# zkemail/zk-email-verify

Measured on NVIDIA H100. Metric: EmailVerifier proofs/sec (witness+prove), higher is better.
Workload: dtype u256 (BN254 Fr/Fq integers, 8x32-bit limbs)

## Files before the change

### include/zkemail_b200.h

```cpp
#ifndef ZKEMAIL_B200_H
#define ZKEMAIL_B200_H

#include <stddef.h>
#include <stdint.h>

#ifdef __cplusplus
extern "C" {
#endif

typedef struct zke_circuit zke_circuit;
typedef struct zke_zkey zke_zkey;
typedef struct zke_ctx zke_ctx;

#define ZKE_FR_BYTES 32

zke_circuit* zke_circuit_build(const char* template_name, const int64_t* params, size_t n_params,
                               char* err, size_t errcap);
zke_circuit* zke_circuit_build_regex(const char* const* parts, const uint8_t* is_public, size_t n_parts, uint32_t msg_len,
                                     char* err, size_t errcap);
zke_circuit* zke_circuit_build_app(const char* spec_json, char* err, size_t errcap);
void zke_circuit_free(zke_circuit* c);
zke_circuit* zke_circuit_from_r1cs(const void* r1cs, size_t len, char* err, size_t errcap);
int64_t zke_circuit_write_r1cs(const zke_circuit* c, uint8_t* out, size_t cap);

typedef struct zke_circuit_info {
    uint32_t n_vars;
    uint32_t n_temps;
    uint32_t n_outputs, n_pub_inputs, n_prv_inputs;
    uint32_t n_public;
    uint32_t n_constraints;
    uint32_t n_levels;
    uint32_t n_ops;
    uint32_t n_coefs;
    uint32_t domain_log2;
    uint32_t n_groups;
    uint64_t nnz_a, nnz_b, nnz_c;
} zke_circuit_info;
int zke_circuit_get_info(const zke_circuit* c, zke_circuit_info* out);

int zke_circuit_group(const zke_circuit* c, uint32_t index, char* name, size_t namecap,
                      uint32_t* first, uint32_t* count, int* kind);
int64_t zke_circuit_input_offset(const zke_circuit* c, const char* name, uint32_t* count);

enum {
    ZKE_ARR_COEFS = 0,
    ZKE_ARR_A_PTR = 1, ZKE_ARR_A_VAR = 2, ZKE_ARR_A_COEF = 3,
    ZKE_ARR_B_PTR = 4, ZKE_ARR_B_VAR = 5, ZKE_ARR_B_COEF = 6,
    ZKE_ARR_C_PTR = 7, ZKE_ARR_C_VAR = 8, ZKE_ARR_C_COEF = 9,
    ZKE_ARR_OPS = 10,
    ZKE_ARR_LEVEL_PTR = 11,
    ZKE_ARR_LC_PTR = 12, ZKE_ARR_LC_VAR = 13, ZKE_ARR_LC_COEF = 14,
    ZKE_ARR_AUX = 15,
    ZKE_ARR_SCOPE_OF_CONSTRAINT = 16,
    ZKE_ARR_SHA_BLOCKS = 17,
    ZKE_ARR_REGEX_SEEDS = 18,
    ZKE_ARR_POSEIDON_BLOCKS = 19
};
const void* zke_circuit_array(const zke_circuit* c, int which, size_t* n_elems);
const char* zke_circuit_scope_name(const zke_circuit* c, uint32_t scope_index);

typedef struct zke_program_stats {
    uint32_t n_levels;
    uint32_t n_iters;
    uint32_t n_ops_kept;
    uint32_t n_coop_ops;
    uint32_t n_terms;
    uint32_t cluster;
    uint64_t digest;
} zke_program_stats;
int zke_circuit_program_stats(const zke_circuit* c, int native_sha, int native_regex, int coop_fpmul, uint32_t cluster,
                              zke_program_stats* out, uint32_t* level_ops, size_t level_cap, char* err, size_t errcap);
enum {
    ZKE_LOWER_NATIVE_SHA = 1, ZKE_LOWER_NATIVE_REGEX = 2, ZKE_LOWER_COOP_FPMUL = 4, ZKE_LOWER_NATIVE_POSEIDON = 8,
    ZKE_LOWER_ALL = 15
};
int zke_circuit_program_stats_ex(const zke_circuit* c, uint32_t flags, uint32_t cluster, zke_program_stats* out,
                                 uint32_t* level_ops, size_t level_cap, char* err, size_t errcap);

int zke_poseidon_hash(const uint8_t* inputs, size_t n, uint8_t* out);

typedef struct zke_registry zke_registry;
int zke_poseidon_batch(const uint8_t* inputs, uint32_t width, size_t count, int device, uint8_t* out, char* err, size_t errcap);
int zke_pubkey_hashes(const uint8_t* moduli, size_t count, uint32_t modulus_bytes, uint32_t n, uint32_t k, int device,
                      uint8_t* out, char* err, size_t errcap);
int zke_domain_key_leaves(const uint8_t* moduli, size_t count, uint32_t modulus_bytes, uint32_t n, uint32_t k,
                          const uint8_t* domains, int device, uint8_t* out, char* err, size_t errcap);
int64_t zke_merkle_build(const uint8_t* leaves, size_t count, uint32_t depth, int device, uint8_t* levels, size_t cap,
                         char* err, size_t errcap);
zke_registry* zke_registry_open(const uint8_t* leaves, size_t count, uint32_t depth, int device, char* err, size_t errcap);
int zke_registry_update(zke_registry* r, const uint64_t* indices, const uint8_t* leaves, size_t k, char* err, size_t errcap);
int zke_registry_nodes(zke_registry* r, const uint32_t* levels, const uint64_t* indices, size_t k, uint8_t* out,
                       char* err, size_t errcap);
int64_t zke_registry_levels(zke_registry* r, uint8_t* out, size_t cap, char* err, size_t errcap);
uint64_t zke_registry_count(const zke_registry* r);
void zke_registry_close(zke_registry* r);
double zke_registry_device_ms(void);


zke_zkey* zke_setup(const zke_circuit* c, uint64_t seed, int device, char* err, size_t errcap);
zke_zkey* zke_zkey_load(const void* zkey_bytes, size_t len, int device, char* err, size_t errcap);
zke_zkey* zke_zkey_load_chunks(const void* const* chunks, const size_t* lens, size_t n_chunks, int device, char* err, size_t errcap);
int64_t zke_zkey_write(const zke_zkey* z, const zke_circuit* c, uint8_t* out, size_t cap);
int zke_zkey_is_toy(const zke_zkey* z);
void zke_zkey_free(zke_zkey* z);
int zke_zkey_info(const zke_zkey* z, uint32_t* n_vars, uint32_t* n_public, uint32_t* domain_log2);
enum {
    ZKE_SEC_ALPHA1 = 101, ZKE_SEC_BETA1 = 102, ZKE_SEC_DELTA1 = 103,
    ZKE_SEC_BETA2 = 104, ZKE_SEC_GAMMA2 = 105, ZKE_SEC_DELTA2 = 106,
    ZKE_SEC_IC = 3, ZKE_SEC_A = 5, ZKE_SEC_B1 = 6, ZKE_SEC_B2 = 7, ZKE_SEC_C = 8, ZKE_SEC_H = 9
};
int64_t zke_zkey_section(const zke_zkey* z, int section, uint8_t* out, size_t cap);

zke_zkey* zke_zkey_from_ptau(const zke_circuit* c, const void* ptau, size_t len, int device, char* err, size_t errcap);
int zke_ptau_info(const zke_circuit* c, const void* ptau, size_t len, uint32_t* power, uint64_t* offsets16, uint64_t* sizes16,
                  char* err, size_t errcap);
int zke_zkey_from_ptau_timing(double* host_ms, double* gpu_ms);
zke_zkey* zke_zkey_contribute(const zke_zkey* prev, const uint8_t* secret32, char* err, size_t errcap);
int zke_zkey_check_contribution(const zke_zkey* prev, const zke_zkey* next, const uint8_t* rand16, char* err, size_t errcap);
int64_t zke_ptau_toy(uint32_t power, const uint8_t* tau_alpha_beta96, int device, uint8_t* out, size_t cap, char* err, size_t errcap);

int64_t zke_ptau_new(uint32_t power, uint8_t* out, size_t cap, char* err, size_t errcap);
int64_t zke_ptau_contribute(const void* ptau, size_t len, const uint8_t* secrets96, int device, uint8_t* out, size_t cap, uint8_t* receipt384,
                            char* err, size_t errcap);
int64_t zke_ptau_prepare(const void* ptau, size_t len, int device, uint8_t* out, size_t cap, char* err, size_t errcap);
int zke_ptau_prepare_timing(double* g1_ms, double* g2_ms);
int zke_ptau_verify(const void* ptau, size_t len, const void* prev, size_t prev_len, const uint8_t* receipt384, const uint8_t* rand16,
                    int device, char* err, size_t errcap);

zke_ctx* zke_ctx_open(const zke_circuit* c, const zke_zkey* zkey_or_null, int device, uint32_t max_batch,
                      char* err, size_t errcap);
void zke_ctx_close(zke_ctx* x);
void* zke_ctx_stream(const zke_ctx* x);
uint64_t zke_kernel_launches(void);

int zke_upload_inputs(zke_ctx* x, const uint8_t* inputs, size_t batch, char* err, size_t errcap);

enum {
    ZKE_STAGE_WITNESS = 0,
    ZKE_STAGE_MATVEC = 1,
    ZKE_STAGE_NTT = 2,
    ZKE_STAGE_MSM_A = 3, ZKE_STAGE_MSM_B1 = 4, ZKE_STAGE_MSM_C = 5,
    ZKE_STAGE_MSM_H = 6,
    ZKE_STAGE_MSM_H_BUCKETS = 7,
    ZKE_STAGE_MSM_B2 = 8,
    ZKE_N_STAGES = 9
};
int zke_ctx_set_lanes(zke_ctx* x, int n);
int zke_ctx_profile(zke_ctx* x, int enable);
int zke_ctx_profile_get(const zke_ctx* x, double* ms_out, uint64_t* count_out);

int zke_witness(zke_ctx* x, const uint8_t* inputs, size_t batch, uint8_t* wtns_out, int32_t* status,
                char* err, size_t errcap);
int zke_load_witness(zke_ctx* x, const uint8_t* wtns, size_t batch, char* err, size_t errcap);
int zke_check_witness(zke_ctx* x, size_t batch, int32_t* status, char* err, size_t errcap);
int zke_prove(zke_ctx* x, size_t batch, const uint8_t* rs, uint8_t* proofs_out, uint8_t* publics_out,
              int32_t* status, char* err, size_t errcap);
int zke_fullprove(zke_ctx* x, const uint8_t* inputs, size_t batch, const uint8_t* rs, uint8_t* proofs_out,
                  uint8_t* publics_out, int32_t* status, char* err, size_t errcap);

int zke_fullprove_submit(zke_ctx* x, const uint8_t* inputs, size_t batch, const uint8_t* rs, char* err, size_t errcap);
int zke_fullprove_collect(zke_ctx* x, uint8_t* proofs_out, uint8_t* publics_out, int32_t* status, char* err, size_t errcap);
int zke_wtns_prove(zke_ctx* x, const void* wtns_bytes, size_t len, const uint8_t* rs, uint8_t* proof_out, uint8_t* publics_out,
                   char* err, size_t errcap);

#define ZKE_SHARD_PARTIAL_BYTES 388
int zke_shard_begin(zke_ctx* x, int rank, int world, char* err, size_t errcap);
void* zke_shard_vector(zke_ctx* x, int which , size_t* n_elems);
int zke_shard_mid(zke_ctx* x, char* err, size_t errcap);
int zke_shard_end(zke_ctx* x, uint8_t* partial_out, uint8_t* publics_out, char* err, size_t errcap);
int zke_shard_combine(const zke_zkey* z, const uint8_t* partials, int world, const uint8_t* rs, uint8_t* proof_out, int32_t* status,
                      char* err, size_t errcap);
int zke_shard_combine_raw(const uint8_t* key_points, const uint8_t* partials, int world, const uint8_t* rs, uint8_t* proof_out,
                          int32_t* status, char* err, size_t errcap);

int zke_verify_json(const char* vkey_json, const char* public_json, const char* proof_json, char* err, size_t errcap);
int zke_verify_batch_json(const char* vkey_json, const char* publics_json, const char* proofs_json, const uint8_t* rand16,
                          uint8_t* ok, char* err, size_t errcap);
typedef struct zke_verifier zke_verifier;
zke_verifier* zke_verifier_open(const char* vkey_json, int device, char* err, size_t errcap);
void zke_verifier_close(zke_verifier* v);
int zke_verifier_batch(zke_verifier* v, size_t n, const uint8_t* proofs, const uint8_t* publics, const uint8_t* rand16,
                       uint8_t* ok, char* err, size_t errcap);
typedef struct zke_agg_srs zke_agg_srs;
zke_agg_srs* zke_agg_srs_from_ptau(const void* ptau_a, size_t len_a, const void* ptau_b, size_t len_b, uint32_t n_max, int device,
                                   char* err, size_t errcap);
void zke_agg_srs_free(zke_agg_srs* s);
uint32_t zke_agg_srs_n_max(const zke_agg_srs* s);
int zke_agg_vk_json(const zke_agg_srs* s, char* out, size_t* len);
size_t zke_agg_bytes(size_t n);
int64_t zke_aggregate(zke_agg_srs* s, const char* vkey_json, size_t n, const uint8_t* proofs, const uint8_t* publics, uint8_t* out,
                      size_t cap, char* err, size_t errcap);
int zke_agg_verify(const char* agg_vk_json, const char* vkey_json, size_t n, const uint8_t* publics, const uint8_t* agg, size_t agg_len,
                   char* err, size_t errcap);
int zke_selftest_pairing_gpu(int device, size_t n, const uint8_t* g1, const uint8_t* g2, uint8_t* out, char* err, size_t errcap);
int zke_zkey_vkey_json(const zke_zkey* z, char* out, size_t* len);
int zke_pairing_alphabeta(const uint8_t* alpha64, const uint8_t* beta128, uint8_t* out384);
int zke_proof_to_json(const uint8_t* proof256, const uint8_t* publics, uint32_t n_public, char* proof_json, size_t* proof_len,
                      char* public_json, size_t* public_len);
int zke_pack_inputs_json(const zke_circuit* c, const char* input_json, uint8_t* out, size_t cap, char* err, size_t errcap);
int zke_fullprove_json(zke_ctx* x, const zke_circuit* c, const char* input_json, char* proof_json, size_t* proof_len,
                       char* public_json, size_t* public_len, char* err, size_t errcap);
int zke_setup_toxic(uint64_t seed, uint8_t* out160);
int zke_selftest_fpmul_hint(uint32_t n, uint32_t k, const uint8_t* a, const uint8_t* b, const uint8_t* p, uint8_t* q, uint8_t* r);

int zke_device_count(void);
const char* zke_version(void);

#ifdef __cplusplus
}
#endif
#endif
```

### zk-email-verify_b200/csrc/engine.cu

```cuda
#include "ff.cuh"
namespace zke { namespace dev { unsigned long long g_kernel_launches = 0; } }
#include "witness.cu"
#include "matvec.cu"
#include "ntt.cu"
#include "msm.cuh"
#include "fixed_base.cuh"
namespace zke { namespace dev {
ZKE_DEFINE_CONSTANT_UPLOAD(upload_constants_engine)
cudaError_t upload_constants_msm_g1(const FieldConsts*, const FieldConsts*);
cudaError_t upload_constants_msm_g2(const FieldConsts*, const FieldConsts*);
cudaError_t upload_constants_fixed_base(const FieldConsts*, const FieldConsts*);
cudaError_t upload_constants_verify(const FieldConsts*, const FieldConsts*);
cudaError_t upload_constants_registry(const FieldConsts*, const FieldConsts*);
} }

#include "../../include/zkemail_b200.h"
#include "cuda_host.hpp"
#include "engine.hpp"
#include "witness_program.hpp"
#include "binfile.hpp"
#include "ec_host.hpp"
#include "setup_host.hpp"
#include <algorithm>
#include <cstdio>
#include <cstring>
#include <atomic>
#include <memory>
#include <mutex>
#include <thread>
#include <unordered_map>

using namespace zke;

void zke::select_device(int device) {
    int n = 0;
    if (cudaGetDeviceCount(&n) != cudaSuccess || n == 0) throw std::runtime_error("no CUDA device available (this library has no CPU fallback)");
    if (device < 0 || device >= n) throw std::runtime_error("bad device index");
    CUDA_OK(cudaSetDevice(device));
    dev::FieldConsts fr, fq;
    fill_consts(fr, fr_params());
    fill_consts(fq, fq_params());
    CUDA_OK(dev::upload_constants_engine(&fr, &fq));
    CUDA_OK(dev::upload_constants_msm_g1(&fr, &fq));
    CUDA_OK(dev::upload_constants_msm_g2(&fr, &fq));
    CUDA_OK(dev::upload_constants_fixed_base(&fr, &fq));
    CUDA_OK(dev::upload_constants_verify(&fr, &fq));
    CUDA_OK(dev::upload_constants_registry(&fr, &fq));
    CUDA_OK(dev::configure_witness_kernel());
}

namespace {

template <class F>
std::vector<AffineH<F>> window_table(const AffineH<F>& gen) {
    std::vector<AffineH<F>> t(32 * 256, AffineH<F>::inf());
    JacobianH<F> base = JacobianH<F>::from_affine(gen);
    for (int w = 0; w < 32; ++w) {
        JacobianH<F> acc = JacobianH<F>::inf();
        for (int d = 1; d < 256; ++d) {
            acc = acc.add(base);
            t[w * 256 + d] = acc.to_affine();
        }
        for (int k = 0; k < 8; ++k) base = base.dbl();
    }
    return t;
}

std::vector<U256> to_standard(const std::vector<Fr>& v) {
    std::vector<U256> out(v.size());
    const unsigned T = std::max(1u, std::min(16u, std::thread::hardware_concurrency()));
    std::vector<std::thread> th;
    for (unsigned t = 0; t < T; ++t)
        th.emplace_back([&, t]() { for (size_t i = v.size() * t / T; i < v.size() * (t + 1) / T; ++i) out[i] = v[i].to_u256(); });
    for (auto& x : th) x.join();
    return out;
}

}

struct zke_zkey {
    uint32_t n_vars = 0, n_public = 0, log_n = 0;
    int device = 0;
    bool toy = false;
    bool delta_one = false;
    G1AffineH alpha1, beta1, delta1;
    G2AffineH beta2, gamma2, delta2;
    std::vector<G1AffineH> ic;
    DevBuf A, B1, B2, C, H;
    int h_levels = 1;
    dev::MsmConfig cfg_h;
    bool has_coefs = false;
    std::vector<uint32_t> a_ptr, a_var, a_coef, b_ptr, b_var, b_coef;
    std::vector<U256> coefs;
};

struct zke_ctx {
    const zke_circuit* circuit = nullptr;
    const zke_zkey* zkey = nullptr;
    int device = 0;
    uint32_t max_batch = 0;
    uint32_t n_vars = 0, n_public = 0, n_inputs = 0;
    cudaStream_t stream = nullptr;
    DevBuf ops, iter_hdr, lc_terms, aux, coop, coef_r, small_inv;
    std::vector<uint32_t> coef_word;
    std::vector<uint32_t> iter_info;
    DevBuf a_ptr, a_terms, b_ptr, b_terms, c_ptr, c_terms;
    dev::DevProgram prog;
    dev::DevR1cs r1cs;
    DevBuf tw_fwd, tw_inv, coset_scale;
    dev::NttTables ntt;
    size_t stride = 0;
    DevBuf inputs, check_flag;
    uint32_t inputs_resident = 0;
    struct Slot {
        bool allocated = false, busy = false;
        DevBuf w_all, inputs, results, first_bad;
        uint8_t* results_host = nullptr;
        uint8_t* publics_host = nullptr;
        std::vector<cudaEvent_t> done;
        cudaEvent_t witness_done = nullptr;
        uint32_t loaded = 0;
        uint32_t batch = 0;
        std::vector<uint8_t> rs;
    };
    Slot slots[2];
    uint64_t n_submitted = 0, n_collected = 0;
    int shard_rank = -1, shard_world = 0, shard_log_g = 0, shard_stage = 0;
    struct Lane { cudaStream_t st = nullptr, heavy = nullptr; cudaEvent_t ev[6] = {}; DevBuf va, vb, vc, vd, msm_ws; };
    Lane lanes[ZKE_MAX_LANES];
    int n_lanes = 1, lanes_alloc = 0;
    int finish_threads = 4;
    dev::MsmConfig cfg_w, cfg_h;
    bool split_streams = true;
    std::vector<uint32_t> bad_host;
    bool profile = false;
    std::vector<cudaEvent_t> ev_pool;
    size_t ev_used = 0;
    struct Span { int stage; size_t e0, e1; };
    std::vector<Span> spans;
    double stage_ms[ZKE_N_STAGES] = {0};
    uint64_t stage_count[ZKE_N_STAGES] = {0};
    cudaEvent_t ev(size_t* idx) {
        if (ev_used == ev_pool.size()) { cudaEvent_t e; cudaEventCreate(&e); ev_pool.push_back(e); }
        *idx = ev_used;
        return ev_pool[ev_used++];
    }
    size_t mark(cudaStream_t st) { size_t i; cudaEventRecord(ev(&i), st); return i; }
    size_t mark() { return mark(stream); }
    void collect() {
        for (auto& s : spans) {
            float ms = 0;
            if (cudaEventElapsedTime(&ms, ev_pool[s.e0], ev_pool[s.e1]) == cudaSuccess) { stage_ms[s.stage] += ms; stage_count[s.stage]++; }
        }
        spans.clear();
        ev_used = 0;
    }
};

static const uint32_t SETUP_SLAB = 1u << 20;
static void h_table_config(zke_zkey* zk, size_t N) {
    const char* e = getenv("ZKE_H_PRECOMP");
    const bool precomp = !(e && atoi(e) == 0);
    zk->cfg_h = dev::msm_config_full((uint32_t)N, precomp);
    zk->h_levels = precomp ? dev::msm_windows(zk->cfg_h) : 1;
}
static void build_h_levels(zke_zkey* zk, size_t N, uint8_t* scratch, cudaStream_t st) {
    for (int lvl = 1; lvl < zk->h_levels; ++lvl) {
        const uint8_t* prev = zk->H.p + (size_t)(lvl - 1) * N * sizeof(dev::G1Affine);
        uint8_t* cur = zk->H.p + (size_t)lvl * N * sizeof(dev::G1Affine);
        for (size_t off = 0; off < N; off += SETUP_SLAB) {
            uint32_t cnt = (uint32_t)std::min<size_t>(SETUP_SLAB, N - off);
            dev::scale_pow2_batch<dev::Fq>(prev + sizeof(dev::G1Affine) * off, cnt, zk->cfg_h.c, scratch, cur + sizeof(dev::G1Affine) * off, st);
        }
    }
    CHECK_LAUNCH();
    CUDA_OK(cudaStreamSynchronize(st));
}

static zke_zkey* do_setup(const zke_circuit* zc, uint64_t seed, int device) {
    select_device(device);
    const Circuit& c = zc->c;
    SetupScalars S = compute_setup_scalars(c, seed);
    std::unique_ptr<zke_zkey> zk(new zke_zkey());
    zk->n_vars = c.n_vars; zk->n_public = c.n_public(); zk->log_n = S.log_n; zk->device = device;
    zk->toy = true;
    const size_t N = (size_t)1 << S.log_n;
    const uint32_t m = c.n_vars, l = c.n_public();

    G1JacH g1 = G1JacH::from_affine(g1_generator());
    G2JacH g2 = G2JacH::from_affine(g2_generator());
    zk->alpha1 = g1.mul(S.alpha.to_u256()).to_affine();
    zk->beta1 = g1.mul(S.beta.to_u256()).to_affine();
    zk->delta1 = g1.mul(S.delta.to_u256()).to_affine();
    zk->beta2 = g2.mul(S.beta.to_u256()).to_affine();
    zk->gamma2 = g2.mul(S.gamma.to_u256()).to_affine();
    zk->delta2 = g2.mul(S.delta.to_u256()).to_affine();

    DevBuf t1, t2, scal, scratch;
    t1.upload(window_table<Fq>(g1_generator()));
    t2.upload(window_table<Fq2>(g2_generator()));
    const uint32_t SLAB = SETUP_SLAB;
    scratch.alloc((size_t)SLAB * sizeof(dev::G2XYZZ));
    cudaStream_t st = nullptr;

    auto run_g1 = [&](const std::vector<Fr>& s, DevBuf& out) {
        std::vector<U256> std_s = to_standard(s);
        scal.upload(std_s);
        out.alloc(s.size() * sizeof(dev::G1Affine));
        for (size_t off = 0; off < s.size(); off += SLAB) {
            uint32_t cnt = (uint32_t)std::min<size_t>(SLAB, s.size() - off);
            dev::fixed_base_batch<dev::Fq>(t1.p, scal.p + 32 * off, cnt, scratch.p, out.p + sizeof(dev::G1Affine) * off, st);
        }
        CHECK_LAUNCH();
        CUDA_OK(cudaStreamSynchronize(st));
    };
    run_g1(S.a, zk->A);
    run_g1(S.b, zk->B1);
    run_g1(S.kc, zk->C);
    {
        h_table_config(zk.get(), N);
        std::vector<U256> std_s = to_standard(S.h);
        scal.upload(std_s);
        zk->H.alloc((size_t)zk->h_levels * N * sizeof(dev::G1Affine));
        for (size_t off = 0; off < N; off += SLAB) {
            uint32_t cnt = (uint32_t)std::min<size_t>(SLAB, N - off);
            dev::fixed_base_batch<dev::Fq>(t1.p, scal.p + 32 * off, cnt, scratch.p, zk->H.p + sizeof(dev::G1Affine) * off, st);
        }
        build_h_levels(zk.get(), N, scratch.p, st);
    }
    {
        std::vector<U256> std_s = to_standard(S.b);
        scal.upload(std_s);
        zk->B2.alloc((size_t)m * sizeof(dev::G2Affine));
        for (size_t off = 0; off < m; off += SLAB) {
            uint32_t cnt = (uint32_t)std::min<size_t>(SLAB, m - off);
            dev::fixed_base_batch<dev::Fq2>(t2.p, scal.p + 32 * off, cnt, scratch.p, zk->B2.p + sizeof(dev::G2Affine) * off, st);
        }
        CHECK_LAUNCH();
        CUDA_OK(cudaStreamSynchronize(st));
    }
    zk->ic.resize(l + 1);
    CUDA_OK(cudaMemcpy(zk->ic.data(), zk->C.p, sizeof(G1AffineH) * (l + 1), cudaMemcpyDeviceToHost));
    CUDA_OK(cudaMemset(zk->C.p, 0, sizeof(G1AffineH) * (l + 1)));
    return zk.release();
}

namespace {
void split_container(const uint8_t* b, size_t len, SecView sec[11]) {
    if (!b || len < 12 || memcmp(b, "zkey", 4) != 0) throw std::runtime_error("not a .zkey file (bad magic)");
    if (rd32(b + 4) != 1) throw std::runtime_error("unsupported .zkey version");
    for (const BinSection& s : binfile_sections(b, len, ".zkey"))
        if (s.type >= 1 && s.type <= 10) sec[s.type] = s.view;
}

template <class Launch>
int64_t first_flagged(uint32_t* flag, Launch launch) {
    CUDA_OK(cudaMemset(flag, 0xff, 4));
    launch(flag);
    ZKE_COUNT_LAUNCH(1);
    CHECK_LAUNCH();
    uint32_t first = 0;
    CUDA_OK(cudaMemcpy(&first, flag, 4, cudaMemcpyDeviceToHost));
    return first == 0xffffffffu ? -1 : (int64_t)first;
}

template <class F>
__global__ void validate_points_kernel(const uint8_t* __restrict__ pts, uint32_t n, F b, uint32_t* bad) {
    const uint32_t i = blockIdx.x * blockDim.x + threadIdx.x;
    if (i >= n) return;
    const dev::Affine<F> p = dev::Affine<F>::load(pts + sizeof(dev::Affine<F>) * (size_t)i);
    if (p.is_inf()) return;
    if (!dev::below_modulus(p.x) || !dev::below_modulus(p.y) || !(p.y.sqr() == p.x.sqr() * p.x + b)) atomicMin(bad, i);
}

template <class F, class HostF>
int64_t first_invalid_point(const uint8_t* pts, size_t n, const HostF& b_host, uint32_t* flag) {
    if (!n) return -1;
    F b;
    static_assert(sizeof(F) == sizeof(HostF), "host / device field images differ");
    memcpy(&b, &b_host, sizeof(F));
    return first_flagged(flag, [&](uint32_t* f) { validate_points_kernel<F><<<(unsigned)((n + 127) / 128), 128>>>(pts, (uint32_t)n, b, f); });
}

Fq2 g2_twist_b() { return Fq2{Fq::from_u64(3), Fq::zero()} * Fq2{Fq::from_u64(9), Fq::one()}.inv(); }

struct U256HashE {
    size_t operator()(const U256& x) const { return (size_t)(x.v[0] * 0x9E3779B97F4A7C15ull ^ x.v[1] * 31 ^ x.v[2] * 131 ^ x.v[3]); }
};
}

static zke_zkey* do_zkey_load(const SecView sec[11], int device) {
    select_device(device);
    for (int s = 1; s <= 9; ++s) if (!sec[s].p) throw std::runtime_error(".zkey section " + std::to_string(s) + " is missing");
    if (sec[1].n < 4 || rd32(sec[1].p) != 1) throw std::runtime_error("not a Groth16 .zkey (protocol id)");
    const uint8_t* h = sec[2].p;
    const size_t HDR = 4 + 32 + 4 + 32 + 12 + 64 + 64 + 128 + 128 + 64 + 128;
    if (sec[2].n < HDR) throw std::runtime_error(".zkey header section too short");
    if (rd32(h) != 32 || memcmp(h + 4, fq_params().p.v, 32) != 0) throw std::runtime_error(".zkey is not over the BN254 base field");
    if (rd32(h + 36) != 32 || memcmp(h + 40, fr_params().p.v, 32) != 0) throw std::runtime_error(".zkey is not over the BN254 scalar field");
    std::unique_ptr<zke_zkey> zk(new zke_zkey());
    zk->device = device;
    zk->n_vars = rd32(h + 72); zk->n_public = rd32(h + 76);
    const uint32_t domain = rd32(h + 80);
    if (domain == 0 || (domain & (domain - 1)) || domain > (1u << 28)) throw std::runtime_error(".zkey domain size is not a power of two <= 2^28");
    zk->log_n = 0;
    while ((1u << zk->log_n) < domain) zk->log_n++;
    const uint32_t m = zk->n_vars, l = zk->n_public;
    if (m == 0 || l + 1 > m) throw std::runtime_error(".zkey header: nPublic + 1 > nVars");
    const size_t N = domain;
    auto need = [&](int s, size_t bytes) {
        if (sec[s].n != bytes) throw std::runtime_error(".zkey section " + std::to_string(s) + " has " + std::to_string(sec[s].n) + " bytes, expected " + std::to_string(bytes));
    };
    need(3, (size_t)(l + 1) * 64); need(5, (size_t)m * 64); need(6, (size_t)m * 64); need(7, (size_t)m * 128);
    need(8, (size_t)(m - l - 1) * 64); need(9, N * 64);

    const uint8_t* q = h + 84;
    memcpy(&zk->alpha1, q, 64); memcpy(&zk->beta1, q + 64, 64); memcpy(&zk->beta2, q + 128, 128);
    memcpy(&zk->gamma2, q + 256, 128); memcpy(&zk->delta1, q + 384, 64); memcpy(&zk->delta2, q + 448, 128);
    auto fq_ok = [](const Fq& x) { return u256_cmp(x.m, fq_params().p) < 0; };
    auto g1_ok = [&](const G1AffineH& p) { return fq_ok(p.x) && fq_ok(p.y) && g1_on_curve(p); };
    auto g2_ok = [&](const G2AffineH& p) { return fq_ok(p.x.c0) && fq_ok(p.x.c1) && fq_ok(p.y.c0) && fq_ok(p.y.c1) && g2_on_curve(p); };
    if (!g1_ok(zk->alpha1) || !g1_ok(zk->beta1) || !g1_ok(zk->delta1) || !g2_ok(zk->beta2) || !g2_ok(zk->gamma2) || !g2_ok(zk->delta2))
        throw std::runtime_error(".zkey header: a key point is not on its curve");
    zk->ic.resize(l + 1);
    memcpy(zk->ic.data(), sec[3].p, (size_t)(l + 1) * 64);
    for (auto& p : zk->ic) if (!g1_ok(p)) throw std::runtime_error(".zkey section 3: an IC point is not on the curve");

    {
        if (sec[4].n < 4) throw std::runtime_error(".zkey section 4 too short");
        const uint32_t n_rec = rd32(sec[4].p);
        if (sec[4].n != 4 + (size_t)n_rec * 44) throw std::runtime_error(".zkey section 4: size does not match its record count");
        const uint8_t* rec = sec[4].p + 4;
        zk->a_ptr.assign(N + 1, 0); zk->b_ptr.assign(N + 1, 0);
        for (uint32_t k = 0; k < n_rec; ++k) {
            const uint8_t* r = rec + 44 * (size_t)k;
            const uint32_t mat = rd32(r), row = rd32(r + 4), sig = rd32(r + 8);
            if (mat > 1 || row >= N || sig >= m) throw std::runtime_error(".zkey section 4: record " + std::to_string(k) + " out of range");
            (mat == 0 ? zk->a_ptr : zk->b_ptr)[row + 1]++;
        }
        for (size_t i = 0; i < N; ++i) { zk->a_ptr[i + 1] += zk->a_ptr[i]; zk->b_ptr[i + 1] += zk->b_ptr[i]; }
        zk->a_var.resize(zk->a_ptr[N]); zk->a_coef.resize(zk->a_ptr[N]);
        zk->b_var.resize(zk->b_ptr[N]); zk->b_coef.resize(zk->b_ptr[N]);
        std::vector<uint32_t> ca(zk->a_ptr.begin(), zk->a_ptr.end() - 1), cb(zk->b_ptr.begin(), zk->b_ptr.end() - 1);
        const Fr r_elem = Fr::from_u256(fr_params().r);
        const Fr rinv2 = (r_elem * r_elem).inv();
        std::unordered_map<U256, uint32_t, U256HashE> index;
        for (uint32_t k = 0; k < n_rec; ++k) {
            const uint8_t* r = rec + 44 * (size_t)k;
            const uint32_t mat = rd32(r), row = rd32(r + 4), sig = rd32(r + 8);
            U256 raw;
            memcpy(raw.v, r + 12, 32);
            auto it = index.find(raw);
            if (it == index.end()) {
                if (u256_cmp(raw, fr_params().p) >= 0) throw std::runtime_error(".zkey section 4: coefficient not reduced mod r");
                it = index.emplace(raw, (uint32_t)zk->coefs.size()).first;
                zk->coefs.push_back((Fr::from_u256(raw) * rinv2).to_u256());
            }
            if (mat == 0) { const uint32_t pos = ca[row]++; zk->a_var[pos] = sig; zk->a_coef[pos] = it->second; }
            else { const uint32_t pos = cb[row]++; zk->b_var[pos] = sig; zk->b_coef[pos] = it->second; }
        }
        if (zk->coefs.size() >= (1u << 24)) throw std::runtime_error(".zkey has more than 2^24 distinct coefficients");
        zk->has_coefs = true;
    }

    DevBuf flag, scratch;
    flag.alloc(4);
    const Fq b1 = Fq::from_u64(3);
    const Fq2 b2 = g2_twist_b();
    auto up = [&](DevBuf& dst, const uint8_t* src, size_t bytes, size_t skip) {
        dst.alloc(skip + bytes);
        if (skip) CUDA_OK(cudaMemset(dst.p, 0, skip));
        if (bytes) CUDA_OK(cudaMemcpy(dst.p + skip, src, bytes, cudaMemcpyHostToDevice));
    };
    auto refuse = [](int64_t bad, const char* what) {
        if (bad >= 0) throw std::runtime_error(std::string(".zkey section ") + what + ": point " + std::to_string(bad) + " is not on the curve");
    };
    uint32_t* fl = (uint32_t*)flag.p;
    up(zk->A, sec[5].p, sec[5].n, 0);   refuse(first_invalid_point<dev::Fq>(zk->A.p, m, b1, fl), "5 (A)");
    up(zk->B1, sec[6].p, sec[6].n, 0);  refuse(first_invalid_point<dev::Fq>(zk->B1.p, m, b1, fl), "6 (B1)");
    up(zk->B2, sec[7].p, sec[7].n, 0);  refuse(first_invalid_point<dev::Fq2>(zk->B2.p, m, b2, fl), "7 (B2)");
    up(zk->C, sec[8].p, sec[8].n, (size_t)(l + 1) * 64);
    refuse(first_invalid_point<dev::Fq>(zk->C.p, m, b1, fl), "8 (C)");
    h_table_config(zk.get(), N);
    zk->H.alloc((size_t)zk->h_levels * N * sizeof(dev::G1Affine));
    CUDA_OK(cudaMemcpy(zk->H.p, sec[9].p, N * 64, cudaMemcpyHostToDevice));
    refuse(first_invalid_point<dev::Fq>(zk->H.p, N, b1, fl), "9 (H)");
    scratch.alloc((size_t)SETUP_SLAB * sizeof(dev::G1XYZZ));
    build_h_levels(zk.get(), N, scratch.p, nullptr);
    return zk.release();
}

static int64_t do_zkey_write(const zke_zkey* zk, const zke_circuit* zc, uint8_t* out, size_t cap) {
    const uint32_t m = zk->n_vars, l = zk->n_public;
    const size_t N = (size_t)1 << zk->log_n;
    const Circuit* c = zc ? &zc->c : nullptr;
    if (!zk->has_coefs) {
        if (!c) throw std::runtime_error("a key made by zke_setup needs its circuit to write the coefficient section");
        if (c->n_vars != m || c->n_public() != l || c->domain_log2() != zk->log_n) throw std::runtime_error("zkey does not belong to this circuit");
    }
    size_t n_rec;
    if (zk->has_coefs) n_rec = zk->a_var.size() + zk->b_var.size();
    else n_rec = c->a_var.size() + c->b_var.size() + l + 1;
    const size_t HDR = 4 + 32 + 4 + 32 + 12 + 64 + 64 + 128 + 128 + 64 + 128;
    const size_t sizes[11] = {0, 4, HDR, (size_t)(l + 1) * 64, 4 + n_rec * 44, (size_t)m * 64, (size_t)m * 64, (size_t)m * 128,
                              (size_t)(m - l - 1) * 64, N * 64, 68};
    size_t total = 12;
    for (int s = 1; s <= 10; ++s) total += 12 + sizes[s];
    if (!out) return (int64_t)total;
    if (cap < total) return -2;
    CUDA_OK(cudaSetDevice(zk->device));
    BinWriter w{out};
    w.header("zkey", 1, 10);
    w.section(1, sizes[1]); w.u32(1);
    w.section(2, sizes[2]);
    w.u32(32); w.bytes(fq_params().p.v, 32); w.u32(32); w.bytes(fr_params().p.v, 32); w.u32(m); w.u32(l); w.u32((uint32_t)N);
    w.bytes(&zk->alpha1, 64); w.bytes(&zk->beta1, 64); w.bytes(&zk->beta2, 128); w.bytes(&zk->gamma2, 128); w.bytes(&zk->delta1, 64); w.bytes(&zk->delta2, 128);
    w.section(3, sizes[3]); w.bytes(zk->ic.data(), (size_t)(l + 1) * 64);
    w.section(4, sizes[4]); w.u32((uint32_t)n_rec);
    {
        const std::vector<U256>& coefs = zk->has_coefs ? zk->coefs : c->coefs;
        const Fr r_elem = Fr::from_u256(fr_params().r);
        const Fr r2 = r_elem * r_elem;
        std::vector<U256> stored(coefs.size());
        for (size_t i = 0; i < coefs.size(); ++i) stored[i] = (Fr::from_u256(coefs[i]) * r2).to_u256();
        auto rows = [&](uint32_t mat, const std::vector<uint32_t>& ptr, const std::vector<uint32_t>& var, const std::vector<uint32_t>& coef, size_t n_rows) {
            for (size_t row = 0; row < n_rows; ++row)
                for (uint32_t k = ptr[row]; k < ptr[row + 1]; ++k) { w.u32(mat); w.u32((uint32_t)row); w.u32(var[k]); w.bytes(stored[coef[k]].v, 32); }
        };
        if (zk->has_coefs) {
            rows(0, zk->a_ptr, zk->a_var, zk->a_coef, N);
            rows(1, zk->b_ptr, zk->b_var, zk->b_coef, N);
        } else {
            rows(0, c->a_ptr, c->a_var, c->a_coef, c->n_constraints);
            rows(1, c->b_ptr, c->b_var, c->b_coef, c->n_constraints);
            const U256 one_r2 = r2.to_u256();
            for (uint32_t j = 0; j <= l; ++j) { w.u32(0); w.u32(c->n_constraints + j); w.u32(j); w.bytes(one_r2.v, 32); }
        }
    }
    auto dev_sec = [&](int s, const DevBuf& b, size_t skip) {
        w.section(s, sizes[s]);
        if (sizes[s]) CUDA_OK(cudaMemcpy(w.p, b.p + skip, sizes[s], cudaMemcpyDeviceToHost));
        w.p += sizes[s];
    };
    dev_sec(5, zk->A, 0); dev_sec(6, zk->B1, 0); dev_sec(7, zk->B2, 0); dev_sec(8, zk->C, (size_t)(l + 1) * 64); dev_sec(9, zk->H, 0);
    w.section(10, sizes[10]); memset(w.p, 0, 68); w.p += 68;
    return (int64_t)(w.p - out);
}

static void alloc_slot(zke_ctx* x, zke_ctx::Slot& S) {
    if (S.allocated) return;
    S.w_all.alloc(x->stride * 32 * x->max_batch);
    S.inputs.alloc((size_t)std::max(1u, x->n_inputs) * 32 * x->max_batch);
    S.first_bad.alloc(4 * (size_t)x->max_batch);
    if (x->zkey) {
        S.results.alloc((size_t)x->max_batch * ZKE_RESULT_STRIDE);
        CUDA_OK(cudaHostAlloc((void**)&S.results_host, (size_t)x->max_batch * ZKE_RESULT_STRIDE, cudaHostAllocDefault));
        CUDA_OK(cudaHostAlloc((void**)&S.publics_host, (size_t)x->max_batch * std::max(1u, x->n_public) * 32, cudaHostAllocDefault));
        S.done.resize(x->max_batch);
        for (auto& e : S.done) CUDA_OK(cudaEventCreateWithFlags(&e, cudaEventDisableTiming));
        CUDA_OK(cudaEventCreateWithFlags(&S.witness_done, cudaEventDisableTiming));
    }
    S.allocated = true;
}

static void check_key_matrices(const Circuit& c, const zke_zkey& zk) {
    const size_t N = (size_t)1 << zk.log_n;
    const uint32_t nc = c.n_constraints, l = c.n_public();
    typedef std::vector<std::pair<uint32_t, Fr>> Form;
    auto canonical = [](Form& f) {
        std::sort(f.begin(), f.end(), [](const std::pair<uint32_t, Fr>& a, const std::pair<uint32_t, Fr>& b) { return a.first < b.first; });
        size_t o = 0;
        for (size_t i = 0; i < f.size();) {
            std::pair<uint32_t, Fr> t = f[i++];
            while (i < f.size() && f[i].first == t.first) t.second = t.second + f[i++].second;
            if (!t.second.is_zero()) f[o++] = t;
        }
        f.resize(o);
    };
    Form x, y;
    auto compare = [&](const char* name, const std::vector<uint32_t>& kp, const std::vector<uint32_t>& kv, const std::vector<uint32_t>& kc,
                       const std::vector<uint32_t>& cp, const std::vector<uint32_t>& cv, const std::vector<uint32_t>& cc, bool extra) {
        for (size_t row = 0; row < N; ++row) {
            const uint32_t kb = kp[row], ke = kp[row + 1];
            if (row < nc) {
                const uint32_t b = cp[row], e = cp[row + 1];
                bool same = e - b == ke - kb;
                for (uint32_t k = 0; same && k < e - b; ++k) same = cv[b + k] == kv[kb + k] && c.coefs[cc[b + k]] == zk.coefs[kc[kb + k]];
                if (same) continue;
            }
            x.clear(); y.clear();
            for (uint32_t k = kb; k < ke; ++k) x.emplace_back(kv[k], Fr::from_u256(zk.coefs[kc[k]]));
            if (row < nc) {
                for (uint32_t k = cp[row]; k < cp[row + 1]; ++k) y.emplace_back(cv[k], Fr::from_u256(c.coefs[cc[k]]));
            } else if (extra && row <= (size_t)nc + l) {
                y.emplace_back((uint32_t)(row - nc), Fr::one());
            }
            canonical(x); canonical(y);
            bool same = x.size() == y.size();
            for (size_t i = 0; same && i < x.size(); ++i) same = x[i].first == y[i].first && x[i].second == y[i].second;
            if (!same) throw std::runtime_error(std::string("zkey does not belong to this circuit: ") + name + " row " + std::to_string(row) + " differs");
        }
    };
    compare("A", zk.a_ptr, zk.a_var, zk.a_coef, c.a_ptr, c.a_var, c.a_coef, true);
    compare("B", zk.b_ptr, zk.b_var, zk.b_coef, c.b_ptr, c.b_var, c.b_coef, false);
}

static void upload_program(zke_ctx* x, const Circuit& c) {
    const uint32_t max_batch = x->max_batch;
    LowerOptions opt;
    if (const char* e = getenv("ZKE_NATIVE_SHA")) opt.native_sha = atoi(e) != 0;
    if (const char* e = getenv("ZKE_NATIVE_REGEX")) opt.native_regex = atoi(e) != 0;
    if (const char* e = getenv("ZKE_NATIVE_POSEIDON")) opt.native_poseidon = atoi(e) != 0;
    if (const char* e = getenv("ZKE_COOP_FPMUL")) opt.coop_fpmul = atoi(e) != 0;
    const uint32_t sms = (uint32_t)dev::sm_count();
    opt.cluster = max_batch <= 8 ? 8 : (max_batch <= 32 ? 4 : (2 * max_batch <= sms ? 2 : 1));
    if (const char* e = getenv("ZKE_WITNESS_CLUSTER")) { const int v = atoi(e); if (v == 1 || v == 2 || v == 4 || v == 8) opt.cluster = (uint32_t)v; }
    WitnessStream S = lower_witness_program(c, x->coef_word, opt);
    x->ops.upload(S.ops);
    x->iter_hdr.upload(S.iter_hdr);
    x->lc_terms.upload(S.terms);
    x->aux.upload(S.aux);
    x->coop.upload(S.coop);
    x->iter_info = std::move(S.iter_info);
    const uint32_t NSMALL = 4096;
    std::vector<Fr> inv(NSMALL);
    for (uint32_t i = 0; i < NSMALL; ++i) inv[i] = Fr::from_u64(i);
    batch_inverse(inv.data(), NSMALL);
    std::vector<U256> inv_std(NSMALL);
    for (uint32_t i = 0; i < NSMALL; ++i) inv_std[i] = inv[i].to_u256();
    x->small_inv.upload(inv_std);
    dev::DevProgram& P = x->prog;
    P.ops = (const uint4*)x->ops.p; P.iter_hdr = (const uint4*)x->iter_hdr.p; P.coop = (const uint32_t*)x->coop.p;
    P.terms = (const uint2*)x->lc_terms.p; P.aux = (const uint32_t*)x->aux.p; P.coef_r = x->coef_r.p;
    P.small_inv = x->small_inv.p; P.n_small_inv = NSMALL;
    P.trace = nullptr;
    P.cluster = S.cluster;
    P.n_iters = S.n_iters; P.n_ops = (uint32_t)c.ops.size(); P.n_vars = c.n_vars; P.n_temps = c.n_temps;
    P.n_outputs = c.n_outputs; P.n_inputs = c.n_inputs();
}

static void upload_r1cs(zke_ctx* x, const Circuit* cp, const zke_zkey* zk) {
    auto up_terms = [&](const std::vector<uint32_t>& var, const std::vector<uint32_t>& coef, DevBuf& dst) {
        std::vector<uint32_t> t(2 * var.size() + 2);
        for (size_t i = 0; i < var.size(); ++i) { t[2 * i] = var[i]; t[2 * i + 1] = x->coef_word[coef[i]]; }
        dst.upload(t);
    };
    dev::DevR1cs& R = x->r1cs;
    if (cp) {
        const Circuit& c = *cp;
        x->a_ptr.upload(c.a_ptr); x->b_ptr.upload(c.b_ptr); x->c_ptr.upload(c.c_ptr);
        up_terms(c.a_var, c.a_coef, x->a_terms); up_terms(c.b_var, c.b_coef, x->b_terms); up_terms(c.c_var, c.c_coef, x->c_terms);
        R.c_ptr = (const uint32_t*)x->c_ptr.p; R.c_terms = (const uint2*)x->c_terms.p;
        R.n_constraints = c.n_constraints; R.n_public = c.n_public();
    } else {
        x->a_ptr.upload(zk->a_ptr); x->b_ptr.upload(zk->b_ptr);
        up_terms(zk->a_var, zk->a_coef, x->a_terms); up_terms(zk->b_var, zk->b_coef, x->b_terms);
        R.c_ptr = nullptr; R.c_terms = nullptr;
        R.n_constraints = 1u << zk->log_n; R.n_public = 0;
    }
    R.a_ptr = (const uint32_t*)x->a_ptr.p; R.b_ptr = (const uint32_t*)x->b_ptr.p;
    R.a_terms = (const uint2*)x->a_terms.p; R.b_terms = (const uint2*)x->b_terms.p;
    R.coef_r = x->coef_r.p; R.n_vars = x->n_vars;
}

namespace {
struct ShoupPair { U256 w, wq; };
U256 mul_lo256(const U256& a, const U256& b) {
    uint64_t t[4] = {0, 0, 0, 0};
    for (int i = 0; i < 4; ++i) {
        u128 c = 0;
        for (int j = 0; i + j < 4; ++j) {
            c += (u128)a.v[j] * b.v[i] + t[i + j];
            t[i + j] = (uint64_t)c;
            c >>= 64;
        }
    }
    return U256{{t[0], t[1], t[2], t[3]}};
}
const U256& fr_neg_inv256() {
    static const U256 v = [] {
        const U256& p = fr_params().p;
        U256 y = {{(uint64_t)0 - fr_params().inv, 0, 0, 0}};
        for (int it = 0; it < 2; ++it) {
            U256 t = mul_lo256(p, y), two = {{2, 0, 0, 0}}, d;
            u256_sub(d, two, t);
            y = mul_lo256(y, d);
        }
        U256 zero = {{0, 0, 0, 0}}, n;
        u256_sub(n, zero, y);
        return n;
    }();
    return v;
}
ShoupPair shoup_pair(const Fr& w) { return ShoupPair{w.to_u256(), mul_lo256(w.m, fr_neg_inv256())}; }
}

static void build_ntt_tables(zke_ctx* x, unsigned log_n) {
    const size_t N = (size_t)1 << log_n;
    const Fr omega = fr_root_of_unity(log_n), omega_inv = omega.inv();
    const Fr g = fr_root_of_unity(log_n + 1);
    const Fr n_inv = Fr::from_u64(N).inv();
    bool shoup = false;
    if (const char* e = getenv("ZKE_NTT_SHOUP")) shoup = atoi(e) != 0;
    const size_t esz = shoup ? 64 : 32;
    std::vector<uint8_t> fw(esz * std::max<size_t>(1, N / 2)), iv(esz * std::max<size_t>(1, N / 2)), cs(esz * N);
    auto put = [&](std::vector<uint8_t>& tab, size_t i, const Fr& w) {
        if (shoup) { const ShoupPair sp = shoup_pair(w); memcpy(&tab[64 * i], sp.w.v, 32); memcpy(&tab[64 * i + 32], sp.wq.v, 32); }
        else memcpy(&tab[32 * i], w.m.v, 32);
    };
    const unsigned T = std::max(1u, std::min(16u, std::thread::hardware_concurrency()));
    std::vector<std::thread> th;
    for (unsigned t = 0; t < T; ++t) {
        th.emplace_back([&, t]() {
            size_t beg = (N / 2) * t / T, end = (N / 2) * (t + 1) / T;
            if (beg < end) {
                U256 e = {{(uint64_t)beg, 0, 0, 0}};
                Fr a = omega.pow(e), b = omega_inv.pow(e);
                for (size_t i = beg; i < end; ++i) { put(fw, i, a); put(iv, i, b); a = a * omega; b = b * omega_inv; }
            }
            beg = N * t / T; end = N * (t + 1) / T;
            if (beg < end) {
                U256 e = {{(uint64_t)beg, 0, 0, 0}};
                Fr a = g.pow(e) * n_inv;
                for (size_t j = beg; j < end; ++j) {
                    size_t p = 0;
                    for (unsigned bit = 0; bit < log_n; ++bit) if (j & ((size_t)1 << bit)) p |= (size_t)1 << (log_n - 1 - bit);
                    put(cs, p, a);
                    a = a * g;
                }
            }
        });
    }
    for (auto& t : th) t.join();
    if (N == 1) { put(fw, 0, Fr::one()); put(iv, 0, Fr::one()); }
    x->tw_fwd.upload(fw); x->tw_inv.upload(iv); x->coset_scale.upload(cs);
    x->ntt.tw_fwd = x->tw_fwd.p; x->ntt.tw_inv = x->tw_inv.p; x->ntt.log_n = (int)log_n; x->ntt.shoup = shoup;
}

static void open_lanes(zke_ctx* x, size_t N, int prio_least, int prio_greatest) {
    const uint32_t max_batch = x->max_batch;
    x->cfg_w = dev::msm_config_witness();
    x->cfg_h = x->zkey->cfg_h;
    size_t ws = std::max(dev::MsmPlan<dev::Fq>::workspace_bytes(x->n_vars, x->cfg_w),
                         dev::MsmPlan<dev::Fq>::workspace_bytes((uint32_t)N, x->cfg_h));
    ws = std::max(ws, dev::MsmPlan<dev::Fq2>::workspace_bytes(x->n_vars, x->cfg_w));
    int want = 8;
    if (const char* e = getenv("ZKE_LANES")) want = atoi(e);
    if (const char* e = getenv("ZKE_SPLIT_STREAMS")) x->split_streams = atoi(e) != 0;
    if (const char* e = getenv("ZKE_FINISH_THREADS")) x->finish_threads = std::max(1, std::min(32, atoi(e)));
    want = std::max(1, std::min(ZKE_MAX_LANES, std::min<int>(want, (int)max_batch)));
    {
        size_t free_b = 0, total_b = 0;
        CUDA_OK(cudaMemGetInfo(&free_b, &total_b));
        const size_t lane_bytes = 4 * N * 32 + ws;
        const size_t keep = x->stride * 32 * max_batch + ((size_t)1 << 30);
        const size_t fit = free_b > keep ? (free_b - keep) / lane_bytes : 0;
        want = std::max(1, std::min<int>(want, (int)std::min<size_t>(fit, ZKE_MAX_LANES)));
    }
    const int prio_light = prio_greatest < prio_least - 1 ? prio_greatest + 1 : prio_greatest;
    for (int i = 0; i < want; ++i) {
        zke_ctx::Lane& L = x->lanes[i];
        CUDA_OK(cudaStreamCreateWithPriority(&L.st, cudaStreamNonBlocking, prio_light));
        CUDA_OK(cudaStreamCreateWithPriority(&L.heavy, cudaStreamNonBlocking, prio_least));
        for (auto& e : L.ev) CUDA_OK(cudaEventCreateWithFlags(&e, cudaEventDisableTiming));
        L.va.alloc(N * 32); L.vb.alloc(N * 32); L.vc.alloc(N * 32); L.vd.alloc(N * 32);
        L.msm_ws.alloc(ws);
    }
    x->lanes_alloc = x->n_lanes = want;
}

static zke_ctx* do_open(const zke_circuit* zc, const zke_zkey* zk, int device, uint32_t max_batch) {
    select_device(device);
    const Circuit* cp = zc ? &zc->c : nullptr;
    if (!cp && !(zk && zk->has_coefs)) throw std::runtime_error("a context needs a circuit, or a proving key loaded from a .zkey");
    if (zk && cp && (zk->n_vars != cp->n_vars || zk->n_public != cp->n_public() || zk->log_n != cp->domain_log2()))
        throw std::runtime_error("zkey does not belong to this circuit");
    if (zk && zk->device != device) throw std::runtime_error("zkey lives on another device");
    if (max_batch == 0) throw std::runtime_error("max_batch must be positive");
    std::unique_ptr<zke_ctx> x(new zke_ctx());
    x->circuit = zc; x->zkey = zk; x->device = device; x->max_batch = max_batch;
    x->n_vars = cp ? cp->n_vars : zk->n_vars;
    x->n_public = cp ? cp->n_public() : zk->n_public;
    x->n_inputs = cp ? cp->n_inputs() : 0;
    int prio_least = 0, prio_greatest = 0;
    CUDA_OK(cudaDeviceGetStreamPriorityRange(&prio_least, &prio_greatest));
    CUDA_OK(cudaStreamCreateWithPriority(&x->stream, cudaStreamNonBlocking, prio_greatest));

    const std::vector<U256>& coefs = cp ? cp->coefs : zk->coefs;
    x->coef_word = coef_words(coefs);
    {
        std::vector<Fr> cr(std::max<size_t>(1, coefs.size()));
        for (size_t i = 0; i < coefs.size(); ++i) cr[i] = Fr::from_u256(coefs[i]);
        x->coef_r.upload(cr);
    }

    if (zk && cp && cp->r1cs_only && zk->has_coefs) check_key_matrices(*cp, *zk);

    if (cp && !cp->r1cs_only) upload_program(x.get(), *cp);
    upload_r1cs(x.get(), cp, zk);
    x->stride = (size_t)x->n_vars + (cp ? cp->n_temps : 0);
    x->inputs.alloc((size_t)std::max(1u, x->n_inputs) * 32 * max_batch);
    x->check_flag.alloc(8);
    x->bad_host.resize(max_batch);
    alloc_slot(x.get(), x->slots[0]);

    if (zk) {
        build_ntt_tables(x.get(), zk->log_n);
        open_lanes(x.get(), (size_t)1 << zk->log_n, prio_least, prio_greatest);
    }
    CUDA_OK(cudaDeviceSynchronize());
    return x.release();
}

static std::string assert_message(const zke_ctx* x, uint32_t email, uint32_t row) {
    std::string scope = "?";
    if (x->circuit) {
        const Circuit& c = x->circuit->c;
        if (row < c.scope_of_constraint.size()) scope = c.scopes[c.scope_of_constraint[row]];
    }
    return "Assert Failed: constraint " + std::to_string(row) + " in template " + scope + " @ email " + std::to_string(email);
}

static void require_idle(const zke_ctx* x) {
    if (x->n_submitted != x->n_collected) throw std::runtime_error("a submitted batch is still in flight: call zke_fullprove_collect first");
}

static void do_witness(zke_ctx* x, zke_ctx::Slot& S, const uint8_t* inputs, size_t batch) {
    if (!x->circuit) throw std::runtime_error("this context was opened from a .zkey alone: it has no witness program (use zke_load_witness / zke_wtns_prove)");
    const Circuit& c = x->circuit->c;
    if (c.r1cs_only) throw std::runtime_error(R1CS_NO_PROGRAM);
    if (batch == 0 || batch > x->max_batch) throw std::runtime_error("batch exceeds the context's max_batch");
    CUDA_OK(cudaSetDevice(x->device));
    const uint8_t* in_dev = x->inputs.p;
    if (inputs) {
        if (c.n_inputs()) CUDA_OK(cudaMemcpyAsync(S.inputs.p, inputs, (size_t)c.n_inputs() * 32 * batch, cudaMemcpyHostToDevice, x->stream));
        in_dev = S.inputs.p;
    } else if (x->inputs_resident < batch) {
        throw std::runtime_error("inputs == NULL but no (or too few) inputs are resident: call zke_upload_inputs first");
    }
    size_t p0 = 0;
    if (x->profile) p0 = x->mark();
    if (const char* tp = getenv("ZKE_WITNESS_TRACE")) {
        DevBuf tr;
        tr.alloc(8 * ((size_t)x->prog.n_iters + 1));
        dev::DevProgram P = x->prog;
        P.trace = (unsigned long long*)tr.p;
        dev::launch_witness(P, S.w_all.p, x->stride, in_dev, (uint32_t)batch, x->stream);
        CUDA_OK(cudaStreamSynchronize(x->stream));
        std::vector<unsigned long long> h(x->prog.n_iters);
        CUDA_OK(cudaMemcpy(h.data(), tr.p, 8 * h.size(), cudaMemcpyDeviceToHost));
        if (FILE* f = fopen(tp, "wb")) {
            fwrite(h.data(), 8, h.size(), f);
            fwrite(x->iter_info.data(), 4, x->iter_info.size(), f);
            fclose(f);
        }
    }
    dev::launch_witness(x->prog, S.w_all.p, x->stride, in_dev, (uint32_t)batch, x->stream);
    CHECK_LAUNCH();
    if (x->profile) x->spans.push_back({ZKE_STAGE_WITNESS, p0, x->mark()});
    S.loaded = (uint32_t)batch;
}

static int do_check(zke_ctx* x, zke_ctx::Slot& S, size_t batch, int32_t* status, std::string& msg) {
    CUDA_OK(cudaMemsetAsync(S.first_bad.p, 0xff, 4 * batch, x->stream));
    dev::launch_check_rows(x->r1cs, S.w_all.p, x->stride, (uint32_t)batch, (uint32_t*)S.first_bad.p, x->stream);
    CHECK_LAUNCH();
    CUDA_OK(cudaMemcpyAsync(x->bad_host.data(), S.first_bad.p, 4 * batch, cudaMemcpyDeviceToHost, x->stream));
    CUDA_OK(cudaStreamSynchronize(x->stream));
    if (x->profile) x->collect();
    int bad = 0;
    for (size_t e = 0; e < batch; ++e) {
        int32_t s = x->bad_host[e] == 0xffffffffu ? -1 : (int32_t)x->bad_host[e];
        if (status) status[e] = s;
        if (s >= 0) { if (!bad) msg = assert_message(x, (uint32_t)e, (uint32_t)s); ++bad; }
    }
    return bad;
}

template <class F>
static AffineH<F> finish_msm(const uint8_t* block, const dev::MsmConfig& cfg) {
    const XyzzH<F>* slots = reinterpret_cast<const XyzzH<F>*>(block);
    const int n_windows = cfg.precomputed ? 1 : (255 + cfg.c - 1) / cfg.c;
    XyzzH<F> acc = XyzzH<F>::inf();
    for (int j = n_windows - 1; j >= 0; --j) {
        if (!acc.is_inf()) for (int k = 0; k < cfg.c; ++k) acc.dbl();
        acc.add(slots[dev::MSM_ONES_SLOTS + j]);
    }
    if (cfg.classify) for (int i = 0; i < dev::MSM_ONES_SLOTS; ++i) acc.add(slots[i]);
    return acc.to_affine();
}

template <class Queued>
static void enqueue_witness_msms(const zke_ctx* x, const uint8_t* w, uint32_t lo, uint32_t hi, uint8_t* ws, uint8_t* res,
                                 cudaStream_t st, Queued queued) {
    const zke_zkey* zk = x->zkey;
    w += 32ull * lo;
    dev::MsmPlan<dev::Fq>::run(zk->A.p + 64ull * lo, w, hi - lo, x->cfg_w, ws, res + RES_A * ZKE_RES_G1_BLOCK, st);
    queued(ZKE_STAGE_MSM_A);
    dev::MsmPlan<dev::Fq>::run(zk->B1.p + 64ull * lo, w, hi - lo, x->cfg_w, ws, res + RES_B1 * ZKE_RES_G1_BLOCK, st);
    queued(ZKE_STAGE_MSM_B1);
    dev::MsmPlan<dev::Fq>::run(zk->C.p + 64ull * lo, w, hi - lo, x->cfg_w, ws, res + RES_C * ZKE_RES_G1_BLOCK, st);
    queued(ZKE_STAGE_MSM_C);
    dev::MsmPlan<dev::Fq2>::run(zk->B2.p + 128ull * lo, w, hi - lo, x->cfg_w, ws, res + RES_B2 * ZKE_RES_G1_BLOCK, st);
    CHECK_LAUNCH();
    queued(ZKE_STAGE_MSM_B2);
}

struct MsmSums { G1AffineH a, b1, c, h; G2AffineH b2; };

static MsmSums finish_msms(const uint8_t* res, const dev::MsmConfig& cfg_w, const dev::MsmConfig& cfg_h) {
    return MsmSums{finish_msm<Fq>(res + RES_A * ZKE_RES_G1_BLOCK, cfg_w), finish_msm<Fq>(res + RES_B1 * ZKE_RES_G1_BLOCK, cfg_w),
                   finish_msm<Fq>(res + RES_C * ZKE_RES_G1_BLOCK, cfg_w), finish_msm<Fq>(res + RES_H * ZKE_RES_G1_BLOCK, cfg_h),
                   finish_msm<Fq2>(res + RES_B2 * ZKE_RES_G1_BLOCK, cfg_w)};
}

struct KeyPoints { G1AffineH alpha1, beta1, delta1; G2AffineH beta2, delta2; };

static void assemble_proof(const KeyPoints& kp, const G1JacH& a, const G1JacH& b1, const G1JacH& c, const G1JacH& h, const G2JacH& b2,
                           const U256& r, const U256& s, uint8_t out[256]) {
    const G1JacH delta1 = G1JacH::from_affine(kp.delta1);
    const G1JacH pa = G1JacH::from_affine(kp.alpha1).add(a).add(delta1.mul(r));
    const G2JacH pb2 = G2JacH::from_affine(kp.beta2).add(b2).add(G2JacH::from_affine(kp.delta2).mul(s));
    const G1JacH pb1 = G1JacH::from_affine(kp.beta1).add(b1).add(delta1.mul(s));
    const U256 rs_prod = (Fr::from_u256(r) * Fr::from_u256(s)).to_u256();
    const G1JacH pc = c.add(h).add(pa.mul(s)).add(pb1.mul(r)).add(delta1.mul(rs_prod).neg());
    store_g1(out, pa.to_affine());
    store_g2(out + 64, pb2.to_affine());
    store_g1(out + 192, pc.to_affine());
}

static void sync_lanes(zke_ctx* x) {
    cudaStreamSynchronize(x->stream);
    for (int i = 0; i < x->lanes_alloc; ++i) { cudaStreamSynchronize(x->lanes[i].st); cudaStreamSynchronize(x->lanes[i].heavy); }
}

static void enqueue_prove(zke_ctx* x, zke_ctx::Slot& S, size_t batch, const uint8_t* rs) {
    const zke_zkey* zk = x->zkey;
    if (!zk) throw std::runtime_error("context was opened without a proving key");
    if (batch == 0 || batch > S.loaded) throw std::runtime_error("no witness loaded for this batch (call zke_witness first)");
    if (rs) {
        for (size_t e = 0; e < 2 * batch; ++e) {
            U256 v;
            memcpy(v.v, rs + 32 * e, 32);
            if (u256_cmp(v, fr_params().p) >= 0) throw std::runtime_error("r / s not reduced mod the group order");
        }
        S.rs.assign(rs, rs + 64 * batch);
    } else {
        S.rs.clear();
    }
    CUDA_OK(cudaSetDevice(x->device));
    const uint32_t N = 1u << zk->log_n, m = x->n_vars, l = x->n_public;
    const bool prof = x->profile;
    const int n_lanes = prof ? 1 : x->n_lanes;
    if (const char* e = getenv("ZKE_SPLIT_STREAMS")) x->split_streams = atoi(e) != 0;
    if (l) CUDA_OK(cudaMemcpy2DAsync(S.publics_host, (size_t)l * 32, S.w_all.p + 32, x->stride * 32, (size_t)l * 32, batch, cudaMemcpyDeviceToHost, x->stream));
    CUDA_OK(cudaEventRecord(S.witness_done, x->stream));
    for (int i = 0; i < n_lanes; ++i) CUDA_OK(cudaStreamWaitEvent(x->lanes[i].st, S.witness_done, 0));
    for (size_t e = 0; e < batch; ++e) {
        zke_ctx::Lane& L = x->lanes[e % n_lanes];
        cudaStream_t st = L.st;
        const uint8_t* w = S.w_all.p + 32 * x->stride * e;
        uint8_t* res = S.results.p + (size_t)ZKE_RESULT_STRIDE * e;
        uint32_t* flag = (uint32_t*)(res + ZKE_RES_FLAG_OFF);
        size_t t0 = 0, t1 = 0;
        CUDA_OK(cudaMemsetAsync(flag, 0xff, 4, st));
        if (prof) t0 = x->mark(st);
        auto span = [&](int stage) { if (prof) { t1 = x->mark(st); x->spans.push_back({stage, t0, t1}); t0 = t1; } };
        cudaStream_t hv = (prof || !x->split_streams) ? st : L.heavy;
        dev::launch_build_ab(x->r1cs, w, L.va.p, L.vb.p, L.vc.p, N, flag, st);
        span(ZKE_STAGE_MATVEC);
        if (hv != st) { CUDA_OK(cudaEventRecord(L.ev[0], st)); CUDA_OK(cudaStreamWaitEvent(hv, L.ev[0], 0)); }
        dev::launch_intt_dif(L.va.p, x->ntt, x->coset_scale.p, hv);
        dev::launch_intt_dif(L.vb.p, x->ntt, x->coset_scale.p, hv);
        dev::launch_intt_dif(L.vc.p, x->ntt, x->coset_scale.p, hv);
        dev::launch_ntt_dit(L.va.p, x->ntt, hv);
        dev::launch_ntt_dit(L.vb.p, x->ntt, hv);
        dev::launch_ntt_dit(L.vc.p, x->ntt, hv);
        dev::launch_quotient(L.va.p, L.vb.p, L.vc.p, L.vd.p, N, hv);
        CHECK_LAUNCH();
        if (hv != st) CUDA_OK(cudaEventRecord(L.ev[1], hv));
        span(ZKE_STAGE_NTT);
        enqueue_witness_msms(x, w, 0, m, L.msm_ws.p, res, st, span);
        if (hv != st) CUDA_OK(cudaStreamWaitEvent(st, L.ev[1], 0));
        const dev::MsmPlan<dev::Fq>::Heavy heavy{hv, L.ev[2], L.ev[3]};
        size_t i0 = 0, i1 = 0;
        cudaEvent_t evs[2] = {prof ? x->ev(&i0) : nullptr, prof ? x->ev(&i1) : nullptr};
        dev::MsmPlan<dev::Fq>::run(zk->H.p, L.vd.p, N, x->cfg_h, L.msm_ws.p, res + RES_H * ZKE_RES_G1_BLOCK, st, prof ? evs : nullptr, &heavy);
        if (prof) x->spans.push_back({ZKE_STAGE_MSM_H_BUCKETS, i0, i1});
        span(ZKE_STAGE_MSM_H);
        CHECK_LAUNCH();
        CUDA_OK(cudaMemcpyAsync(S.results_host + (size_t)ZKE_RESULT_STRIDE * e, res, ZKE_RESULT_STRIDE, cudaMemcpyDeviceToHost, st));
        CUDA_OK(cudaEventRecord(S.done[e], st));
    }
    S.batch = (uint32_t)batch;
}

static int finish_prove(zke_ctx* x, zke_ctx::Slot& S, uint8_t* proofs_out, uint8_t* publics_out, int32_t* status, std::string& msg) {
    const zke_zkey* zk = x->zkey;
    const size_t batch = S.batch;
    const uint32_t l = x->n_public;
    const KeyPoints kp{zk->alpha1, zk->beta1, zk->delta1, zk->beta2, zk->delta2};
    std::vector<int32_t> st_local(batch, -1);
    std::string first_error;
    std::mutex err_mutex;
    auto one = [&](size_t e) {
        CUDA_OK(cudaEventSynchronize(S.done[e]));
        const uint8_t* res = S.results_host + (size_t)ZKE_RESULT_STRIDE * e;
        uint32_t flag;
        memcpy(&flag, res + ZKE_RES_FLAG_OFF, 4);
        const int32_t s = flag == 0xffffffffu ? -1 : (int32_t)flag;
        st_local[e] = s;
        uint8_t* out = proofs_out + 256 * e;
        if (s >= 0) { memset(out, 0, 256); return; }
        U256 r, sc;
        if (!S.rs.empty()) { memcpy(r.v, S.rs.data() + 64 * e, 32); memcpy(sc.v, S.rs.data() + 64 * e + 32, 32); }
        else { random_scalar(r); random_scalar(sc); }
        const MsmSums m = finish_msms(res, x->cfg_w, x->cfg_h);
        assemble_proof(kp, G1JacH::from_affine(m.a), G1JacH::from_affine(m.b1), G1JacH::from_affine(m.c), G1JacH::from_affine(m.h),
                       G2JacH::from_affine(m.b2), r, sc, out);
    };
    const int T = (int)std::max<size_t>(1, std::min<size_t>((size_t)x->finish_threads, batch));
    std::atomic<size_t> next{0};
    auto worker = [&]() {
        try {
            cudaSetDevice(x->device);
            for (;;) {
                const size_t e = next.fetch_add(1);
                if (e >= batch) break;
                one(e);
            }
        } catch (const std::exception& ex) {
            std::lock_guard<std::mutex> lock(err_mutex);
            if (first_error.empty()) first_error = ex.what();
        }
    };
    if (T == 1) worker();
    else {
        std::vector<std::thread> th;
        for (int t = 0; t < T; ++t) th.emplace_back(worker);
        for (auto& t : th) t.join();
    }
    if (x->profile) { sync_lanes(x); x->collect(); }
    if (!first_error.empty()) { sync_lanes(x); throw std::runtime_error(first_error); }
    int bad = 0;
    for (size_t e = 0; e < batch; ++e) {
        if (status) status[e] = st_local[e];
        if (st_local[e] >= 0) { if (!bad) msg = assert_message(x, (uint32_t)e, (uint32_t)st_local[e]); ++bad; }
    }
    if (publics_out && l) memcpy(publics_out, S.publics_host, (size_t)l * 32 * batch);
    return bad;
}

static int do_prove(zke_ctx* x, zke_ctx::Slot& S, size_t batch, const uint8_t* rs, uint8_t* proofs_out, uint8_t* publics_out, int32_t* status, std::string& msg) {
    try {
        enqueue_prove(x, S, batch, rs);
    } catch (...) {
        sync_lanes(x);
        throw;
    }
    return finish_prove(x, S, proofs_out, publics_out, status, msg);
}

static const uint8_t* parse_wtns(const uint8_t* b, size_t len, uint32_t expect_vars) {
    if (!b || len < 12 || memcmp(b, "wtns", 4) != 0) throw std::runtime_error("not a .wtns file (bad magic)");
    std::vector<BinSection> secs;
    try { secs = binfile_sections(b, len, ".wtns"); }
    catch (const std::runtime_error&) { throw std::runtime_error("truncated .wtns"); }
    const uint8_t *s1 = nullptr, *s2 = nullptr;
    size_t n1 = 0, n2 = 0;
    for (const BinSection& s : secs) {
        if (s.type == 1) { s1 = s.view.p; n1 = s.view.n; }
        if (s.type == 2) { s2 = s.view.p; n2 = s.view.n; }
    }
    if (!s1 || !s2 || n1 < 40) throw std::runtime_error(".wtns sections missing");
    if (rd32(s1) != 32 || memcmp(s1 + 4, fr_params().p.v, 32) != 0) throw std::runtime_error(".wtns is not over the BN254 scalar field");
    const uint32_t n = rd32(s1 + 36);
    if (n != expect_vars) throw std::runtime_error(".wtns has " + std::to_string(n) + " values, the key expects " + std::to_string(expect_vars));
    if (n2 != (size_t)n * 32) throw std::runtime_error(".wtns data section has the wrong size");
    return s2;
}

static void load_witness(zke_ctx* x, zke_ctx::Slot& S, const uint8_t* wtns, size_t batch) {
    if (batch == 0 || batch > x->max_batch) throw std::runtime_error("batch exceeds the context's max_batch");
    CUDA_OK(cudaSetDevice(x->device));
    const size_t m = x->n_vars;
    CUDA_OK(cudaMemcpy2DAsync(S.w_all.p, x->stride * 32, wtns, m * 32, m * 32, batch, cudaMemcpyHostToDevice, x->stream));
    CUDA_OK(cudaMemsetAsync(x->check_flag.p, 0, 8, x->stream));
    dev::launch_check_witness(S.w_all.p, x->stride, (uint32_t)m, (uint32_t)batch, (uint32_t*)x->check_flag.p, x->stream);
    CHECK_LAUNCH();
    uint32_t flags[2] = {0, 0};
    CUDA_OK(cudaMemcpyAsync(flags, x->check_flag.p, 8, cudaMemcpyDeviceToHost, x->stream));
    CUDA_OK(cudaStreamSynchronize(x->stream));
    S.loaded = 0;
    if (flags[0]) throw std::runtime_error("witness value not reduced mod r");
    if (flags[1]) throw std::runtime_error("witness[0] must be 1");
    S.loaded = (uint32_t)batch;
}

static void shard_geometry(const zke_ctx* x, int& log_m, int& log_cols, uint32_t& col0) {
    log_m = (int)x->zkey->log_n - x->shard_log_g;
    log_cols = log_m - x->shard_log_g;
    col0 = (uint32_t)x->shard_rank << log_cols;
}

static void shard_begin(zke_ctx* x, int rank, int world) {
    const zke_zkey* zk = x->zkey;
    if (!zk) throw std::runtime_error("context was opened without a proving key");
    require_idle(x);
    int log_g = 0;
    while ((1 << log_g) < world) ++log_g;
    if (world < 2 || world > 8 || (1 << log_g) != world) throw std::runtime_error("sharded proving supports 2, 4 or 8 GPUs");
    if (rank < 0 || rank >= world) throw std::runtime_error("bad shard rank");
    if ((int)zk->log_n < 2 * log_g + 10) throw std::runtime_error("domain too small to shard (use batch parallelism)");
    zke_ctx::Slot& S = x->slots[0];
    if (S.loaded < 1) throw std::runtime_error("no witness loaded (call zke_witness / zke_load_witness on every rank first)");
    CUDA_OK(cudaSetDevice(x->device));
    x->shard_rank = rank; x->shard_world = world; x->shard_log_g = log_g;
    int log_m, log_cols; uint32_t col0;
    shard_geometry(x, log_m, log_cols, col0);
    zke_ctx::Lane& L = x->lanes[0];
    cudaStream_t st = L.st;
    CUDA_OK(cudaStreamSynchronize(x->stream));
    uint32_t* flag = (uint32_t*)(S.results.p + ZKE_RES_FLAG_OFF);
    CUDA_OK(cudaMemsetAsync(flag, 0xff, 4, st));
    dev::RowMap map;
    map.log_cols = log_cols; map.log_m = log_m; map.col0 = col0;
    const uint32_t n_rows = (uint32_t)world << log_cols;
    dev::launch_build_ab(x->r1cs, S.w_all.p, L.va.p, L.vb.p, L.vc.p, n_rows, flag, st, &map);
    const uint32_t n_cols = 1u << log_cols;
    dev::launch_intt_cross(L.va.p, x->ntt, log_g, col0, n_cols, st);
    dev::launch_intt_cross(L.vb.p, x->ntt, log_g, col0, n_cols, st);
    dev::launch_intt_cross(L.vc.p, x->ntt, log_g, col0, n_cols, st);
    CHECK_LAUNCH();
    CUDA_OK(cudaStreamSynchronize(st));
    x->shard_stage = 1;
}

static void shard_mid(zke_ctx* x) {
    if (x->shard_stage != 1) throw std::runtime_error("zke_shard_mid out of order");
    CUDA_OK(cudaSetDevice(x->device));
    int log_m, log_cols; uint32_t col0;
    shard_geometry(x, log_m, log_cols, col0);
    zke_ctx::Lane& L = x->lanes[0];
    cudaStream_t st = L.st;
    const size_t block_off = ((size_t)x->shard_rank << log_m);
    for (uint8_t* v : {L.va.p, L.vb.p, L.vc.p}) {
        dev::launch_intt_dif_block(v + 32 * block_off, x->ntt, log_m, x->coset_scale.p + (x->ntt.shoup ? 64 : 32) * block_off, st);
        dev::launch_ntt_dit_block(v + 32 * block_off, x->ntt, log_m, st);
    }
    CHECK_LAUNCH();
    CUDA_OK(cudaStreamSynchronize(st));
    x->shard_stage = 2;
}

static const char PARTIAL_COORD[] = "partial point coordinate";
static void write_partial(const MsmSums& m, uint32_t first_bad, uint8_t* out) {
    store_g1(out, m.a); store_g1(out + 64, m.b1); store_g1(out + 128, m.c); store_g1(out + 192, m.h); store_g2(out + 256, m.b2);
    memcpy(out + 384, &first_bad, 4);
}
static MsmSums read_partial(const uint8_t* p, uint32_t& first_bad) {
    const MsmSums m{load_g1(p, PARTIAL_COORD), load_g1(p + 64, PARTIAL_COORD), load_g1(p + 128, PARTIAL_COORD),
                    load_g1(p + 192, PARTIAL_COORD), load_g2(p + 256, PARTIAL_COORD)};
    if (!g1_on_curve(m.a) || !g1_on_curve(m.b1) || !g1_on_curve(m.c) || !g1_on_curve(m.h) || !g2_on_curve(m.b2)) throw std::runtime_error("partial point not on the curve");
    memcpy(&first_bad, p + 384, 4);
    return m;
}

static void shard_end(zke_ctx* x, uint8_t* partial_out, uint8_t* publics_out) {
    if (x->shard_stage != 2) throw std::runtime_error("zke_shard_end out of order");
    const zke_zkey* zk = x->zkey;
    CUDA_OK(cudaSetDevice(x->device));
    int log_m, log_cols; uint32_t col0;
    shard_geometry(x, log_m, log_cols, col0);
    zke_ctx::Slot& S = x->slots[0];
    zke_ctx::Lane& L = x->lanes[0];
    cudaStream_t st = L.st;
    const uint32_t N = 1u << zk->log_n, m = x->n_vars, l = x->n_public;
    const int G = x->shard_world, log_g = x->shard_log_g;
    const uint32_t n_cols = 1u << log_cols;
    dev::launch_ntt_cross(L.va.p, x->ntt, log_g, col0, n_cols, st);
    dev::launch_ntt_cross(L.vb.p, x->ntt, log_g, col0, n_cols, st);
    dev::launch_ntt_cross(L.vc.p, x->ntt, log_g, col0, n_cols, st);
    CUDA_OK(cudaMemsetAsync(L.vd.p, 0, (size_t)N * 32, st));
    dev::launch_quotient_cols(L.va.p, L.vb.p, L.vc.p, L.vd.p, (int)zk->log_n, log_g, col0, (uint32_t)log_cols, st);
    CHECK_LAUNCH();
    const uint32_t lo = (uint32_t)((uint64_t)m * x->shard_rank / G), hi = (uint32_t)((uint64_t)m * (x->shard_rank + 1) / G);
    uint8_t* res = S.results.p;
    enqueue_witness_msms(x, S.w_all.p, lo, hi, L.msm_ws.p, res, st, [](int) {});
    dev::MsmPlan<dev::Fq>::run(zk->H.p, L.vd.p, N, x->cfg_h, L.msm_ws.p, res + RES_H * ZKE_RES_G1_BLOCK, st);
    CHECK_LAUNCH();
    CUDA_OK(cudaMemcpyAsync(S.results_host, res, ZKE_RESULT_STRIDE, cudaMemcpyDeviceToHost, st));
    if (l) CUDA_OK(cudaMemcpyAsync(S.publics_host, S.w_all.p + 32, (size_t)l * 32, cudaMemcpyDeviceToHost, st));
    CUDA_OK(cudaStreamSynchronize(st));
    uint32_t first_bad;
    memcpy(&first_bad, S.results_host + ZKE_RES_FLAG_OFF, 4);
    write_partial(finish_msms(S.results_host, x->cfg_w, x->cfg_h), first_bad, partial_out);
    if (publics_out && l) memcpy(publics_out, S.publics_host, (size_t)l * 32);
    x->shard_stage = 0;
}

static int shard_combine(const KeyPoints& kp, const uint8_t* partials, int world, const uint8_t* rs, uint8_t* out, int32_t* status) {
    G1JacH sa = G1JacH::inf(), sb1 = G1JacH::inf(), sc = G1JacH::inf(), sh = G1JacH::inf();
    G2JacH sb2 = G2JacH::inf();
    uint32_t first_bad = 0xffffffffu;
    for (int r = 0; r < world; ++r) {
        uint32_t f;
        const MsmSums m = read_partial(partials + (size_t)ZKE_SHARD_PARTIAL_BYTES * r, f);
        sa = sa.add_affine(m.a); sb1 = sb1.add_affine(m.b1); sc = sc.add_affine(m.c); sh = sh.add_affine(m.h); sb2 = sb2.add_affine(m.b2);
        first_bad = std::min(first_bad, f);
    }
    if (status) *status = first_bad == 0xffffffffu ? -1 : (int32_t)first_bad;
    if (first_bad != 0xffffffffu) { memset(out, 0, 256); return 1; }
    U256 r, s;
    if (rs) { memcpy(r.v, rs, 32); memcpy(s.v, rs + 32, 32); }
    else { random_scalar(r); random_scalar(s); }
    if (u256_cmp(r, fr_params().p) >= 0 || u256_cmp(s, fr_params().p) >= 0) throw std::runtime_error("r / s not reduced mod the group order");
    assemble_proof(kp, sa, sb1, sc, sh, sb2, r, s, out);
    return 0;
}

extern "C" {

int zke_device_count(void) {
    int n = 0;
    if (cudaGetDeviceCount(&n) != cudaSuccess) return 0;
    return n;
}

zke_zkey* zke_setup(const zke_circuit* c, uint64_t seed, int device, char* err, size_t errcap) {
    try { if (!c) throw std::runtime_error("null circuit"); return do_setup(c, seed, device); }
    catch (const std::exception& e) { set_err(err, errcap, e.what()); return nullptr; }
}
zke_zkey* zke_zkey_load(const void* zkey_bytes, size_t len, int device, char* err, size_t errcap) {
    try {
        SecView sec[11];
        split_container((const uint8_t*)zkey_bytes, len, sec);
        return do_zkey_load(sec, device);
    } catch (const std::exception& e) { set_err(err, errcap, e.what()); return nullptr; }
}
zke_zkey* zke_zkey_load_chunks(const void* const* chunks, const size_t* lens, size_t n_chunks, int device, char* err, size_t errcap) {
    try {
        if (!chunks || !lens || n_chunks < 9) throw std::runtime_error("expected the chunk files b..j (sections 1-9; k is optional)");
        SecView sec[11];
        for (size_t i = 0; i < n_chunks && i < 10; ++i) sec[i + 1] = SecView{(const uint8_t*)chunks[i], lens[i]};
        return do_zkey_load(sec, device);
    } catch (const std::exception& e) { set_err(err, errcap, e.what()); return nullptr; }
}
int64_t zke_zkey_write(const zke_zkey* z, const zke_circuit* c, uint8_t* out, size_t cap) {
    try { if (!z) return -1; return do_zkey_write(z, c, out, cap); }
    catch (const std::exception&) { return -3; }
}
int zke_zkey_is_toy(const zke_zkey* z) { return z ? (z->toy ? 1 : 0) : -1; }
void zke_zkey_free(zke_zkey* z) { if (z) { cudaSetDevice(z->device); delete z; } }

int zke_zkey_info(const zke_zkey* z, uint32_t* n_vars, uint32_t* n_public, uint32_t* domain_log2) {
    if (!z) return -1;
    if (n_vars) *n_vars = z->n_vars;
    if (n_public) *n_public = z->n_public;
    if (domain_log2) *domain_log2 = z->log_n;
    return 0;
}

int64_t zke_zkey_section(const zke_zkey* z, int section, uint8_t* out, size_t cap) {
    if (!z) return -1;
    try {
        CUDA_OK(cudaSetDevice(z->device));
        const size_t N = (size_t)1 << z->log_n;
        auto g1_host = [&](const G1AffineH* pts, size_t n) -> int64_t {
            if (!out) return (int64_t)n;
            if (cap < n * 64) return -2;
            for (size_t i = 0; i < n; ++i) store_g1(out + 64 * i, pts[i]);
            return (int64_t)n;
        };
        auto g1_dev = [&](const DevBuf& b, size_t n) -> int64_t {
            if (!out) return (int64_t)n;
            std::vector<G1AffineH> h(n);
            CUDA_OK(cudaMemcpy(h.data(), b.p, n * sizeof(G1AffineH), cudaMemcpyDeviceToHost));
            return g1_host(h.data(), n);
        };
        auto g2_host = [&](const G2AffineH* pts, size_t n) -> int64_t {
            if (!out) return (int64_t)n;
            if (cap < n * 128) return -2;
            for (size_t i = 0; i < n; ++i) store_g2(out + 128 * i, pts[i]);
            return (int64_t)n;
        };
        switch (section) {
            case ZKE_SEC_ALPHA1: return g1_host(&z->alpha1, 1);
            case ZKE_SEC_BETA1: return g1_host(&z->beta1, 1);
            case ZKE_SEC_DELTA1: return g1_host(&z->delta1, 1);
            case ZKE_SEC_BETA2: return g2_host(&z->beta2, 1);
            case ZKE_SEC_GAMMA2: return g2_host(&z->gamma2, 1);
            case ZKE_SEC_DELTA2: return g2_host(&z->delta2, 1);
            case ZKE_SEC_IC: return g1_host(z->ic.data(), z->ic.size());
            case ZKE_SEC_A: return g1_dev(z->A, z->n_vars);
            case ZKE_SEC_B1: return g1_dev(z->B1, z->n_vars);
            case ZKE_SEC_C: return g1_dev(z->C, z->n_vars);
            case ZKE_SEC_H: return g1_dev(z->H, N);
            case ZKE_SEC_B2: {
                if (!out) return z->n_vars;
                std::vector<G2AffineH> h(z->n_vars);
                CUDA_OK(cudaMemcpy(h.data(), z->B2.p, h.size() * sizeof(G2AffineH), cudaMemcpyDeviceToHost));
                return g2_host(h.data(), h.size());
            }
            default: return -1;
        }
    } catch (const std::exception&) { return -3; }
}

zke_ctx* zke_ctx_open(const zke_circuit* c, const zke_zkey* zkey, int device, uint32_t max_batch, char* err, size_t errcap) {
    try { return do_open(c, zkey, device, max_batch); }
    catch (const std::exception& e) { set_err(err, errcap, e.what()); return nullptr; }
}
void zke_ctx_close(zke_ctx* x) {
    if (!x) return;
    cudaSetDevice(x->device);
    sync_lanes(x);
    for (auto e : x->ev_pool) cudaEventDestroy(e);
    for (auto& S : x->slots) {
        for (auto e : S.done) cudaEventDestroy(e);
        if (S.witness_done) cudaEventDestroy(S.witness_done);
        if (S.results_host) cudaFreeHost(S.results_host);
        if (S.publics_host) cudaFreeHost(S.publics_host);
    }
    for (int i = 0; i < x->lanes_alloc; ++i) {
        if (x->lanes[i].st) cudaStreamDestroy(x->lanes[i].st);
        if (x->lanes[i].heavy) cudaStreamDestroy(x->lanes[i].heavy);
        for (auto e : x->lanes[i].ev) if (e) cudaEventDestroy(e);
    }
    if (x->stream) cudaStreamDestroy(x->stream);
    delete x;
}

int zke_upload_inputs(zke_ctx* x, const uint8_t* inputs, size_t batch, char* err, size_t errcap) {
    try {
        if (!x || !inputs) throw std::runtime_error("null argument");
        if (x->circuit && x->circuit->c.r1cs_only) throw std::runtime_error(R1CS_NO_PROGRAM);
        if (batch == 0 || batch > x->max_batch) throw std::runtime_error("batch exceeds the context's max_batch");
        require_idle(x);
        CUDA_OK(cudaSetDevice(x->device));
        const size_t n = x->n_inputs;
        if (n) CUDA_OK(cudaMemcpy(x->inputs.p, inputs, n * 32 * batch, cudaMemcpyHostToDevice));
        x->inputs_resident = (uint32_t)batch;
        return 0;
    } catch (const std::exception& e) { set_err(err, errcap, e.what()); return -1; }
}

int zke_ctx_set_lanes(zke_ctx* x, int n) {
    if (!x || n < 1) return -1;
    x->n_lanes = n > x->lanes_alloc ? x->lanes_alloc : n;
    return x->n_lanes;
}
int zke_ctx_profile(zke_ctx* x, int enable) {
    if (!x) return -1;
    x->profile = enable != 0;
    for (int i = 0; i < ZKE_N_STAGES; ++i) { x->stage_ms[i] = 0; x->stage_count[i] = 0; }
    return 0;
}
int zke_ctx_profile_get(const zke_ctx* x, double* ms_out, uint64_t* count_out) {
    if (!x) return -1;
    for (int i = 0; i < ZKE_N_STAGES; ++i) { if (ms_out) ms_out[i] = x->stage_ms[i]; if (count_out) count_out[i] = x->stage_count[i]; }
    return ZKE_N_STAGES;
}
void* zke_ctx_stream(const zke_ctx* x) { return x ? (void*)x->stream : nullptr; }
uint64_t zke_kernel_launches(void) { return dev::g_kernel_launches; }

int zke_witness(zke_ctx* x, const uint8_t* inputs, size_t batch, uint8_t* wtns_out, int32_t* status, char* err, size_t errcap) {
    try {
        if (!x) throw std::runtime_error("null context");
        require_idle(x);
        zke_ctx::Slot& S = x->slots[0];
        do_witness(x, S, inputs, batch);
        std::string msg;
        int bad = do_check(x, S, batch, status, msg);
        if (wtns_out) {
            const size_t m = x->n_vars;
            CUDA_OK(cudaMemcpy2D(wtns_out, m * 32, S.w_all.p, x->stride * 32, m * 32, batch, cudaMemcpyDeviceToHost));
        }
        if (bad) { set_err(err, errcap, msg); return bad; }
        return 0;
    } catch (const std::exception& e) { set_err(err, errcap, e.what()); return -1; }
}

int zke_load_witness(zke_ctx* x, const uint8_t* wtns, size_t batch, char* err, size_t errcap) {
    try {
        if (!x || !wtns) throw std::runtime_error("null argument");
        require_idle(x);
        load_witness(x, x->slots[0], wtns, batch);
        return 0;
    } catch (const std::exception& e) { set_err(err, errcap, e.what()); return -1; }
}

int zke_check_witness(zke_ctx* x, size_t batch, int32_t* status, char* err, size_t errcap) {
    try {
        if (!x) throw std::runtime_error("null context");
        if (!x->circuit) throw std::runtime_error("this context was opened from a .zkey alone: it has no C matrix to check witnesses against (open it with the circuit)");
        require_idle(x);
        zke_ctx::Slot& S = x->slots[0];
        if (batch == 0 || batch > S.loaded) throw std::runtime_error("no witness loaded for this batch (call zke_load_witness first)");
        CUDA_OK(cudaSetDevice(x->device));
        std::string msg;
        int bad = do_check(x, S, batch, status, msg);
        if (bad) { set_err(err, errcap, msg); return bad; }
        return 0;
    } catch (const std::exception& e) { set_err(err, errcap, e.what()); return -1; }
}

int zke_prove(zke_ctx* x, size_t batch, const uint8_t* rs, uint8_t* proofs_out, uint8_t* publics_out, int32_t* status, char* err, size_t errcap) {
    try {
        if (!x || !proofs_out) throw std::runtime_error("null argument");
        require_idle(x);
        std::string msg;
        int bad = do_prove(x, x->slots[0], batch, rs, proofs_out, publics_out, status, msg);
        if (bad) { set_err(err, errcap, msg); return bad; }
        return 0;
    } catch (const std::exception& e) { set_err(err, errcap, e.what()); return -1; }
}

int zke_wtns_prove(zke_ctx* x, const void* wtns_bytes, size_t len, const uint8_t* rs, uint8_t* proof_out, uint8_t* publics_out,
                   char* err, size_t errcap) {
    try {
        if (!x || !proof_out) throw std::runtime_error("null argument");
        require_idle(x);
        const uint8_t* data = parse_wtns((const uint8_t*)wtns_bytes, len, x->n_vars);
        load_witness(x, x->slots[0], data, 1);
        std::string msg;
        int32_t status = -1;
        int bad = do_prove(x, x->slots[0], 1, rs, proof_out, publics_out, &status, msg);
        if (bad) { set_err(err, errcap, msg); return bad; }
        return 0;
    } catch (const std::exception& e) { set_err(err, errcap, e.what()); return -1; }
}

int zke_fullprove_submit(zke_ctx* x, const uint8_t* inputs, size_t batch, const uint8_t* rs, char* err, size_t errcap) {
    try {
        if (!x) throw std::runtime_error("null context");
        if (x->profile) throw std::runtime_error("stage profiling needs the synchronous entry points");
        if (x->n_submitted - x->n_collected >= 2) throw std::runtime_error("two batches are already in flight: collect one first");
        CUDA_OK(cudaSetDevice(x->device));
        zke_ctx::Slot& S = x->slots[x->n_submitted & 1];
        alloc_slot(x, S);
        try {
            do_witness(x, S, inputs, batch);
            enqueue_prove(x, S, batch, rs);
        } catch (...) { sync_lanes(x); throw; }
        S.busy = true;
        x->n_submitted++;
        return 0;
    } catch (const std::exception& e) { set_err(err, errcap, e.what()); return -1; }
}

int zke_fullprove_collect(zke_ctx* x, uint8_t* proofs_out, uint8_t* publics_out, int32_t* status, char* err, size_t errcap) {
    try {
        if (!x || !proofs_out) throw std::runtime_error("null argument");
        if (x->n_submitted == x->n_collected) throw std::runtime_error("nothing was submitted");
        zke_ctx::Slot& S = x->slots[x->n_collected & 1];
        x->n_collected++;
        S.busy = false;
        std::string msg;
        int bad = finish_prove(x, S, proofs_out, publics_out, status, msg);
        if (bad) { set_err(err, errcap, msg); return bad; }
        return 0;
    } catch (const std::exception& e) { set_err(err, errcap, e.what()); return -1; }
}

int zke_fullprove(zke_ctx* x, const uint8_t* inputs, size_t batch, const uint8_t* rs, uint8_t* proofs_out, uint8_t* publics_out,
                  int32_t* status, char* err, size_t errcap) {
    try {
        if (!x || !proofs_out) throw std::runtime_error("null argument");
        require_idle(x);
        zke_ctx::Slot& S = x->slots[0];
        do_witness(x, S, inputs, batch);
        std::string msg;
        int bad = do_prove(x, S, batch, rs, proofs_out, publics_out, status, msg);
        if (bad) { set_err(err, errcap, msg); return bad; }
        return 0;
    } catch (const std::exception& e) { set_err(err, errcap, e.what()); return -1; }
}

int zke_shard_begin(zke_ctx* x, int rank, int world, char* err, size_t errcap) {
    try { if (!x) throw std::runtime_error("null context"); shard_begin(x, rank, world); return 0; }
    catch (const std::exception& e) { set_err(err, errcap, e.what()); return -1; }
}
void* zke_shard_vector(zke_ctx* x, int which, size_t* n_elems) {
    if (!x || !x->zkey || which < 0 || which > 2 || x->lanes_alloc < 1) return nullptr;
    if (n_elems) *n_elems = (size_t)1 << x->zkey->log_n;
    zke_ctx::Lane& L = x->lanes[0];
    return which == 0 ? L.va.p : (which == 1 ? L.vb.p : L.vc.p);
}
int zke_shard_mid(zke_ctx* x, char* err, size_t errcap) {
    try { if (!x) throw std::runtime_error("null context"); shard_mid(x); return 0; }
    catch (const std::exception& e) { set_err(err, errcap, e.what()); return -1; }
}
int zke_shard_end(zke_ctx* x, uint8_t* partial_out, uint8_t* publics_out, char* err, size_t errcap) {
    try { if (!x || !partial_out) throw std::runtime_error("null argument"); shard_end(x, partial_out, publics_out); return 0; }
    catch (const std::exception& e) { set_err(err, errcap, e.what()); return -1; }
}
int zke_shard_combine(const zke_zkey* z, const uint8_t* partials, int world, const uint8_t* rs, uint8_t* proof_out, int32_t* status,
                      char* err, size_t errcap) {
    try {
        if (!z || !partials || !proof_out || world < 1) throw std::runtime_error("bad argument");
        const KeyPoints kp{z->alpha1, z->beta1, z->delta1, z->beta2, z->delta2};
        int bad = shard_combine(kp, partials, world, rs, proof_out, status);
        if (bad) set_err(err, errcap, "Assert Failed: constraint " + std::to_string(status ? *status : 0));
        return bad;
    } catch (const std::exception& e) { set_err(err, errcap, e.what()); return -1; }
}
int zke_shard_combine_raw(const uint8_t* key_points, const uint8_t* partials, int world, const uint8_t* rs, uint8_t* proof_out,
                          int32_t* status, char* err, size_t errcap) {
    try {
        if (!key_points || !partials || !proof_out || world < 1) throw std::runtime_error("bad argument");
        const KeyPoints kp{load_g1(key_points, PARTIAL_COORD), load_g1(key_points + 64, PARTIAL_COORD), load_g1(key_points + 128, PARTIAL_COORD),
                          load_g2(key_points + 192, PARTIAL_COORD), load_g2(key_points + 320, PARTIAL_COORD)};
        int bad = shard_combine(kp, partials, world, rs, proof_out, status);
        if (bad) set_err(err, errcap, "Assert Failed: constraint " + std::to_string(status ? *status : 0));
        return bad;
    } catch (const std::exception& e) { set_err(err, errcap, e.what()); return -1; }
}

}

#include "setup.cu"
#include "ptau.cu"
#include "aggregate.cu"
```

### zk-email-verify_b200/csrc/msm.cu

```cuda
#include "device_engine.cuh"
#include "msm.cuh"
#include "msm_ba.cuh"
#include "msm_sort.cuh"
#if defined(ZKE_MSM_G1)
#include "msm_tc.cuh"
#endif
#include <algorithm>
#include <cstdlib>
#include <stdexcept>

namespace zke {
namespace dev {

static const int LIST_FANIN = 32;
static const int TREE_FANIN = 8;

__device__ __forceinline__ Fr load_scalar(const uint8_t* scalars, uint32_t i) { return Fr::load(scalars + 32ull * i); }

template <class F>
__global__ void classify_kernel(const uint8_t* __restrict__ points, const uint8_t* __restrict__ scalars, uint32_t n,
                                uint32_t* ones_list, uint32_t* gen_list, uint32_t* counters ) {
    const uint32_t i = blockIdx.x * blockDim.x + threadIdx.x;
    if (i >= n) return;
    Fr s = load_scalar(scalars, i);
    if (s.is_zero()) return;
    Affine<F> p = Affine<F>::load(points + sizeof(Affine<F>) * (size_t)i);
    if (p.is_inf()) return;
    bool one = s.v[0] == 1 && (s.v[1] | s.v[2] | s.v[3] | s.v[4] | s.v[5] | s.v[6] | s.v[7]) == 0;
    if (one) ones_list[atomicAdd(&counters[0], 1u)] = i;
    else gen_list[atomicAdd(&counters[1], 1u)] = i;
}

template <class F>
__global__ void sum_affine_list_kernel(const uint8_t* __restrict__ points, const uint32_t* __restrict__ list,
                                       const uint32_t* __restrict__ count_ptr, uint32_t count_fixed, uint8_t* out) {
    const uint32_t count = count_ptr ? *count_ptr : count_fixed;
    const uint32_t t = blockIdx.x * blockDim.x + threadIdx.x;
    const uint32_t n_out = max(1u, (count + LIST_FANIN - 1) / LIST_FANIN);
    if (t >= n_out) return;
    XYZZ<F> acc = XYZZ<F>::inf();
    for (uint32_t k = t; k < count; k += n_out) {
        uint32_t idx = list ? list[k] : k;
        acc.madd(Affine<F>::load(points + sizeof(Affine<F>) * (size_t)idx), false);
    }
    acc.store(out + sizeof(XYZZ<F>) * (size_t)t);
}

__device__ __forceinline__ uint32_t tree_level_size(uint32_t count, uint32_t level) {
    uint32_t n = max(1u, (count + LIST_FANIN - 1) / LIST_FANIN);
    for (uint32_t d = 0; d < level; ++d) n = max(1u, (n + TREE_FANIN - 1) / TREE_FANIN);
    return n;
}
template <class F>
__global__ void sum_xyzz_kernel(const uint8_t* __restrict__ in, const uint32_t* __restrict__ count_ptr, uint32_t count_fixed,
                                uint32_t level, uint32_t pad_to, uint8_t* out) {
    const uint32_t count = count_ptr ? *count_ptr : count_fixed;
    const uint32_t n_in = tree_level_size(count, level), n_out = tree_level_size(count, level + 1);
    const uint32_t t = blockIdx.x * blockDim.x + threadIdx.x;
    if (t >= n_out) {
        if (t < pad_to) XYZZ<F>::inf().store(out + sizeof(XYZZ<F>) * (size_t)t);
        return;
    }
    XYZZ<F> acc = XYZZ<F>::inf();
    for (uint32_t k = t; k < n_in; k += n_out) acc.add(XYZZ<F>::load(in + sizeof(XYZZ<F>) * (size_t)k));
    acc.store(out + sizeof(XYZZ<F>) * (size_t)t);
}

struct Digits {
    int c, n_windows;
    uint32_t half;
    uint32_t chunk;
    uint32_t group;
    uint32_t window_bucket_stride;
    uint32_t window_point_stride;
};

__device__ __forceinline__ uint32_t window_bits(const Fr& s, int bit, int c) {
    const int w = bit >> 5, b = bit & 31;
    uint64_t two = s.v[w];
    if (w + 1 < 8) two |= (uint64_t)s.v[w + 1] << 32;
    return (uint32_t)((two >> b) & ((1u << c) - 1));
}

__device__ __forceinline__ bool minimal_magnitude(Fr& s) {
    const FieldConsts& C = FR_C;
    Fr n;
    n.v[0] = sub_cc(C.mod[0], s.v[0]);
#pragma unroll
    for (int i = 1; i < 8; ++i) n.v[i] = subc_cc(C.mod[i], s.v[i]);
    (void)subc(0, 0);
    bool less = false, decided = false;
#pragma unroll
    for (int i = 7; i >= 0; --i) {
        if (!decided && n.v[i] != s.v[i]) { less = n.v[i] < s.v[i]; decided = true; }
    }
    if (less) { s = n; return true; }
    return false;
}

template <class Fn>
__device__ __forceinline__ void for_each_digit(Fr s, const Digits& D, Fn f) {
    const bool flip = minimal_magnitude(s);
    uint32_t carry = 0;
    for (int j = 0; j < D.n_windows; ++j) {
        uint32_t raw = window_bits(s, j * D.c, D.c) + carry;
        if (raw > D.half) {
            carry = 1;
            const uint32_t mag = (1u << D.c) - raw;
            if (mag) f(j, mag - 1, !flip);
        } else {
            carry = 0;
            if (raw) f(j, raw - 1, flip);
        }
    }
}

static const int SORT_PART_BITS = 8;
static const uint32_t SORT_PARTS = 1u << SORT_PART_BITS;
static const int SORT_MAX_FINE_BITS = 11;
static const int SORT_THREADS = 256;
static const int SORT_FINE_THREADS = 512;
static const uint32_t SORT_STAGE = 6656;
static const uint32_t SORT_TILE = 16384;
static const uint32_t SORT_TWO_LEVEL_MIN_BUCKETS = 1u << 16;
static const size_t SORT_FINE_SMEM = 4 * (3 * ((size_t)1 << SORT_MAX_FINE_BITS) + 1 + SORT_FINE_THREADS + SORT_TILE);

template <int THREADS>
__device__ __forceinline__ void block_exclusive_scan(uint32_t* s, uint32_t n, uint32_t* tmp) {
    const uint32_t per = (n + THREADS - 1) / THREADS, beg = min(n, threadIdx.x * per), end = min(n, beg + per);
    uint32_t local = 0;
    for (uint32_t i = beg; i < end; ++i) local += s[i];
    tmp[threadIdx.x] = local;
    __syncthreads();
    for (uint32_t off = 1; off < THREADS; off <<= 1) {
        const uint32_t v = threadIdx.x >= off ? tmp[threadIdx.x - off] : 0;
        __syncthreads();
        tmp[threadIdx.x] += v;
        __syncthreads();
    }
    uint32_t run = tmp[threadIdx.x] - local;
    for (uint32_t i = beg; i < end; ++i) { const uint32_t v = s[i]; s[i] = run; run += v; }
    if (threadIdx.x == THREADS - 1) s[n] = tmp[THREADS - 1];
    __syncthreads();
}

static __global__ void __launch_bounds__(SORT_THREADS)
sort_coarse_count_kernel(const uint8_t* __restrict__ scalars, const uint32_t* __restrict__ list, const uint32_t* __restrict__ count_ptr,
                         uint32_t count_fixed, Digits D, int fine_bits, uint32_t n_parts, uint32_t tile, uint32_t* mat) {
    __shared__ uint32_t s_bin[SORT_PARTS];
    const uint32_t count = count_ptr ? *count_ptr : count_fixed;
    for (uint32_t i = threadIdx.x; i < n_parts; i += SORT_THREADS) s_bin[i] = 0;
    __syncthreads();
    const uint32_t beg = blockIdx.x * tile, end = min(count, beg + tile);
    for (uint32_t t = beg + threadIdx.x; t < end; t += SORT_THREADS) {
        Fr s = load_scalar(scalars, list ? list[t] : t);
        for_each_digit(s, D, [&](int j, uint32_t b, bool) { atomicAdd(&s_bin[((uint32_t)j * D.window_bucket_stride + b) >> fine_bits], 1u); });
    }
    __syncthreads();
    for (uint32_t i = threadIdx.x; i < n_parts; i += SORT_THREADS) mat[(size_t)i * gridDim.x + blockIdx.x] = s_bin[i];
}

static __global__ void __launch_bounds__(SORT_THREADS)
sort_coarse_scatter_kernel(const uint8_t* __restrict__ scalars, const uint32_t* __restrict__ list, const uint32_t* __restrict__ count_ptr,
                           uint32_t count_fixed, Digits D, int fine_bits, uint32_t n_parts, uint32_t tile, const uint32_t* __restrict__ off,
                           uint32_t* __restrict__ stage, uint16_t* __restrict__ stage_fine) {
    __shared__ uint32_t s_base[SORT_PARTS + 1], s_cur[SORT_PARTS], s_goff[SORT_PARTS], s_tmp[SORT_THREADS];
    __shared__ uint32_t s_word[SORT_STAGE];
    __shared__ uint16_t s_fine[SORT_STAGE];
    const uint32_t count = count_ptr ? *count_ptr : count_fixed;
    for (uint32_t p = threadIdx.x; p < SORT_PARTS; p += SORT_THREADS) {
        const size_t c = (size_t)p * gridDim.x + blockIdx.x;
        s_goff[p] = p < n_parts ? off[c] : 0;
        s_base[p] = p < n_parts ? off[c + 1] - off[c] : 0;
    }
    __syncthreads();
    block_exclusive_scan<SORT_THREADS>(s_base, SORT_PARTS, s_tmp);
    for (uint32_t p = threadIdx.x; p < SORT_PARTS; p += SORT_THREADS) s_cur[p] = s_base[p];
    __syncthreads();
    const uint32_t beg = blockIdx.x * tile, end = min(count, beg + tile);
    for (uint32_t t = beg + threadIdx.x; t < end; t += SORT_THREADS) {
        const uint32_t idx = list ? list[t] : t;
        Fr s = load_scalar(scalars, idx);
        for_each_digit(s, D, [&](int j, uint32_t b, bool neg) {
            const uint32_t bucket = (uint32_t)j * D.window_bucket_stride + b;
            const uint32_t pos = atomicAdd(&s_cur[bucket >> fine_bits], 1u);
            s_word[pos] = ((uint32_t)j * D.window_point_stride + idx) | (neg ? 0x80000000u : 0u);
            s_fine[pos] = (uint16_t)(bucket & ((1u << fine_bits) - 1));
        });
    }
    __syncthreads();
    for (uint32_t i = threadIdx.x; i < s_base[SORT_PARTS]; i += SORT_THREADS) {
        const uint32_t p = sort_tile_part(s_base, SORT_PARTS, i);
        const uint32_t g = s_goff[p] + (i - s_base[p]);
        stage[g] = s_word[i];
        stage_fine[g] = s_fine[i];
    }
}

static __global__ void sort_part_count_kernel(const uint32_t* __restrict__ coarse_off, uint32_t coarse_blocks, uint32_t n_parts,
                                              uint32_t* part_count) {
    const uint32_t p = blockIdx.x * blockDim.x + threadIdx.x;
    if (p < n_parts) part_count[p] = coarse_off[(size_t)(p + 1) * coarse_blocks] - coarse_off[(size_t)p * coarse_blocks];
}

__device__ __forceinline__ bool sort_fine_tile(const uint32_t* coarse_off, uint32_t coarse_blocks, const uint32_t* tile_base, uint32_t n_parts,
                                               uint32_t w, uint32_t& tb, uint32_t& tiles_p, uint32_t& t, uint32_t& beg, uint32_t& end) {
    if (w >= tile_base[n_parts]) return false;
    const uint32_t p = sort_tile_part(tile_base, n_parts, w);
    tb = tile_base[p]; tiles_p = tile_base[p + 1] - tb; t = w - tb;
    beg = coarse_off[(size_t)p * coarse_blocks] + t * SORT_TILE;
    end = min(coarse_off[(size_t)(p + 1) * coarse_blocks], beg + SORT_TILE);
    return true;
}

static __global__ void __launch_bounds__(SORT_THREADS)
sort_fine_count_kernel(const uint32_t* __restrict__ coarse_off, uint32_t coarse_blocks, const uint32_t* __restrict__ tile_base,
                       uint32_t n_parts, int fine_bits, const uint16_t* __restrict__ stage_fine, uint32_t* mat) {
    __shared__ uint32_t s_bin[1u << SORT_MAX_FINE_BITS];
    const uint32_t n_fine = 1u << fine_bits;
    uint32_t tb, tiles_p, t, beg, end;
    if (!sort_fine_tile(coarse_off, coarse_blocks, tile_base, n_parts, blockIdx.x, tb, tiles_p, t, beg, end)) {
        for (uint32_t f = threadIdx.x; f < n_fine; f += SORT_THREADS) mat[((size_t)blockIdx.x << fine_bits) + f] = 0;
        return;
    }
    for (uint32_t f = threadIdx.x; f < n_fine; f += SORT_THREADS) s_bin[f] = 0;
    __syncthreads();
    for (uint32_t k = beg + threadIdx.x; k < end; k += SORT_THREADS) atomicAdd(&s_bin[stage_fine[k]], 1u);
    __syncthreads();
    for (uint32_t f = threadIdx.x; f < n_fine; f += SORT_THREADS) mat[sort_cell(tb, tiles_p, f, t, fine_bits)] = s_bin[f];
}

static __global__ void __launch_bounds__(SORT_FINE_THREADS)
sort_fine_scatter_kernel(const uint32_t* __restrict__ coarse_off, uint32_t coarse_blocks, const uint32_t* __restrict__ tile_base,
                         uint32_t n_parts, int fine_bits, const uint32_t* __restrict__ stage, const uint16_t* __restrict__ stage_fine,
                         const uint32_t* __restrict__ off, uint32_t* __restrict__ entries) {
    extern __shared__ uint32_t smem[];
    const uint32_t n_fine = 1u << fine_bits;
    uint32_t* s_base = smem;
    uint32_t* s_cur = s_base + n_fine + 1;
    uint32_t* s_goff = s_cur + n_fine;
    uint32_t* s_tmp = s_goff + n_fine;
    uint32_t* s_word = s_tmp + SORT_FINE_THREADS;
    uint32_t tb, tiles_p, t, beg, end;
    if (!sort_fine_tile(coarse_off, coarse_blocks, tile_base, n_parts, blockIdx.x, tb, tiles_p, t, beg, end)) return;
    for (uint32_t f = threadIdx.x; f < n_fine; f += SORT_FINE_THREADS) {
        const size_t c = sort_cell(tb, tiles_p, f, t, fine_bits);
        s_goff[f] = off[c];
        s_base[f] = off[c + 1] - off[c];
    }
    __syncthreads();
    block_exclusive_scan<SORT_FINE_THREADS>(s_base, n_fine, s_tmp);
    for (uint32_t f = threadIdx.x; f < n_fine; f += SORT_FINE_THREADS) s_cur[f] = s_base[f];
    __syncthreads();
    for (uint32_t k = beg + threadIdx.x; k < end; k += SORT_FINE_THREADS) s_word[atomicAdd(&s_cur[stage_fine[k]], 1u)] = stage[k];
    __syncthreads();
    for (uint32_t i = threadIdx.x; i < end - beg; i += SORT_FINE_THREADS) {
        const uint32_t f = sort_tile_part(s_base, n_fine, i);
        entries[s_goff[f] + (i - s_base[f])] = s_word[i];
    }
}

static __global__ void sort_offsets_kernel(uint32_t n_buckets, int fine_bits, const uint32_t* __restrict__ coarse_off, uint32_t coarse_blocks,
                                           const uint32_t* __restrict__ tile_base, const uint32_t* __restrict__ fine_off,
                                           uint32_t* hist, uint32_t* offsets) {
    const uint32_t b = blockIdx.x * blockDim.x + threadIdx.x;
    if (b > n_buckets) return;
    const uint32_t o = sort_bucket_offset(b, n_buckets, fine_bits, coarse_off, coarse_blocks, tile_base, fine_off);
    offsets[b] = o;
    hist[b] = b < n_buckets ? sort_bucket_offset(b + 1, n_buckets, fine_bits, coarse_off, coarse_blocks, tile_base, fine_off) - o : 0;
}

static __global__ void digit_hist_kernel(const uint8_t* __restrict__ scalars, const uint32_t* __restrict__ list,
                                         const uint32_t* __restrict__ count_ptr, uint32_t count_fixed, Digits D, uint32_t* hist) {
    const uint32_t count = count_ptr ? *count_ptr : count_fixed;
    for (uint32_t t = blockIdx.x * blockDim.x + threadIdx.x; t < count; t += gridDim.x * blockDim.x) {
        const uint32_t idx = list ? list[t] : t;
        Fr s = load_scalar(scalars, idx);
        for_each_digit(s, D, [&](int j, uint32_t b, bool) { atomicAdd(&hist[(uint32_t)j * D.window_bucket_stride + b], 1u); });
    }
}
static __global__ void digit_scatter_kernel(const uint8_t* __restrict__ scalars, const uint32_t* __restrict__ list,
                                            const uint32_t* __restrict__ count_ptr, uint32_t count_fixed, Digits D,
                                            const uint32_t* __restrict__ offsets, uint32_t* cursor, uint32_t* entries) {
    const uint32_t count = count_ptr ? *count_ptr : count_fixed;
    for (uint32_t t = blockIdx.x * blockDim.x + threadIdx.x; t < count; t += gridDim.x * blockDim.x) {
        const uint32_t idx = list ? list[t] : t;
        Fr s = load_scalar(scalars, idx);
        for_each_digit(s, D, [&](int j, uint32_t b, bool neg) {
            const uint32_t bucket = (uint32_t)j * D.window_bucket_stride + b;
            const uint32_t pos = offsets[bucket] + atomicAdd(&cursor[bucket], 1u);
            entries[pos] = ((uint32_t)j * D.window_point_stride + idx) | (neg ? 0x80000000u : 0u);
        });
    }
}

template <class F>
__global__ void __launch_bounds__(256)
gather_points_kernel(const uint32_t* __restrict__ entries, const uint32_t* __restrict__ offsets, uint32_t n_buckets,
                     const uint8_t* __restrict__ points, Affine<F>* __restrict__ sorted) {
    const uint32_t total = offsets[n_buckets];
    for (uint32_t k = blockIdx.x * blockDim.x + threadIdx.x; k < total; k += gridDim.x * blockDim.x) {
        const uint32_t e = entries[k];
        Affine<F> p = Affine<F>::load(points + sizeof(Affine<F>) * (size_t)(e & 0x7fffffffu));
        if (e >> 31) p.y = p.y.neg();
        p.store(sorted + k);
    }
}

static const int SCAN_TILE = 2048;
static const uint32_t PASS_FANIN = 32;
__device__ __forceinline__ uint32_t scan_f(uint32_t v, uint32_t chunk, uint32_t levels = 0) {
    if (!chunk) return v;
    v = (v + chunk - 1) / chunk;
    for (uint32_t l = 0; l < levels; ++l) v = (v + PASS_FANIN - 1) / PASS_FANIN;
    return v;
}

static __global__ void __launch_bounds__(256) scan_tile_totals_kernel(const uint32_t* __restrict__ in, uint32_t n, uint32_t chunk, uint32_t levels, uint32_t* tile_sums) {
    __shared__ uint32_t red[256];
    const uint32_t base = blockIdx.x * SCAN_TILE;
    uint32_t local = 0;
    for (uint32_t i = threadIdx.x; i < SCAN_TILE; i += 256) if (base + i < n) local += scan_f(in[base + i], chunk, levels);
    red[threadIdx.x] = local;
    __syncthreads();
    for (uint32_t off = 128; off > 0; off >>= 1) { if (threadIdx.x < off) red[threadIdx.x] += red[threadIdx.x + off]; __syncthreads(); }
    if (threadIdx.x == 0) tile_sums[blockIdx.x] = red[0];
}
static __global__ void __launch_bounds__(1024) scan_small_kernel(uint32_t* data, uint32_t n, uint32_t* total_out) {
    __shared__ uint32_t sums[1024];
    const uint32_t tid = threadIdx.x;
    const uint32_t per = (n + 1023) / 1024;
    const uint32_t beg = min(n, tid * per), end = min(n, beg + per);
    uint32_t local = 0;
    for (uint32_t i = beg; i < end; ++i) local += data[i];
    sums[tid] = local;
    __syncthreads();
    for (uint32_t off = 1; off < 1024; off <<= 1) {
        uint32_t v = tid >= off ? sums[tid - off] : 0;
        __syncthreads();
        sums[tid] += v;
        __syncthreads();
    }
    uint32_t run = sums[tid] - local;
    for (uint32_t i = beg; i < end; ++i) { uint32_t v = data[i]; data[i] = run; run += v; }
    if (tid == 1023 && total_out) *total_out = sums[1023];
}
static __global__ void __launch_bounds__(256) scan_tile_apply_kernel(const uint32_t* __restrict__ in, uint32_t n, uint32_t chunk, uint32_t levels,
                                                              const uint32_t* __restrict__ tile_base, uint32_t* out) {
    __shared__ uint32_t sums[256];
    const uint32_t base = blockIdx.x * SCAN_TILE + threadIdx.x * 8;
    uint32_t v[8], local = 0;
#pragma unroll
    for (int k = 0; k < 8; ++k) { v[k] = (base + k < n) ? scan_f(in[base + k], chunk, levels) : 0; local += v[k]; }
    sums[threadIdx.x] = local;
    __syncthreads();
    for (uint32_t off = 1; off < 256; off <<= 1) {
        uint32_t x = threadIdx.x >= off ? sums[threadIdx.x - off] : 0;
        __syncthreads();
        sums[threadIdx.x] += x;
        __syncthreads();
    }
    uint32_t run = tile_base[blockIdx.x] + sums[threadIdx.x] - local;
#pragma unroll
    for (int k = 0; k < 8; ++k) { if (base + k < n) out[base + k] = run; run += v[k]; }
}
static void exclusive_scan(const uint32_t* in, uint32_t n, uint32_t chunk, uint32_t levels, uint32_t* out, uint32_t* tiles, cudaStream_t st) {
    const uint32_t n_tiles = (n + SCAN_TILE - 1) / SCAN_TILE;
    scan_tile_totals_kernel<<<n_tiles, 256, 0, st>>>(in, n, chunk, levels, tiles);
    scan_small_kernel<<<1, 1024, 0, st>>>(tiles, n_tiles, out + n);
    scan_tile_apply_kernel<<<n_tiles, 256, 0, st>>>(in, n, chunk, levels, tiles, out);
    ZKE_COUNT_LAUNCH(3);
}

struct DigitSort {
    uint32_t n_buckets, n_parts, coarse_tile, coarse_blocks, fine_blocks;
    int fine_bits = 0;
    size_t max_entries, coarse_cells, fine_cells;
    uint32_t *coarse, *coarse_off, *part_count, *tile_base, *fine, *fine_off, *tiles, *stage;
    uint16_t* stage_fine;
    DigitSort(uint32_t n, int n_windows, uint32_t n_buckets_, size_t max_entries_) : n_buckets(n_buckets_), max_entries(max_entries_) {
        while ((n_buckets - 1) >> fine_bits >= SORT_PARTS) ++fine_bits;
        n_parts = sort_parts(n_buckets, fine_bits);
        coarse_tile = SORT_STAGE / (uint32_t)n_windows;
        coarse_blocks = std::max(1u, (n + coarse_tile - 1) / coarse_tile);
        fine_blocks = (uint32_t)(max_entries / SORT_TILE + n_parts);
        coarse_cells = (size_t)n_parts * coarse_blocks;
        fine_cells = (size_t)fine_blocks << fine_bits;
    }
    template <class Take> void place(Take take) {
        coarse = (uint32_t*)take(4 * (coarse_cells + 1));
        coarse_off = (uint32_t*)take(4 * (coarse_cells + 1));
        part_count = (uint32_t*)take(4 * ((size_t)n_parts + 1));
        tile_base = (uint32_t*)take(4 * ((size_t)n_parts + 1));
        fine = (uint32_t*)take(4 * (fine_cells + 1));
        fine_off = (uint32_t*)take(4 * (fine_cells + 1));
        tiles = (uint32_t*)take(4 * (std::max(coarse_cells, fine_cells) / SCAN_TILE + 2));
        stage = (uint32_t*)take(4 * max_entries);
        stage_fine = (uint16_t*)take(2 * max_entries);
    }
    void run(const uint8_t* scalars, const uint32_t* list, const uint32_t* count_ptr, uint32_t count_fixed, const Digits& D,
             uint32_t* hist, uint32_t* offsets, uint32_t* entries, cudaStream_t st) const {
        sort_coarse_count_kernel<<<coarse_blocks, SORT_THREADS, 0, st>>>(scalars, list, count_ptr, count_fixed, D, fine_bits, n_parts, coarse_tile, coarse);
        exclusive_scan(coarse, (uint32_t)coarse_cells, 0, 0, coarse_off, tiles, st);
        sort_coarse_scatter_kernel<<<coarse_blocks, SORT_THREADS, 0, st>>>(scalars, list, count_ptr, count_fixed, D, fine_bits, n_parts, coarse_tile, coarse_off, stage, stage_fine);
        sort_part_count_kernel<<<(n_parts + 255) / 256, 256, 0, st>>>(coarse_off, coarse_blocks, n_parts, part_count);
        exclusive_scan(part_count, n_parts, SORT_TILE, 0, tile_base, tiles, st);
        sort_fine_count_kernel<<<fine_blocks, SORT_THREADS, 0, st>>>(coarse_off, coarse_blocks, tile_base, n_parts, fine_bits, stage_fine, fine);
        exclusive_scan(fine, (uint32_t)fine_cells, 0, 0, fine_off, tiles, st);
        cudaFuncSetAttribute(sort_fine_scatter_kernel, cudaFuncAttributeMaxDynamicSharedMemorySize, (int)SORT_FINE_SMEM);
        sort_fine_scatter_kernel<<<fine_blocks, SORT_FINE_THREADS, SORT_FINE_SMEM, st>>>(coarse_off, coarse_blocks, tile_base, n_parts, fine_bits, stage, stage_fine, fine_off, entries);
        sort_offsets_kernel<<<(n_buckets + 256) / 256, 256, 0, st>>>(n_buckets, fine_bits, coarse_off, coarse_blocks, tile_base, fine_off, hist, offsets);
        ZKE_COUNT_LAUNCH(6);
    }
};

static __global__ void fill_work_kernel(const uint32_t* __restrict__ hist, const uint32_t* __restrict__ chunk_off, uint32_t n_buckets,
                                 uint32_t CHUNK, uint32_t levels, uint32_t* work_bucket) {
    const uint32_t b = blockIdx.x * blockDim.x + threadIdx.x;
    if (b >= n_buckets) return;
    const uint32_t nch = scan_f(hist[b], CHUNK, levels);
    for (uint32_t i = 0; i < nch; ++i) work_bucket[chunk_off[b] + i] = b;
}

static const int ORDER_BLOCK = 256;
__device__ __forceinline__ uint32_t chunk_size_of(uint32_t w, const uint32_t* hist, const uint32_t* chunk_off, const uint32_t* work_bucket, uint32_t CHUNK) {
    const uint32_t b = work_bucket[w];
    return min(CHUNK, hist[b] - (w - chunk_off[b]) * CHUNK);
}
static __global__ void __launch_bounds__(ORDER_BLOCK)
chunk_key_hist_kernel(const uint32_t* __restrict__ hist, const uint32_t* __restrict__ chunk_off, const uint32_t* __restrict__ work_bucket,
                      uint32_t n_buckets, uint32_t CHUNK, uint32_t* mat) {
    extern __shared__ uint32_t s_hist[];
    const uint32_t total = chunk_off[n_buckets];
    for (uint32_t i = threadIdx.x; i < CHUNK; i += ORDER_BLOCK) s_hist[i] = 0;
    __syncthreads();
    const uint32_t w = blockIdx.x * ORDER_BLOCK + threadIdx.x;
    if (w < total) atomicAdd(&s_hist[CHUNK - chunk_size_of(w, hist, chunk_off, work_bucket, CHUNK)], 1u);
    __syncthreads();
    for (uint32_t i = threadIdx.x; i < CHUNK; i += ORDER_BLOCK) mat[(size_t)i * gridDim.x + blockIdx.x] = s_hist[i];
}
static __global__ void __launch_bounds__(ORDER_BLOCK)
chunk_order_kernel(const uint32_t* __restrict__ hist, const uint32_t* __restrict__ chunk_off, const uint32_t* __restrict__ work_bucket,
                   uint32_t n_buckets, uint32_t CHUNK, const uint32_t* __restrict__ mat_off, uint32_t* order) {
    __shared__ uint32_t s_key[ORDER_BLOCK];
    const uint32_t total = chunk_off[n_buckets];
    const uint32_t w = blockIdx.x * ORDER_BLOCK + threadIdx.x;
    const uint32_t key = w < total ? CHUNK - chunk_size_of(w, hist, chunk_off, work_bucket, CHUNK) : 0xffffffffu;
    s_key[threadIdx.x] = key;
    __syncthreads();
    if (w >= total) return;
    uint32_t local = 0;
    for (uint32_t j = 0; j < threadIdx.x; ++j) local += s_key[j] == key;
    order[mat_off[(size_t)key * gridDim.x + blockIdx.x] + local] = w;
}

template <class F, int MINB>
__global__ void __launch_bounds__(128, MINB)
chunk_sum_kernel(const uint8_t* __restrict__ points, const uint32_t* __restrict__ entries, const uint32_t* __restrict__ offsets,
                 const uint32_t* __restrict__ hist, const uint32_t* __restrict__ chunk_off, const uint32_t* __restrict__ work_bucket,
                 const uint32_t* __restrict__ order, uint32_t n_buckets, uint32_t CHUNK, uint8_t* partial) {
    const uint32_t total = chunk_off[n_buckets];
    for (uint32_t t = blockIdx.x * blockDim.x + threadIdx.x; t < total; t += gridDim.x * blockDim.x) {
        const uint32_t w = order[t];
        const uint32_t b = work_bucket[w];
        const uint32_t ci = w - chunk_off[b];
        const uint32_t beg = offsets[b] + ci * CHUNK;
        const uint32_t end = min(offsets[b] + hist[b], beg + CHUNK);
        XYZZ<F> acc = XYZZ<F>::inf();
        for (uint32_t k = beg; k < end; ++k) {
            const uint32_t e = entries[k];
            acc.madd(Affine<F>::load(points + sizeof(Affine<F>) * (size_t)(e & 0x7fffffffu)), (e >> 31) != 0);
        }
        acc.store(partial + sizeof(XYZZ<F>) * (size_t)w);
    }
}

template <class F>
__global__ void __launch_bounds__(128)
partial_pass_kernel(const uint8_t* __restrict__ in, const uint32_t* __restrict__ hist, const uint32_t* __restrict__ off_in,
                    const uint32_t* __restrict__ off_out, const uint32_t* __restrict__ work_bucket, uint32_t n_buckets,
                    uint32_t CHUNK, uint32_t level, uint8_t* out) {
    const uint32_t total = off_out[n_buckets];
    for (uint32_t w = blockIdx.x * blockDim.x + threadIdx.x; w < total; w += gridDim.x * blockDim.x) {
        const uint32_t b = work_bucket[w];
        const uint32_t i = w - off_out[b];
        const uint32_t n_in = scan_f(hist[b], CHUNK, level);
        const uint32_t beg = off_in[b] + i * PASS_FANIN, end = min(off_in[b] + n_in, beg + PASS_FANIN);
        XYZZ<F> acc = XYZZ<F>::inf();
        for (uint32_t k = beg; k < end; ++k) acc.add(XYZZ<F>::load(in + sizeof(XYZZ<F>) * (size_t)k));
        acc.store(out + sizeof(XYZZ<F>) * (size_t)w);
    }
}

template <class F, int ITEMS>
__global__ void __launch_bounds__(128)
group_sum_kernel(const uint8_t* __restrict__ partial, const uint32_t* __restrict__ hist, const uint32_t* __restrict__ chunk_off,
                 uint32_t half, uint32_t n_groups_total, uint32_t CHUNK, uint32_t levels, uint32_t GROUP, uint8_t* group_out) {
    const uint32_t g = blockIdx.x * blockDim.x + threadIdx.x;
    if (g >= n_groups_total) return;
    const uint32_t groups_per_window = (half + GROUP - 1) / GROUP;
    const uint32_t window = g / groups_per_window, gi = g % groups_per_window;
    const uint32_t lo = gi * GROUP, hi = min(half, lo + GROUP);
    XYZZ<F> running = XYZZ<F>::inf(), total = XYZZ<F>::inf();
    for (uint32_t b = hi; b-- > lo;) {
        const uint32_t bucket = window * half + b;
        if (ITEMS == 1) {
            if (hist[bucket]) running.add(XYZZ<F>::load(partial + sizeof(XYZZ<F>) * (size_t)bucket));
        } else {
            const uint32_t nch = scan_f(hist[bucket], CHUNK, levels);
            for (uint32_t i = 0; i < nch; ++i) running.add(XYZZ<F>::load(partial + sizeof(XYZZ<F>) * (size_t)(chunk_off[bucket] + i)));
        }
        total.add(running);
    }
    if (lo && !running.is_inf()) {
        XYZZ<F> acc = XYZZ<F>::inf();
        for (int bit = 31 - __clz(lo); bit >= 0; --bit) {
            acc.dbl();
            if ((lo >> bit) & 1) acc.add(running);
        }
        total.add(acc);
    }
    total.store(group_out + sizeof(XYZZ<F>) * (size_t)g);
}

template <class F>
__global__ void __launch_bounds__(512)
window_reduce_kernel(uint8_t* group_out, uint32_t groups_per_window) {
    uint8_t* base = group_out + sizeof(XYZZ<F>) * (size_t)blockIdx.x * groups_per_window;
    uint32_t n = groups_per_window;
    while (n > 1) {
        const uint32_t halfn = (n + 1) / 2;
        for (uint32_t t = threadIdx.x; t + halfn < n; t += blockDim.x) {
            XYZZ<F> a = XYZZ<F>::load(base + sizeof(XYZZ<F>) * (size_t)t);
            a.add(XYZZ<F>::load(base + sizeof(XYZZ<F>) * (size_t)(t + halfn)));
            a.store(base + sizeof(XYZZ<F>) * (size_t)t);
        }
        __syncthreads();
        n = halfn;
    }
}

template <class F>
__global__ void gather_windows_kernel(const uint8_t* __restrict__ group_out, uint32_t groups_per_window, uint32_t n_windows, uint8_t* out) {
    const uint32_t j = blockIdx.x * blockDim.x + threadIdx.x;
    if (j >= n_windows) return;
    XYZZ<F>::load(group_out + sizeof(XYZZ<F>) * (size_t)j * groups_per_window).store(out + sizeof(XYZZ<F>) * (size_t)j);
}

template <class F>
__global__ void __launch_bounds__(128)
bucket_finish_kernel(const Affine<F>* __restrict__ pts, const uint32_t* __restrict__ hist, const uint32_t* __restrict__ off,
                     uint32_t n_buckets, uint32_t level, XYZZ<F>* __restrict__ out) {
    const uint32_t b = blockIdx.x * blockDim.x + threadIdx.x;
    if (b >= n_buckets) return;
    const uint32_t n = ba_level_count(hist[b], level);
    if (n == 0) return;
    const Affine<F>* p = pts + off[b];
    XYZZ<F> acc = XYZZ<F>::from_affine(Affine<F>::load(p));
    Affine<F> nxt = n > 1 ? Affine<F>::load(p + 1) : Affine<F>::load(p);
    for (uint32_t i = 1; i < n; ++i) {
        const Affine<F> cur = nxt;
        if (i + 1 < n) nxt = Affine<F>::load(p + i + 1);
        acc.madd(cur, false);
    }
    acc.store(out + b);
}

template <class F>
static void run_ba(const MsmConfig& cfg, const uint32_t* hist, const uint32_t* offsets,
                   uint32_t n_buckets, size_t max_entries, uint32_t* tiles, uint8_t* ws, const Digits& D, uint32_t groups, uint8_t* group_out,
                   cudaStream_t st, cudaEvent_t* ev, const typename MsmPlan<F>::Heavy* heavy) {
    const int L = cfg.ba_levels;
    const size_t s1 = BaPlan<F>::slots_bound(max_entries, n_buckets, 1), s2 = BaPlan<F>::slots_bound(max_entries, n_buckets, 2);
    const size_t t1 = (s1 + BA_K - 1) / BA_K;
    uint8_t* p = ws;
    auto take = [&](size_t x) { uint8_t* r = p; p += (x + 255) & ~(size_t)255; return r; };
    Affine<F>* sorted0 = (Affine<F>*)take(sizeof(Affine<F>) * (max_entries + 1));
    F* prefix = (F*)take(sizeof(F) * s1);
    Affine<F>* ping = (Affine<F>*)take(sizeof(Affine<F>) * s1);
    Affine<F>* pong = (Affine<F>*)take(sizeof(Affine<F>) * s2);
    uint32_t* slot_bucket = (uint32_t*)take(4 * s1);
    F* tot = (F*)take(sizeof(F) * t1);
    F* binv_scratch = (F*)take(sizeof(F) * binv_scratch_elems(t1));
    const uint32_t* off[8];
    off[0] = offsets;
    for (int l = 1; l <= L; ++l) {
        uint32_t* o = (uint32_t*)take(4 * ((size_t)n_buckets + 1));
        exclusive_scan(hist, n_buckets, 1u << l, 0, o, tiles, st);
        off[l] = o;
    }
    cudaStream_t hv = (heavy && heavy->st != st) ? heavy->st : st;
    auto to_heavy = [&]() { if (hv != st) { cudaEventRecord(heavy->before, st); cudaStreamWaitEvent(hv, heavy->before, 0); } };
    auto to_light = [&]() { if (hv != st) { cudaEventRecord(heavy->after, hv); cudaStreamWaitEvent(st, heavy->after, 0); } };
    const Affine<F>* in = sorted0;
    Affine<F>* out = ping;
    for (int l = 0; l < L; ++l) {
        const size_t slots = BaPlan<F>::slots_bound(max_entries, n_buckets, l + 1);
        const uint32_t n_threads = (uint32_t)((slots + BA_K - 1) / BA_K);
        const uint32_t blocks = (n_threads + BA_THREADS - 1) / BA_THREADS;
        fill_work_kernel<<<(n_buckets + 255) / 256, 256, 0, st>>>(hist, off[l + 1], n_buckets, 1u << (l + 1), 0, slot_bucket);
        BaLevel lv{hist, off[l], off[l + 1], slot_bucket, n_buckets, (uint32_t)l};
        to_heavy();
        if (ev && l == 0) cudaEventRecord(ev[0], hv);
        ba_forward_kernel<F><<<blocks, BA_THREADS, 0, hv>>>(lv, in, prefix, tot, n_threads);
        to_light();
        batch_inverse<F>(tot, n_threads, binv_scratch, st);
        to_heavy();
        ba_backward_kernel<F><<<blocks, BA_THREADS, 0, hv>>>(lv, in, prefix, tot, out, n_threads);
        if (ev && l == L - 1) cudaEventRecord(ev[1], hv);
        to_light();
        ZKE_COUNT_LAUNCH(3);
        in = out;
        out = (out == ping) ? pong : ping;
    }
    XYZZ<F>* bucket_sum = (XYZZ<F>*)sorted0;
    bucket_finish_kernel<F><<<(n_buckets + 127) / 128, 128, 0, st>>>(in, hist, off[L], n_buckets, (uint32_t)L, bucket_sum);
    group_sum_kernel<F, 1><<<(groups + 127) / 128, 128, 0, st>>>((const uint8_t*)bucket_sum, hist, off[L], D.half, groups, 1u << L, 0, D.group, group_out);
    ZKE_COUNT_LAUNCH(2);
}
template <>
void run_ba<Fq2>(const MsmConfig&, const uint32_t*, const uint32_t*, uint32_t, size_t, uint32_t*, uint8_t*, const Digits&,
                 uint32_t, uint8_t*, cudaStream_t, cudaEvent_t*, const MsmPlan<Fq2>::Heavy*) {}

#if defined(ZKE_MSM_G1)
MsmConfig msm_config_witness() {
    MsmConfig c; c.c = 8; c.chunk = 32; c.group = 8; c.classify = true; c.extra_passes = 2;
    if (const char* e = getenv("ZKE_W_C")) c.c = std::max(4, std::min(16, atoi(e)));
    if (const char* e = getenv("ZKE_W_CHUNK")) c.chunk = (uint32_t)std::max(8, atoi(e));
    if (const char* e = getenv("ZKE_W_GROUP")) c.group = (uint32_t)std::max(2, atoi(e));
    return c;
}
MsmConfig msm_config_full(uint32_t n, bool precomputed) {
    MsmConfig c;
    c.c = n >= (1u << 18) ? 16 : (n >= (1u << 12) ? 12 : 8);
    c.chunk = 256; c.group = n >= (1u << 20) ? 64 : 16; c.classify = false; c.extra_passes = 0;
    c.precomputed = precomputed;
    c.ba_levels = 0;
    if (const char* e = getenv("ZKE_H_BA")) c.ba_levels = precomputed ? std::max(0, std::min(6, atoi(e))) : 0;
    if (const char* e = getenv("ZKE_H_GROUP")) c.group = (uint32_t)std::max(2, atoi(e));
    if (precomputed) {
        c.c = n >= (1u << 20) ? 20 : (n >= (1u << 16) ? 17 : (n >= (1u << 10) ? 12 : 8));
    }
    return c;
}
#endif

template <class F>
size_t MsmPlan<F>::workspace_bytes(uint32_t n, const MsmConfig& cfg) {
    const int W = (255 + cfg.c - 1) / cfg.c;
    const size_t half = (size_t)1 << (cfg.c - 1);
    const size_t bucket_sets = cfg.precomputed ? 1 : W;
    const size_t n_buckets = half * bucket_sets;
    const size_t max_entries = (size_t)n * W;
    const size_t max_chunks = n_buckets + max_entries / cfg.chunk + 1;
    const size_t groups = ((half + cfg.group - 1) / cfg.group) * bucket_sets;
    size_t b = 0;
    auto al = [&](size_t x) { b += (x + 255) & ~(size_t)255; };
    al(4 * 2);
    al(4 * (size_t)n);
    al(4 * (size_t)n);
    al(4 * (n_buckets + 1));
    al(4 * (n_buckets + 1));
    al(4 * (n_buckets + 1));
    al(4 * (n_buckets / SCAN_TILE + 2));
    al(4 * max_entries);
    al(4 * max_chunks);
    al(sizeof(XYZZ<F>) * max_chunks);
    al(sizeof(XYZZ<F>) * (max_chunks / PASS_FANIN + n_buckets + 1));
    al(4 * (n_buckets + 1));
    al(sizeof(XYZZ<F>) * groups);
    al(sizeof(XYZZ<F>) * ((size_t)n / LIST_FANIN + 2));
    al(sizeof(XYZZ<F>) * ((size_t)n / LIST_FANIN + 2));
    if (cfg.ba_levels > 0 && sizeof(F) == 32) al(BaPlan<F>::bytes(max_entries, n_buckets, cfg.ba_levels));
    const size_t order_cells = ((max_chunks + ORDER_BLOCK - 1) / ORDER_BLOCK) * cfg.chunk;
    al(4 * max_chunks);
    al(4 * (order_cells + 1));
    al(4 * (order_cells + 1));
    al(4 * (order_cells / SCAN_TILE + 2));
    if (n_buckets >= SORT_TWO_LEVEL_MIN_BUCKETS) DigitSort((uint32_t)n, W, (uint32_t)n_buckets, max_entries).place([&](size_t x) { al(x); return (uint8_t*)nullptr; });
    else al(4 * (n_buckets + 1));
    return b;
}

template <class F>
void MsmPlan<F>::run(const uint8_t* points, const uint8_t* scalars, uint32_t n, const MsmConfig& cfg, uint8_t* ws,
                     uint8_t* result, cudaStream_t st, cudaEvent_t* ev, const Heavy* heavy) {
    Digits D;
    D.c = cfg.c;
    D.n_windows = (255 + cfg.c - 1) / cfg.c;
    D.half = 1u << (cfg.c - 1);
    D.chunk = cfg.chunk;
    D.group = cfg.group;
    D.window_bucket_stride = cfg.precomputed ? 0 : D.half;
    D.window_point_stride = cfg.precomputed ? n : 0;
    if (D.n_windows > MSM_MAX_WINDOWS) return;
    const uint32_t bucket_sets = cfg.precomputed ? 1 : (uint32_t)D.n_windows;
    const uint32_t n_buckets = D.half * bucket_sets;
    const size_t max_entries = (size_t)n * D.n_windows;
    const size_t max_chunks = n_buckets + max_entries / cfg.chunk + 1;
    const uint32_t groups_per_window = (D.half + D.group - 1) / D.group;
    const uint32_t groups = groups_per_window * bucket_sets;
    uint8_t* p = ws;
    auto take = [&](size_t x) { uint8_t* r = p; p += (x + 255) & ~(size_t)255; return r; };
    uint32_t* counters = (uint32_t*)take(8);
    uint32_t* ones_list = (uint32_t*)take(4 * (size_t)n);
    uint32_t* gen_list = (uint32_t*)take(4 * (size_t)n);
    uint32_t* hist = (uint32_t*)take(4 * ((size_t)n_buckets + 1));
    uint32_t* offsets = (uint32_t*)take(4 * ((size_t)n_buckets + 1));
    uint32_t* chunk_off = (uint32_t*)take(4 * ((size_t)n_buckets + 1));
    uint32_t* tiles = (uint32_t*)take(4 * ((size_t)n_buckets / SCAN_TILE + 2));
    uint32_t* entries = (uint32_t*)take(4 * max_entries);
    uint32_t* work_bucket = (uint32_t*)take(4 * max_chunks);
    uint8_t* partial = take(sizeof(XYZZ<F>) * max_chunks);
    uint8_t* partial2 = take(sizeof(XYZZ<F>) * (max_chunks / PASS_FANIN + n_buckets + 1));
    uint32_t* off2 = (uint32_t*)take(4 * ((size_t)n_buckets + 1));
    uint8_t* group_out = take(sizeof(XYZZ<F>) * groups);
    const size_t list_slots = (size_t)n / LIST_FANIN + 2;
    uint8_t* red_a = take(sizeof(XYZZ<F>) * list_slots);
    uint8_t* red_b = take(sizeof(XYZZ<F>) * list_slots);
    const bool use_ba = cfg.ba_levels > 0 && sizeof(F) == 32;
    uint8_t* ba_ws = use_ba ? take(BaPlan<F>::bytes(max_entries, n_buckets, cfg.ba_levels)) : nullptr;
    const size_t order_cells = ((max_chunks + ORDER_BLOCK - 1) / ORDER_BLOCK) * cfg.chunk;
    uint32_t* order = (uint32_t*)take(4 * max_chunks);
    uint32_t* order_mat = (uint32_t*)take(4 * (order_cells + 1));
    uint32_t* order_off = (uint32_t*)take(4 * (order_cells + 1));
    uint32_t* order_tiles = (uint32_t*)take(4 * (order_cells / SCAN_TILE + 2));
    const bool two_level = n_buckets >= SORT_TWO_LEVEL_MIN_BUCKETS;
    DigitSort sort(n, D.n_windows, n_buckets, max_entries);
    if (sort.fine_bits > SORT_MAX_FINE_BITS) throw std::runtime_error("MSM bucket sort: more than 2^19 buckets");
    uint32_t* cursor = nullptr;
    if (two_level) sort.place(take);
    else cursor = (uint32_t*)take(4 * ((size_t)n_buckets + 1));

    uint8_t* res_ones = result;
    uint8_t* res_windows = result + sizeof(XYZZ<F>) * MSM_ONES_SLOTS;
    cudaMemsetAsync(result, 0, sizeof(XYZZ<F>) * MSM_RESULT_SLOTS, st);

    const uint32_t* gen_count = nullptr;
    const uint32_t* gen_idx = nullptr;
    if (cfg.classify) {
        cudaMemsetAsync(counters, 0, 8, st);
        classify_kernel<F><<<(n + 255) / 256, 256, 0, st>>>(points, scalars, n, ones_list, gen_list, counters);
        uint32_t upper = (n + LIST_FANIN - 1) / LIST_FANIN;
        sum_affine_list_kernel<F><<<(upper + 127) / 128, 128, 0, st>>>(points, ones_list, counters, 0, red_a);
        ZKE_COUNT_LAUNCH(2);
        uint8_t *src = red_a, *dst = red_b;
        uint32_t level = 0;
        for (;;) {
            const uint32_t next = (upper + TREE_FANIN - 1) / TREE_FANIN;
            const bool last = next <= MSM_ONES_SLOTS;
            uint8_t* out = last ? res_ones : dst;
            const uint32_t threads = last ? (uint32_t)MSM_ONES_SLOTS : next;
            sum_xyzz_kernel<F><<<(threads + 63) / 64, 64, 0, st>>>(src, counters, 0, level, last ? MSM_ONES_SLOTS : 0, out);
            ZKE_COUNT_LAUNCH(1);
            if (last) break;
            uint8_t* t = src; src = dst; dst = t;
            upper = next;
            ++level;
        }
        gen_count = counters + 1;
        gen_idx = gen_list;
    }
    const int sms = sm_count();
    if (two_level) {
        sort.run(scalars, gen_idx, gen_count, n, D, hist, offsets, entries, st);
    } else {
        cudaMemsetAsync(hist, 0, 4 * ((size_t)n_buckets + 1), st);
        cudaMemsetAsync(cursor, 0, 4 * ((size_t)n_buckets + 1), st);
        digit_hist_kernel<<<sms * 8, 256, 0, st>>>(scalars, gen_idx, gen_count, n, D, hist);
        exclusive_scan(hist, n_buckets, 0, 0, offsets, tiles, st);
        digit_scatter_kernel<<<sms * 8, 256, 0, st>>>(scalars, gen_idx, gen_count, n, D, offsets, cursor, entries);
        ZKE_COUNT_LAUNCH(2);
    }
    if (use_ba) {
        gather_points_kernel<F><<<sms * 8, 256, 0, st>>>(entries, offsets, n_buckets, points, (Affine<F>*)ba_ws);
        ZKE_COUNT_LAUNCH(1);
        run_ba<F>(cfg, hist, offsets, n_buckets, max_entries, tiles, ba_ws, D, groups, group_out, st, ev, heavy);
    } else {
        exclusive_scan(hist, n_buckets, D.chunk, 0, chunk_off, tiles, st);
        fill_work_kernel<<<(n_buckets + 255) / 256, 256, 0, st>>>(hist, chunk_off, n_buckets, D.chunk, 0, work_bucket);
        {
            const uint32_t nblk = (uint32_t)((max_chunks + ORDER_BLOCK - 1) / ORDER_BLOCK);
            chunk_key_hist_kernel<<<nblk, ORDER_BLOCK, 4 * D.chunk, st>>>(hist, chunk_off, work_bucket, n_buckets, D.chunk, order_mat);
            exclusive_scan(order_mat, nblk * D.chunk, 0, 0, order_off, order_tiles, st);
            chunk_order_kernel<<<nblk, ORDER_BLOCK, 0, st>>>(hist, chunk_off, work_bucket, n_buckets, D.chunk, order_off, order);
            ZKE_COUNT_LAUNCH(2);
        }
        cudaStream_t st_light = st;
        if (heavy && heavy->st != st) {
            cudaEventRecord(heavy->before, st);
            cudaStreamWaitEvent(heavy->st, heavy->before, 0);
            st = heavy->st;
        }
        if (ev) cudaEventRecord(ev[0], st);
        {
            int minb = sizeof(F) == 32 ? 5 : 4, waves = 4;
            if (const char* e = getenv("ZKE_CHUNK_MINB")) minb = atoi(e);
            if (const char* e = getenv("ZKE_CHUNK_WAVES")) waves = std::max(1, atoi(e));
            bool done = false;
#if defined(ZKE_MSM_G1)
            const char* h_tc_env = getenv("ZKE_H_TC");
            const int h_tc = h_tc_env ? atoi(h_tc_env) : 0;
            if (h_tc > 0 && cfg.precomputed) {
                if (const TcTable* tab = tc_table_fq()) {
                    const uint8_t* pts = reinterpret_cast<const uint8_t*>(points);
                    if (h_tc >= 5) chunk_sum_tc_kernel<5><<<sms * 5 * waves, 128, 0, st>>>(pts, entries, offsets, hist, chunk_off, work_bucket, order, n_buckets, D.chunk, partial, tab);
                    else if (h_tc == 4) chunk_sum_tc_kernel<4><<<sms * 4 * waves, 128, 0, st>>>(pts, entries, offsets, hist, chunk_off, work_bucket, order, n_buckets, D.chunk, partial, tab);
                    else chunk_sum_tc_kernel<3><<<sms * 3 * waves, 128, 0, st>>>(pts, entries, offsets, hist, chunk_off, work_bucket, order, n_buckets, D.chunk, partial, tab);
                    done = true;
                }
            }
#endif
            size_t pad = 0;
            if (const char* e = getenv("ZKE_CHUNK_PAD_SMEM")) pad = (size_t)std::max(0, std::min(48 * 1024, atoi(e)));
            if (done) {}
            else if (minb >= 6) chunk_sum_kernel<F, 6><<<sms * 6 * waves, 128, pad, st>>>(points, entries, offsets, hist, chunk_off, work_bucket, order, n_buckets, D.chunk, partial);
            else if (minb == 5) chunk_sum_kernel<F, 5><<<sms * 5 * waves, 128, pad, st>>>(points, entries, offsets, hist, chunk_off, work_bucket, order, n_buckets, D.chunk, partial);
            else chunk_sum_kernel<F, 4><<<sms * 4 * waves, 128, pad, st>>>(points, entries, offsets, hist, chunk_off, work_bucket, order, n_buckets, D.chunk, partial);
        }
        if (ev) cudaEventRecord(ev[1], st);
        if (st != st_light) {
            cudaEventRecord(heavy->after, st);
            cudaStreamWaitEvent(st_light, heavy->after, 0);
            st = st_light;
        }
        uint8_t *items = partial, *items_next = partial2;
        uint32_t *off_cur = chunk_off, *off_next = off2;
        uint32_t levels = 0;
        for (uint32_t pass = 0; pass < cfg.extra_passes; ++pass) {
            exclusive_scan(hist, n_buckets, D.chunk, levels + 1, off_next, tiles, st);
            fill_work_kernel<<<(n_buckets + 255) / 256, 256, 0, st>>>(hist, off_next, n_buckets, D.chunk, levels + 1, work_bucket);
            partial_pass_kernel<F><<<sms * 4, 128, 0, st>>>(items, hist, off_cur, off_next, work_bucket, n_buckets, D.chunk, levels, items_next);
            ZKE_COUNT_LAUNCH(2);
            uint8_t* t = items; items = items_next; items_next = t;
            uint32_t* o = off_cur; off_cur = off_next; off_next = o;
            ++levels;
        }
        group_sum_kernel<F, 0><<<(groups + 127) / 128, 128, 0, st>>>(items, hist, off_cur, D.half, groups, D.chunk, levels, D.group, group_out);
    }
    window_reduce_kernel<F><<<bucket_sets, 512, 0, st>>>(group_out, groups_per_window);
    gather_windows_kernel<F><<<1, 64, 0, st>>>(group_out, groups_per_window, bucket_sets, res_windows);
    ZKE_COUNT_LAUNCH(5);
}

#if defined(ZKE_MSM_G1)
template struct MsmPlan<Fq>;
#elif defined(ZKE_MSM_G2)
template struct MsmPlan<Fq2>;
#else
#error "compile msm.cu through msm_g1.cu / msm_g2.cu"
#endif

}
}
```

### zk-email-verify_b200/csrc/msm.cuh

```cuda
#pragma once
#include "ec.cuh"

namespace zke {
namespace dev {

struct MsmConfig {
    int c = 16;
    uint32_t chunk = 256;
    uint32_t group = 16;
    bool classify = false;
    uint32_t extra_passes = 0;
    bool precomputed = false;
    int ba_levels = 0;
};
MsmConfig msm_config_witness();
MsmConfig msm_config_full(uint32_t n, bool precomputed);
inline int msm_windows(const MsmConfig& c) { return (255 + c.c - 1) / c.c; }

static const int MSM_ONES_SLOTS = 32;
static const int MSM_MAX_WINDOWS = 32;
static const int MSM_RESULT_SLOTS = MSM_ONES_SLOTS + MSM_MAX_WINDOWS;

template <class F>
struct MsmPlan {
    static size_t workspace_bytes(uint32_t n, const MsmConfig& cfg);
    struct Heavy { cudaStream_t st; cudaEvent_t before, after; };
    static void run(const uint8_t* points, const uint8_t* scalars, uint32_t n, const MsmConfig& cfg, uint8_t* workspace,
                    uint8_t* result, cudaStream_t st, cudaEvent_t* ev = nullptr, const Heavy* heavy = nullptr);
};

}
}
```

### zk-email-verify_b200/host/zkemail_b200/_lib.py

```python
from __future__ import annotations
import ctypes
import os

_HERE = os.path.dirname(os.path.abspath(__file__))
LIB_PATH = os.environ.get(
    "ZKEMAIL_B200_LIB", os.path.normpath(os.path.join(_HERE, "..", "..", "lib", "libzkemail_b200.so"))
)
if not os.path.exists(LIB_PATH):
    raise ImportError(
        f"{LIB_PATH} not found - build it first (python -c 'import __graft_entry__ as g; g.build()' "
        "or make -C zk-email-verify_b200/csrc); there is no fallback implementation"
    )
lib = ctypes.CDLL(LIB_PATH)

c_void_p, c_char_p, c_size_t = ctypes.c_void_p, ctypes.c_char_p, ctypes.c_size_t
c_u32, c_u64, c_i64, c_int = ctypes.c_uint32, ctypes.c_uint64, ctypes.c_int64, ctypes.c_int
ERRCAP = 4096


class CircuitInfo(ctypes.Structure):
    _fields_ = [(n, c_u32) for n in (
        "n_vars", "n_temps", "n_outputs", "n_pub_inputs", "n_prv_inputs", "n_public", "n_constraints",
        "n_levels", "n_ops", "n_coefs", "domain_log2", "n_groups")] + [(n, c_u64) for n in ("nnz_a", "nnz_b", "nnz_c")]


class ProgramStats(ctypes.Structure):
    _fields_ = [(n, c_u32) for n in ("n_levels", "n_iters", "n_ops_kept", "n_coop_ops", "n_terms", "cluster")] + [("digest", c_u64)]


def _sig(name, restype, argtypes):
    fn = getattr(lib, name)
    fn.restype = restype
    fn.argtypes = argtypes
    return fn


zke_circuit_build = _sig("zke_circuit_build", c_void_p, [c_char_p, ctypes.POINTER(c_i64), c_size_t, c_char_p, c_size_t])
zke_circuit_free = _sig("zke_circuit_free", None, [c_void_p])
zke_circuit_build_app = _sig("zke_circuit_build_app", c_void_p, [c_char_p, c_char_p, c_size_t])
zke_circuit_from_r1cs = _sig("zke_circuit_from_r1cs", c_void_p, [c_void_p, c_size_t, c_char_p, c_size_t])
zke_circuit_write_r1cs = _sig("zke_circuit_write_r1cs", c_i64, [c_void_p, c_void_p, c_size_t])
zke_circuit_get_info = _sig("zke_circuit_get_info", c_int, [c_void_p, ctypes.POINTER(CircuitInfo)])
zke_circuit_group = _sig("zke_circuit_group", c_int, [c_void_p, c_u32, c_char_p, c_size_t, ctypes.POINTER(c_u32),
                                                       ctypes.POINTER(c_u32), ctypes.POINTER(c_int)])
zke_circuit_input_offset = _sig("zke_circuit_input_offset", c_i64, [c_void_p, c_char_p, ctypes.POINTER(c_u32)])
zke_circuit_array = _sig("zke_circuit_array", c_void_p, [c_void_p, c_int, ctypes.POINTER(c_size_t)])
zke_circuit_scope_name = _sig("zke_circuit_scope_name", c_char_p, [c_void_p, c_u32])
zke_circuit_program_stats = _sig("zke_circuit_program_stats", c_int, [c_void_p, c_int, c_int, c_int, c_u32, ctypes.POINTER(ProgramStats),
                                                                      ctypes.POINTER(c_u32), c_size_t, c_char_p, c_size_t])
zke_circuit_program_stats_ex = _sig("zke_circuit_program_stats_ex", c_int, [c_void_p, c_u32, c_u32, ctypes.POINTER(ProgramStats),
                                                                            ctypes.POINTER(c_u32), c_size_t, c_char_p, c_size_t])
LOWER_NATIVE_SHA, LOWER_NATIVE_REGEX, LOWER_COOP_FPMUL, LOWER_NATIVE_POSEIDON = 1, 2, 4, 8
zke_poseidon_hash = _sig("zke_poseidon_hash", c_int, [c_char_p, c_size_t, c_char_p])
zke_poseidon_batch = _sig("zke_poseidon_batch", c_int, [c_char_p, c_u32, c_size_t, c_int, c_void_p, c_char_p, c_size_t])
zke_pubkey_hashes = _sig("zke_pubkey_hashes", c_int, [c_char_p, c_size_t, c_u32, c_u32, c_u32, c_int, c_void_p, c_char_p, c_size_t])
zke_domain_key_leaves = _sig("zke_domain_key_leaves", c_int, [c_char_p, c_size_t, c_u32, c_u32, c_u32, c_char_p, c_int, c_void_p,
                                                               c_char_p, c_size_t])
zke_merkle_build = _sig("zke_merkle_build", c_i64, [c_char_p, c_size_t, c_u32, c_int, c_void_p, c_size_t, c_char_p, c_size_t])
zke_registry_open = _sig("zke_registry_open", c_void_p, [c_char_p, c_size_t, c_u32, c_int, c_char_p, c_size_t])
zke_registry_update = _sig("zke_registry_update", c_int, [c_void_p, c_void_p, c_char_p, c_size_t, c_char_p, c_size_t])
zke_registry_nodes = _sig("zke_registry_nodes", c_int, [c_void_p, c_void_p, c_void_p, c_size_t, c_void_p, c_char_p, c_size_t])
zke_registry_levels = _sig("zke_registry_levels", c_i64, [c_void_p, c_void_p, c_size_t, c_char_p, c_size_t])
zke_registry_count = _sig("zke_registry_count", c_u64, [c_void_p])
zke_registry_close = _sig("zke_registry_close", None, [c_void_p])
zke_registry_device_ms = _sig("zke_registry_device_ms", ctypes.c_double, [])
zke_device_count = _sig("zke_device_count", c_int, [])
zke_version = _sig("zke_version", c_char_p, [])

(ARR_COEFS, ARR_A_PTR, ARR_A_VAR, ARR_A_COEF, ARR_B_PTR, ARR_B_VAR, ARR_B_COEF, ARR_C_PTR, ARR_C_VAR, ARR_C_COEF,
 ARR_OPS, ARR_LEVEL_PTR, ARR_LC_PTR, ARR_LC_VAR, ARR_LC_COEF, ARR_AUX, ARR_SCOPE_OF_CONSTRAINT) = range(17)
ARR_SHA_BLOCKS = 17
ARR_REGEX_SEEDS = 18
ARR_POSEIDON_BLOCKS = 19


class ZkeError(RuntimeError):
    pass

c_u8p = ctypes.POINTER(ctypes.c_uint8)
c_i32p = ctypes.POINTER(ctypes.c_int32)
zke_setup = _sig("zke_setup", c_void_p, [c_void_p, c_u64, c_int, c_char_p, c_size_t])
zke_zkey_free = _sig("zke_zkey_free", None, [c_void_p])
zke_zkey_load = _sig("zke_zkey_load", c_void_p, [c_void_p, c_size_t, c_int, c_char_p, c_size_t])
zke_zkey_load_chunks = _sig("zke_zkey_load_chunks", c_void_p, [ctypes.POINTER(c_void_p), ctypes.POINTER(c_size_t), c_size_t, c_int, c_char_p, c_size_t])
zke_zkey_write = _sig("zke_zkey_write", c_i64, [c_void_p, c_void_p, c_void_p, c_size_t])
zke_zkey_is_toy = _sig("zke_zkey_is_toy", c_int, [c_void_p])
zke_circuit_build_regex = _sig("zke_circuit_build_regex", c_void_p, [ctypes.POINTER(c_char_p), c_char_p, c_size_t, c_u32, c_char_p, c_size_t])
zke_fullprove_submit = _sig("zke_fullprove_submit", c_int, [c_void_p, c_void_p, c_size_t, c_void_p, c_char_p, c_size_t])
zke_fullprove_collect = _sig("zke_fullprove_collect", c_int, [c_void_p, c_void_p, c_void_p, c_void_p, c_char_p, c_size_t])
zke_wtns_prove = _sig("zke_wtns_prove", c_int, [c_void_p, c_void_p, c_size_t, c_void_p, c_void_p, c_void_p, c_char_p, c_size_t])
zke_pairing_alphabeta = _sig("zke_pairing_alphabeta", c_int, [c_void_p, c_void_p, c_void_p])
zke_zkey_info = _sig("zke_zkey_info", c_int, [c_void_p, ctypes.POINTER(c_u32), ctypes.POINTER(c_u32), ctypes.POINTER(c_u32)])
zke_zkey_section = _sig("zke_zkey_section", c_i64, [c_void_p, c_int, c_void_p, c_size_t])
zke_ctx_open = _sig("zke_ctx_open", c_void_p, [c_void_p, c_void_p, c_int, c_u32, c_char_p, c_size_t])
zke_ctx_close = _sig("zke_ctx_close", None, [c_void_p])
zke_ctx_stream = _sig("zke_ctx_stream", c_void_p, [c_void_p])
zke_kernel_launches = _sig("zke_kernel_launches", c_u64, [])
zke_witness = _sig("zke_witness", c_int, [c_void_p, c_void_p, c_size_t, c_void_p, c_void_p, c_char_p, c_size_t])
zke_load_witness = _sig("zke_load_witness", c_int, [c_void_p, c_void_p, c_size_t, c_char_p, c_size_t])
zke_check_witness = _sig("zke_check_witness", c_int, [c_void_p, c_size_t, c_void_p, c_char_p, c_size_t])
zke_prove = _sig("zke_prove", c_int, [c_void_p, c_size_t, c_void_p, c_void_p, c_void_p, c_void_p, c_char_p, c_size_t])
zke_fullprove = _sig("zke_fullprove", c_int, [c_void_p, c_void_p, c_size_t, c_void_p, c_void_p, c_void_p, c_void_p, c_char_p, c_size_t])
zke_verify_json = _sig("zke_verify_json", c_int, [c_char_p, c_char_p, c_char_p, c_char_p, c_size_t])
zke_verify_batch_json = _sig("zke_verify_batch_json", c_int, [c_char_p, c_char_p, c_char_p, c_void_p, c_void_p, c_char_p, c_size_t])
zke_verifier_open = _sig("zke_verifier_open", c_void_p, [c_char_p, c_int, c_char_p, c_size_t])
zke_verifier_close = _sig("zke_verifier_close", None, [c_void_p])
zke_verifier_batch = _sig("zke_verifier_batch", c_int, [c_void_p, c_size_t, c_void_p, c_void_p, c_void_p, c_void_p, c_char_p, c_size_t])
zke_selftest_pairing_gpu = _sig("zke_selftest_pairing_gpu", c_int, [c_int, c_size_t, c_void_p, c_void_p, c_void_p, c_char_p, c_size_t])
zke_zkey_vkey_json = _sig("zke_zkey_vkey_json", c_int, [c_void_p, c_char_p, ctypes.POINTER(c_size_t)])
zke_proof_to_json = _sig("zke_proof_to_json", c_int, [c_void_p, c_void_p, c_u32, c_char_p, ctypes.POINTER(c_size_t), c_char_p, ctypes.POINTER(c_size_t)])
zke_pack_inputs_json = _sig("zke_pack_inputs_json", c_int, [c_void_p, c_char_p, c_void_p, c_size_t, c_char_p, c_size_t])
zke_fullprove_json = _sig("zke_fullprove_json", c_int, [c_void_p, c_void_p, c_char_p, c_char_p, ctypes.POINTER(c_size_t), c_char_p,
                                                        ctypes.POINTER(c_size_t), c_char_p, c_size_t])
zke_upload_inputs = _sig("zke_upload_inputs", c_int, [c_void_p, c_void_p, c_size_t, c_char_p, c_size_t])
zke_ctx_set_lanes = _sig("zke_ctx_set_lanes", c_int, [c_void_p, c_int])
zke_ctx_profile = _sig("zke_ctx_profile", c_int, [c_void_p, c_int])
zke_ctx_profile_get = _sig("zke_ctx_profile_get", c_int, [c_void_p, ctypes.POINTER(ctypes.c_double), ctypes.POINTER(c_u64)])
STAGES = ("witness", "matvec", "ntt", "msm_a", "msm_b1", "msm_c", "msm_h", "msm_h_buckets", "msm_b2")
zke_setup_toxic = _sig("zke_setup_toxic", c_int, [c_u64, c_void_p])
zke_zkey_from_ptau = _sig("zke_zkey_from_ptau", c_void_p, [c_void_p, c_void_p, c_size_t, c_int, c_char_p, c_size_t])
zke_ptau_info = _sig("zke_ptau_info", c_int, [c_void_p, c_void_p, c_size_t, ctypes.POINTER(c_u32), ctypes.POINTER(c_u64),
                                              ctypes.POINTER(c_u64), c_char_p, c_size_t])
zke_zkey_from_ptau_timing = _sig("zke_zkey_from_ptau_timing", c_int, [ctypes.POINTER(ctypes.c_double), ctypes.POINTER(ctypes.c_double)])
zke_zkey_contribute = _sig("zke_zkey_contribute", c_void_p, [c_void_p, c_void_p, c_char_p, c_size_t])
zke_zkey_check_contribution = _sig("zke_zkey_check_contribution", c_int, [c_void_p, c_void_p, c_void_p, c_char_p, c_size_t])
zke_ptau_toy = _sig("zke_ptau_toy", c_i64, [c_u32, c_void_p, c_int, c_void_p, c_size_t, c_char_p, c_size_t])
zke_ptau_new = _sig("zke_ptau_new", c_i64, [c_u32, c_void_p, c_size_t, c_char_p, c_size_t])
zke_ptau_contribute = _sig("zke_ptau_contribute", c_i64, [c_void_p, c_size_t, c_void_p, c_int, c_void_p, c_size_t, c_void_p, c_char_p, c_size_t])
zke_ptau_prepare = _sig("zke_ptau_prepare", c_i64, [c_void_p, c_size_t, c_int, c_void_p, c_size_t, c_char_p, c_size_t])
zke_ptau_prepare_timing = _sig("zke_ptau_prepare_timing", c_int, [ctypes.POINTER(ctypes.c_double), ctypes.POINTER(ctypes.c_double)])
zke_ptau_verify = _sig("zke_ptau_verify", c_int, [c_void_p, c_size_t, c_void_p, c_size_t, c_void_p, c_void_p, c_int, c_char_p, c_size_t])
zke_agg_srs_from_ptau = _sig("zke_agg_srs_from_ptau", c_void_p, [c_void_p, c_size_t, c_void_p, c_size_t, c_u32, c_int, c_char_p, c_size_t])
zke_agg_srs_free = _sig("zke_agg_srs_free", None, [c_void_p])
zke_agg_srs_n_max = _sig("zke_agg_srs_n_max", c_u32, [c_void_p])
zke_agg_vk_json = _sig("zke_agg_vk_json", c_int, [c_void_p, c_char_p, ctypes.POINTER(c_size_t)])
zke_agg_bytes = _sig("zke_agg_bytes", c_size_t, [c_size_t])
zke_aggregate = _sig("zke_aggregate", c_i64, [c_void_p, c_char_p, c_size_t, c_void_p, c_void_p, c_void_p, c_size_t, c_char_p, c_size_t])
zke_agg_verify = _sig("zke_agg_verify", c_int, [c_char_p, c_char_p, c_size_t, c_void_p, c_void_p, c_size_t, c_char_p, c_size_t])
zke_selftest_fpmul_hint =_sig("zke_selftest_fpmul_hint", c_int, [c_u32, c_u32, c_void_p, c_void_p, c_void_p, c_void_p, c_void_p])

(SEC_ALPHA1, SEC_BETA1, SEC_DELTA1, SEC_BETA2, SEC_GAMMA2, SEC_DELTA2) = (101, 102, 103, 104, 105, 106)
(SEC_IC, SEC_A, SEC_B1, SEC_B2, SEC_C, SEC_H) = (3, 5, 6, 7, 8, 9)

SHARD_PARTIAL_BYTES = 388
zke_shard_begin = _sig("zke_shard_begin", c_int, [c_void_p, c_int, c_int, c_char_p, c_size_t])
zke_shard_vector = _sig("zke_shard_vector", c_void_p, [c_void_p, c_int, ctypes.POINTER(c_size_t)])
zke_shard_mid = _sig("zke_shard_mid", c_int, [c_void_p, c_char_p, c_size_t])
zke_shard_end = _sig("zke_shard_end", c_int, [c_void_p, c_void_p, c_void_p, c_char_p, c_size_t])
zke_shard_combine = _sig("zke_shard_combine", c_int, [c_void_p, c_void_p, c_int, c_void_p, c_void_p, ctypes.POINTER(ctypes.c_int32), c_char_p, c_size_t])
zke_shard_combine_raw = _sig("zke_shard_combine_raw", c_int, [c_void_p, c_void_p, c_int, c_void_p, c_void_p, ctypes.POINTER(ctypes.c_int32), c_char_p, c_size_t])
```

Before: 47.75.

## Batch witness MSMs across proofs with grid-y member dimension on dedicated stream

Witness MSMs (A, B1, C, B2) now run for groups of up to 8 proofs at once. Each kernel gets a blockIdx.y member index with per-member workspace and scalar/result strides, and the work is issued on a separate group stream instead of once per proof inside each lane. Lanes keep the H MSM and wait on a group-done event before copying results back. This cuts per-proof kernel launches and fills the GPU better for the smaller witness MSMs, at the cost of a large shared workspace (g × member_ws), less memory left for lanes, and a serialization point on one group stream.

```diff
diff --git a/include/zkemail_b200.h b/include/zkemail_b200.h
--- a/include/zkemail_b200.h
+++ b/include/zkemail_b200.h
@@ -146,6 +146,7 @@
     ZKE_N_STAGES = 9
 };
 int zke_ctx_set_lanes(zke_ctx* x, int n);
+int zke_ctx_set_msm_group(zke_ctx* x, int g);
 int zke_ctx_profile(zke_ctx* x, int enable);
 int zke_ctx_profile_get(const zke_ctx* x, double* ms_out, uint64_t* count_out);
 
diff --git a/zk-email-verify_b200/csrc/engine.cu b/zk-email-verify_b200/csrc/engine.cu
--- a/zk-email-verify_b200/csrc/engine.cu
+++ b/zk-email-verify_b200/csrc/engine.cu
@@ -131,6 +131,10 @@
     int n_lanes = 1, lanes_alloc = 0;
     int finish_threads = 4;
     dev::MsmConfig cfg_w, cfg_h;
+    cudaStream_t group_st = nullptr;
+    DevBuf group_ws;
+    int msm_group = 1, msm_group_alloc = 0;
+    std::vector<cudaEvent_t> group_done;
     bool split_streams = true;
     std::vector<uint32_t> bad_host;
     bool profile = false;
@@ -641,9 +645,10 @@
     const uint32_t max_batch = x->max_batch;
     x->cfg_w = dev::msm_config_witness();
     x->cfg_h = x->zkey->cfg_h;
-    size_t ws = std::max(dev::MsmPlan<dev::Fq>::workspace_bytes(x->n_vars, x->cfg_w),
-                         dev::MsmPlan<dev::Fq>::workspace_bytes((uint32_t)N, x->cfg_h));
-    ws = std::max(ws, dev::MsmPlan<dev::Fq2>::workspace_bytes(x->n_vars, x->cfg_w));
+    const size_t ws = dev::MsmPlan<dev::Fq>::workspace_bytes((uint32_t)N, x->cfg_h);
+    const size_t member_ws = std::max(dev::MsmPlan<dev::Fq>::workspace_bytes(x->n_vars, x->cfg_w),
+                                      dev::MsmPlan<dev::Fq2>::workspace_bytes(x->n_vars, x->cfg_w));
+    const size_t keep_slot = x->stride * 32 * max_batch + ((size_t)1 << 30);
     int want = 8;
     if (const char* e = getenv("ZKE_LANES")) want = atoi(e);
     if (const char* e = getenv("ZKE_SPLIT_STREAMS")) x->split_streams = atoi(e) != 0;
@@ -653,7 +658,7 @@
         size_t free_b = 0, total_b = 0;
         CUDA_OK(cudaMemGetInfo(&free_b, &total_b));
         const size_t lane_bytes = 4 * N * 32 + ws;
-        const size_t keep = x->stride * 32 * max_batch + ((size_t)1 << 30);
+        const size_t keep = keep_slot + member_ws;
         const size_t fit = free_b > keep ? (free_b - keep) / lane_bytes : 0;
         want = std::max(1, std::min<int>(want, (int)std::min<size_t>(fit, ZKE_MAX_LANES)));
     }
@@ -667,6 +672,18 @@
         L.msm_ws.alloc(ws);
     }
     x->lanes_alloc = x->n_lanes = want;
+    size_t g = std::min<size_t>(8, max_batch);
+    {
+        size_t free_b = 0, total_b = 0;
+        CUDA_OK(cudaMemGetInfo(&free_b, &total_b));
+        const size_t fit = free_b > keep_slot ? (free_b - keep_slot) / member_ws : 0;
+        g = std::max<size_t>(1, std::min(g, fit));
+    }
+    CUDA_OK(cudaStreamCreateWithPriority(&x->group_st, cudaStreamNonBlocking, prio_light));
+    x->group_ws.alloc(g * member_ws);
+    x->group_done.resize(max_batch);
+    for (auto& e : x->group_done) CUDA_OK(cudaEventCreateWithFlags(&e, cudaEventDisableTiming));
+    x->msm_group_alloc = x->msm_group = (int)g;
 }
 
 static zke_ctx* do_open(const zke_circuit* zc, const zke_zkey* zk, int device, uint32_t max_batch) {
@@ -791,17 +808,22 @@
 }
 
 template <class Queued>
-static void enqueue_witness_msms(const zke_ctx* x, const uint8_t* w, uint32_t lo, uint32_t hi, uint8_t* ws, uint8_t* res,
+static void enqueue_witness_msms(const zke_ctx* x, const zke_ctx::Slot& S, uint32_t first, uint32_t members, uint32_t lo, uint32_t hi,
                                  cudaStream_t st, Queued queued) {
+    if (members < 1 || (int)members > x->msm_group_alloc) throw std::runtime_error("witness MSM group larger than its workspace");
     const zke_zkey* zk = x->zkey;
-    w += 32ull * lo;
-    dev::MsmPlan<dev::Fq>::run(zk->A.p + 64ull * lo, w, hi - lo, x->cfg_w, ws, res + RES_A * ZKE_RES_G1_BLOCK, st);
+    const size_t w_stride = 32 * x->stride;
+    const uint8_t* w = S.w_all.p + w_stride * first + 32ull * lo;
+    uint8_t* res = S.results.p + (size_t)ZKE_RESULT_STRIDE * first;
+    uint8_t* ws = x->group_ws.p;
+    const dev::MsmGroup g{members, w_stride, ZKE_RESULT_STRIDE};
+    dev::MsmPlan<dev::Fq>::run(zk->A.p + 64ull * lo, w, hi - lo, x->cfg_w, ws, res + RES_A * ZKE_RES_G1_BLOCK, st, nullptr, nullptr, g);
     queued(ZKE_STAGE_MSM_A);
-    dev::MsmPlan<dev::Fq>::run(zk->B1.p + 64ull * lo, w, hi - lo, x->cfg_w, ws, res + RES_B1 * ZKE_RES_G1_BLOCK, st);
+    dev::MsmPlan<dev::Fq>::run(zk->B1.p + 64ull * lo, w, hi - lo, x->cfg_w, ws, res + RES_B1 * ZKE_RES_G1_BLOCK, st, nullptr, nullptr, g);
     queued(ZKE_STAGE_MSM_B1);
-    dev::MsmPlan<dev::Fq>::run(zk->C.p + 64ull * lo, w, hi - lo, x->cfg_w, ws, res + RES_C * ZKE_RES_G1_BLOCK, st);
+    dev::MsmPlan<dev::Fq>::run(zk->C.p + 64ull * lo, w, hi - lo, x->cfg_w, ws, res + RES_C * ZKE_RES_G1_BLOCK, st, nullptr, nullptr, g);
     queued(ZKE_STAGE_MSM_C);
-    dev::MsmPlan<dev::Fq2>::run(zk->B2.p + 128ull * lo, w, hi - lo, x->cfg_w, ws, res + RES_B2 * ZKE_RES_G1_BLOCK, st);
+    dev::MsmPlan<dev::Fq2>::run(zk->B2.p + 128ull * lo, w, hi - lo, x->cfg_w, ws, res + RES_B2 * ZKE_RES_G1_BLOCK, st, nullptr, nullptr, g);
     CHECK_LAUNCH();
     queued(ZKE_STAGE_MSM_B2);
 }
@@ -831,6 +853,7 @@
 
 static void sync_lanes(zke_ctx* x) {
     cudaStreamSynchronize(x->stream);
+    if (x->group_st) cudaStreamSynchronize(x->group_st);
     for (int i = 0; i < x->lanes_alloc; ++i) { cudaStreamSynchronize(x->lanes[i].st); cudaStreamSynchronize(x->lanes[i].heavy); }
 }
 
@@ -855,6 +878,14 @@
     if (const char* e = getenv("ZKE_SPLIT_STREAMS")) x->split_streams = atoi(e) != 0;
     if (l) CUDA_OK(cudaMemcpy2DAsync(S.publics_host, (size_t)l * 32, S.w_all.p + 32, x->stride * 32, (size_t)l * 32, batch, cudaMemcpyDeviceToHost, x->stream));
     CUDA_OK(cudaEventRecord(S.witness_done, x->stream));
+    const uint32_t G = prof ? 1 : (uint32_t)x->msm_group;
+    if (!prof) {
+        CUDA_OK(cudaStreamWaitEvent(x->group_st, S.witness_done, 0));
+        for (uint32_t e0 = 0, k = 0; e0 < batch; e0 += G, ++k) {
+            enqueue_witness_msms(x, S, e0, std::min<uint32_t>(G, (uint32_t)batch - e0), 0, m, x->group_st, [](int) {});
+            CUDA_OK(cudaEventRecord(x->group_done[k], x->group_st));
+        }
+    }
     for (int i = 0; i < n_lanes; ++i) CUDA_OK(cudaStreamWaitEvent(x->lanes[i].st, S.witness_done, 0));
     for (size_t e = 0; e < batch; ++e) {
         zke_ctx::Lane& L = x->lanes[e % n_lanes];
@@ -880,7 +911,7 @@
         CHECK_LAUNCH();
         if (hv != st) CUDA_OK(cudaEventRecord(L.ev[1], hv));
         span(ZKE_STAGE_NTT);
-        enqueue_witness_msms(x, w, 0, m, L.msm_ws.p, res, st, span);
+        if (prof) enqueue_witness_msms(x, S, (uint32_t)e, 1, 0, m, st, span);
         if (hv != st) CUDA_OK(cudaStreamWaitEvent(st, L.ev[1], 0));
         const dev::MsmPlan<dev::Fq>::Heavy heavy{hv, L.ev[2], L.ev[3]};
         size_t i0 = 0, i1 = 0;
@@ -889,6 +920,7 @@
         if (prof) x->spans.push_back({ZKE_STAGE_MSM_H_BUCKETS, i0, i1});
         span(ZKE_STAGE_MSM_H);
         CHECK_LAUNCH();
+        if (!prof) CUDA_OK(cudaStreamWaitEvent(st, x->group_done[e / G], 0));
         CUDA_OK(cudaMemcpyAsync(S.results_host + (size_t)ZKE_RESULT_STRIDE * e, res, ZKE_RESULT_STRIDE, cudaMemcpyDeviceToHost, st));
         CUDA_OK(cudaEventRecord(S.done[e], st));
     }
@@ -1086,7 +1118,7 @@
     CHECK_LAUNCH();
     const uint32_t lo = (uint32_t)((uint64_t)m * x->shard_rank / G), hi = (uint32_t)((uint64_t)m * (x->shard_rank + 1) / G);
     uint8_t* res = S.results.p;
-    enqueue_witness_msms(x, S.w_all.p, lo, hi, L.msm_ws.p, res, st, [](int) {});
+    enqueue_witness_msms(x, S, 0, 1, lo, hi, st, [](int) {});
     dev::MsmPlan<dev::Fq>::run(zk->H.p, L.vd.p, N, x->cfg_h, L.msm_ws.p, res + RES_H * ZKE_RES_G1_BLOCK, st);
     CHECK_LAUNCH();
     CUDA_OK(cudaMemcpyAsync(S.results_host, res, ZKE_RESULT_STRIDE, cudaMemcpyDeviceToHost, st));
@@ -1227,6 +1259,8 @@
         if (x->lanes[i].heavy) cudaStreamDestroy(x->lanes[i].heavy);
         for (auto e : x->lanes[i].ev) if (e) cudaEventDestroy(e);
     }
+    for (auto e : x->group_done) cudaEventDestroy(e);
+    if (x->group_st) cudaStreamDestroy(x->group_st);
     if (x->stream) cudaStreamDestroy(x->stream);
     delete x;
 }
@@ -1249,6 +1283,11 @@
     if (!x || n < 1) return -1;
     x->n_lanes = n > x->lanes_alloc ? x->lanes_alloc : n;
     return x->n_lanes;
+}
+int zke_ctx_set_msm_group(zke_ctx* x, int g) {
+    if (!x || g < 1) return -1;
+    x->msm_group = g > x->msm_group_alloc ? x->msm_group_alloc : g;
+    return x->msm_group;
 }
 int zke_ctx_profile(zke_ctx* x, int enable) {
     if (!x) return -1;
diff --git a/zk-email-verify_b200/csrc/msm.cu b/zk-email-verify_b200/csrc/msm.cu
--- a/zk-email-verify_b200/csrc/msm.cu
+++ b/zk-email-verify_b200/csrc/msm.cu
@@ -17,11 +17,19 @@
 
 __device__ __forceinline__ Fr load_scalar(const uint8_t* scalars, uint32_t i) { return Fr::load(scalars + 32ull * i); }
 
+template <class T>
+__device__ __forceinline__ T* member(T* p, size_t stride) {
+    return p ? reinterpret_cast<T*>(reinterpret_cast<uintptr_t>(p) + blockIdx.y * stride) : p;
+}
+
 template <class F>
 __global__ void classify_kernel(const uint8_t* __restrict__ points, const uint8_t* __restrict__ scalars, uint32_t n,
-                                uint32_t* ones_list, uint32_t* gen_list, uint32_t* counters ) {
+                                uint32_t* ones_list, uint32_t* gen_list, uint32_t* counters ,
+                                size_t ws, size_t scalar_stride) {
     const uint32_t i = blockIdx.x * blockDim.x + threadIdx.x;
     if (i >= n) return;
+    scalars = member(scalars, scalar_stride);
+    ones_list = member(ones_list, ws); gen_list = member(gen_list, ws); counters = member(counters, ws);
     Fr s = load_scalar(scalars, i);
     if (s.is_zero()) return;
     Affine<F> p = Affine<F>::load(points + sizeof(Affine<F>) * (size_t)i);
@@ -33,7 +41,8 @@
 
 template <class F>
 __global__ void sum_affine_list_kernel(const uint8_t* __restrict__ points, const uint32_t* __restrict__ list,
-                                       const uint32_t* __restrict__ count_ptr, uint32_t count_fixed, uint8_t* out) {
+                                       const uint32_t* __restrict__ count_ptr, uint32_t count_fixed, uint8_t* out, size_t ws) {
+    list = member(list, ws); count_ptr = member(count_ptr, ws); out = member(out, ws);
     const uint32_t count = count_ptr ? *count_ptr : count_fixed;
     const uint32_t t = blockIdx.x * blockDim.x + threadIdx.x;
     const uint32_t n_out = max(1u, (count + LIST_FANIN - 1) / LIST_FANIN);
@@ -53,7 +62,8 @@
 }
 template <class F>
 __global__ void sum_xyzz_kernel(const uint8_t* __restrict__ in, const uint32_t* __restrict__ count_ptr, uint32_t count_fixed,
-                                uint32_t level, uint32_t pad_to, uint8_t* out) {
+                                uint32_t level, uint32_t pad_to, uint8_t* out, size_t ws, size_t out_stride) {
+    in = member(in, ws); count_ptr = member(count_ptr, ws); out = member(out, out_stride);
     const uint32_t count = count_ptr ? *count_ptr : count_fixed;
     const uint32_t n_in = tree_level_size(count, level), n_out = tree_level_size(count, level + 1);
     const uint32_t t = blockIdx.x * blockDim.x + threadIdx.x;
@@ -271,7 +281,10 @@
 }
 
 static __global__ void digit_hist_kernel(const uint8_t* __restrict__ scalars, const uint32_t* __restrict__ list,
-                                         const uint32_t* __restrict__ count_ptr, uint32_t count_fixed, Digits D, uint32_t* hist) {
+                                         const uint32_t* __restrict__ count_ptr, uint32_t count_fixed, Digits D, uint32_t* hist,
+                                         size_t ws, size_t scalar_stride) {
+    scalars = member(scalars, scalar_stride);
+    list = member(list, ws); count_ptr = member(count_ptr, ws); hist = member(hist, ws);
     const uint32_t count = count_ptr ? *count_ptr : count_fixed;
     for (uint32_t t = blockIdx.x * blockDim.x + threadIdx.x; t < count; t += gridDim.x * blockDim.x) {
         const uint32_t idx = list ? list[t] : t;
@@ -281,7 +294,11 @@
 }
 static __global__ void digit_scatter_kernel(const uint8_t* __restrict__ scalars, const uint32_t* __restrict__ list,
                                             const uint32_t* __restrict__ count_ptr, uint32_t count_fixed, Digits D,
-                                            const uint32_t* __restrict__ offsets, uint32_t* cursor, uint32_t* entries) {
+                                            const uint32_t* __restrict__ offsets, uint32_t* cursor, uint32_t* entries,
+                                            size_t ws, size_t scalar_stride) {
+    scalars = member(scalars, scalar_stride);
+    list = member(list, ws); count_ptr = member(count_ptr, ws);
+    offsets = member(offsets, ws); cursor = member(cursor, ws); entries = member(entries, ws);
     const uint32_t count = count_ptr ? *count_ptr : count_fixed;
     for (uint32_t t = blockIdx.x * blockDim.x + threadIdx.x; t < count; t += gridDim.x * blockDim.x) {
         const uint32_t idx = list ? list[t] : t;
@@ -316,8 +333,10 @@
     return v;
 }
 
-static __global__ void __launch_bounds__(256) scan_tile_totals_kernel(const uint32_t* __restrict__ in, uint32_t n, uint32_t chunk, uint32_t levels, uint32_t* tile_sums) {
+static __global__ void __launch_bounds__(256) scan_tile_totals_kernel(const uint32_t* __restrict__ in, uint32_t n, uint32_t chunk, uint32_t levels, uint32_t* tile_sums,
+                                                                      size_t ws) {
     __shared__ uint32_t red[256];
+    in = member(in, ws); tile_sums = member(tile_sums, ws);
     const uint32_t base = blockIdx.x * SCAN_TILE;
     uint32_t local = 0;
     for (uint32_t i = threadIdx.x; i < SCAN_TILE; i += 256) if (base + i < n) local += scan_f(in[base + i], chunk, levels);
@@ -326,8 +345,9 @@
     for (uint32_t off = 128; off > 0; off >>= 1) { if (threadIdx.x < off) red[threadIdx.x] += red[threadIdx.x + off]; __syncthreads(); }
     if (threadIdx.x == 0) tile_sums[blockIdx.x] = red[0];
 }
-static __global__ void __launch_bounds__(1024) scan_small_kernel(uint32_t* data, uint32_t n, uint32_t* total_out) {
+static __global__ void __launch_bounds__(1024) scan_small_kernel(uint32_t* data, uint32_t n, uint32_t* total_out, size_t ws) {
     __shared__ uint32_t sums[1024];
+    data = member(data, ws); total_out = member(total_out, ws);
     const uint32_t tid = threadIdx.x;
     const uint32_t per = (n + 1023) / 1024;
     const uint32_t beg = min(n, tid * per), end = min(n, beg + per);
@@ -346,8 +366,9 @@
     if (tid == 1023 && total_out) *total_out = sums[1023];
 }
 static __global__ void __launch_bounds__(256) scan_tile_apply_kernel(const uint32_t* __restrict__ in, uint32_t n, uint32_t chunk, uint32_t levels,
-                                                              const uint32_t* __restrict__ tile_base, uint32_t* out) {
+                                                              const uint32_t* __restrict__ tile_base, uint32_t* out, size_t ws) {
     __shared__ uint32_t sums[256];
+    in = member(in, ws); tile_base = member(tile_base, ws); out = member(out, ws);
     const uint32_t base = blockIdx.x * SCAN_TILE + threadIdx.x * 8;
     uint32_t v[8], local = 0;
 #pragma unroll
@@ -364,11 +385,12 @@
 #pragma unroll
     for (int k = 0; k < 8; ++k) { if (base + k < n) out[base + k] = run; run += v[k]; }
 }
-static void exclusive_scan(const uint32_t* in, uint32_t n, uint32_t chunk, uint32_t levels, uint32_t* out, uint32_t* tiles, cudaStream_t st) {
+static void exclusive_scan(const uint32_t* in, uint32_t n, uint32_t chunk, uint32_t levels, uint32_t* out, uint32_t* tiles, cudaStream_t st,
+                           uint32_t members = 1, size_t ws = 0) {
     const uint32_t n_tiles = (n + SCAN_TILE - 1) / SCAN_TILE;
-    scan_tile_totals_kernel<<<n_tiles, 256, 0, st>>>(in, n, chunk, levels, tiles);
-    scan_small_kernel<<<1, 1024, 0, st>>>(tiles, n_tiles, out + n);
-    scan_tile_apply_kernel<<<n_tiles, 256, 0, st>>>(in, n, chunk, levels, tiles, out);
+    scan_tile_totals_kernel<<<dim3(n_tiles, members), 256, 0, st>>>(in, n, chunk, levels, tiles, ws);
+    scan_small_kernel<<<dim3(1, members), 1024, 0, st>>>(tiles, n_tiles, out + n, ws);
+    scan_tile_apply_kernel<<<dim3(n_tiles, members), 256, 0, st>>>(in, n, chunk, levels, tiles, out, ws);
     ZKE_COUNT_LAUNCH(3);
 }
 
@@ -415,9 +437,10 @@
 };
 
 static __global__ void fill_work_kernel(const uint32_t* __restrict__ hist, const uint32_t* __restrict__ chunk_off, uint32_t n_buckets,
-                                 uint32_t CHUNK, uint32_t levels, uint32_t* work_bucket) {
+                                 uint32_t CHUNK, uint32_t levels, uint32_t* work_bucket, size_t ws) {
     const uint32_t b = blockIdx.x * blockDim.x + threadIdx.x;
     if (b >= n_buckets) return;
+    hist = member(hist, ws); chunk_off = member(chunk_off, ws); work_bucket = member(work_bucket, ws);
     const uint32_t nch = scan_f(hist[b], CHUNK, levels);
     for (uint32_t i = 0; i < nch; ++i) work_bucket[chunk_off[b] + i] = b;
 }
@@ -429,8 +452,9 @@
 }
 static __global__ void __launch_bounds__(ORDER_BLOCK)
 chunk_key_hist_kernel(const uint32_t* __restrict__ hist, const uint32_t* __restrict__ chunk_off, const uint32_t* __restrict__ work_bucket,
-                      uint32_t n_buckets, uint32_t CHUNK, uint32_t* mat) {
+                      uint32_t n_buckets, uint32_t CHUNK, uint32_t* mat, size_t ws) {
     extern __shared__ uint32_t s_hist[];
+    hist = member(hist, ws); chunk_off = member(chunk_off, ws); work_bucket = member(work_bucket, ws); mat = member(mat, ws);
     const uint32_t total = chunk_off[n_buckets];
     for (uint32_t i = threadIdx.x; i < CHUNK; i += ORDER_BLOCK) s_hist[i] = 0;
     __syncthreads();
@@ -441,8 +465,10 @@
 }
 static __global__ void __launch_bounds__(ORDER_BLOCK)
 chunk_order_kernel(const uint32_t* __restrict__ hist, const uint32_t* __restrict__ chunk_off, const uint32_t* __restrict__ work_bucket,
-                   uint32_t n_buckets, uint32_t CHUNK, const uint32_t* __restrict__ mat_off, uint32_t* order) {
+                   uint32_t n_buckets, uint32_t CHUNK, const uint32_t* __restrict__ mat_off, uint32_t* order, size_t ws) {
     __shared__ uint32_t s_key[ORDER_BLOCK];
+    hist = member(hist, ws); chunk_off = member(chunk_off, ws); work_bucket = member(work_bucket, ws);
+    mat_off = member(mat_off, ws); order = member(order, ws);
     const uint32_t total = chunk_off[n_buckets];
     const uint32_t w = blockIdx.x * ORDER_BLOCK + threadIdx.x;
     const uint32_t key = w < total ? CHUNK - chunk_size_of(w, hist, chunk_off, work_bucket, CHUNK) : 0xffffffffu;
@@ -458,7 +484,9 @@
 __global__ void __launch_bounds__(128, MINB)
 chunk_sum_kernel(const uint8_t* __restrict__ points, const uint32_t* __restrict__ entries, const uint32_t* __restrict__ offsets,
                  const uint32_t* __restrict__ hist, const uint32_t* __restrict__ chunk_off, const uint32_t* __restrict__ work_bucket,
-                 const uint32_t* __restrict__ order, uint32_t n_buckets, uint32_t CHUNK, uint8_t* partial) {
+                 const uint32_t* __restrict__ order, uint32_t n_buckets, uint32_t CHUNK, uint8_t* partial, size_t ws) {
+    entries = member(entries, ws); offsets = member(offsets, ws); hist = member(hist, ws); chunk_off = member(chunk_off, ws);
+    work_bucket = member(work_bucket, ws); order = member(order, ws); partial = member(partial, ws);
     const uint32_t total = chunk_off[n_buckets];
     for (uint32_t t = blockIdx.x * blockDim.x + threadIdx.x; t < total; t += gridDim.x * blockDim.x) {
         const uint32_t w = order[t];
@@ -479,7 +507,9 @@
 __global__ void __launch_bounds__(128)
 partial_pass_kernel(const uint8_t* __restrict__ in, const uint32_t* __restrict__ hist, const uint32_t* __restrict__ off_in,
                     const uint32_t* __restrict__ off_out, const uint32_t* __restrict__ work_bucket, uint32_t n_buckets,
-                    uint32_t CHUNK, uint32_t level, uint8_t* out) {
+                    uint32_t CHUNK, uint32_t level, uint8_t* out, size_t ws) {
+    in = member(in, ws); hist = member(hist, ws); off_in = member(off_in, ws); off_out = member(off_out, ws);
+    work_bucket = member(work_bucket, ws); out = member(out, ws);
     const uint32_t total = off_out[n_buckets];
     for (uint32_t w = blockIdx.x * blockDim.x + threadIdx.x; w < total; w += gridDim.x * blockDim.x) {
         const uint32_t b = work_bucket[w];
@@ -495,9 +525,10 @@
 template <class F, int ITEMS>
 __global__ void __launch_bounds__(128)
 group_sum_kernel(const uint8_t* __restrict__ partial, const uint32_t* __restrict__ hist, const uint32_t* __restrict__ chunk_off,
-                 uint32_t half, uint32_t n_groups_total, uint32_t CHUNK, uint32_t levels, uint32_t GROUP, uint8_t* group_out) {
+                 uint32_t half, uint32_t n_groups_total, uint32_t CHUNK, uint32_t levels, uint32_t GROUP, uint8_t* group_out, size_t ws) {
     const uint32_t g = blockIdx.x * blockDim.x + threadIdx.x;
     if (g >= n_groups_total) return;
+    partial = member(partial, ws); hist = member(hist, ws); chunk_off = member(chunk_off, ws); group_out = member(group_out, ws);
     const uint32_t groups_per_window = (half + GROUP - 1) / GROUP;
     const uint32_t window = g / groups_per_window, gi = g % groups_per_window;
     const uint32_t lo = gi * GROUP, hi = min(half, lo + GROUP);
@@ -525,8 +556,8 @@
 
 template <class F>
 __global__ void __launch_bounds__(512)
-window_reduce_kernel(uint8_t* group_out, uint32_t groups_per_window) {
-    uint8_t* base = group_out + sizeof(XYZZ<F>) * (size_t)blockIdx.x * groups_per_window;
+window_reduce_kernel(uint8_t* group_out, uint32_t groups_per_window, size_t ws) {
+    uint8_t* base = member(group_out, ws) + sizeof(XYZZ<F>) * (size_t)blockIdx.x * groups_per_window;
     uint32_t n = groups_per_window;
     while (n > 1) {
         const uint32_t halfn = (n + 1) / 2;
@@ -541,9 +572,11 @@
 }
 
 template <class F>
-__global__ void gather_windows_kernel(const uint8_t* __restrict__ group_out, uint32_t groups_per_window, uint32_t n_windows, uint8_t* out) {
+__global__ void gather_windows_kernel(const uint8_t* __restrict__ group_out, uint32_t groups_per_window, uint32_t n_windows, uint8_t* out,
+                                      size_t ws, size_t out_stride) {
     const uint32_t j = blockIdx.x * blockDim.x + threadIdx.x;
     if (j >= n_windows) return;
+    group_out = member(group_out, ws); out = member(out, out_stride);
     XYZZ<F>::load(group_out + sizeof(XYZZ<F>) * (size_t)j * groups_per_window).store(out + sizeof(XYZZ<F>) * (size_t)j);
 }
 
@@ -598,7 +631,7 @@
         const size_t slots = BaPlan<F>::slots_bound(max_entries, n_buckets, l + 1);
         const uint32_t n_threads = (uint32_t)((slots + BA_K - 1) / BA_K);
         const uint32_t blocks = (n_threads + BA_THREADS - 1) / BA_THREADS;
-        fill_work_kernel<<<(n_buckets + 255) / 256, 256, 0, st>>>(hist, off[l + 1], n_buckets, 1u << (l + 1), 0, slot_bucket);
+        fill_work_kernel<<<(n_buckets + 255) / 256, 256, 0, st>>>(hist, off[l + 1], n_buckets, 1u << (l + 1), 0, slot_bucket, 0);
         BaLevel lv{hist, off[l], off[l + 1], slot_bucket, n_buckets, (uint32_t)l};
         to_heavy();
         if (ev && l == 0) cudaEventRecord(ev[0], hv);
@@ -615,7 +648,7 @@
     }
     XYZZ<F>* bucket_sum = (XYZZ<F>*)sorted0;
     bucket_finish_kernel<F><<<(n_buckets + 127) / 128, 128, 0, st>>>(in, hist, off[L], n_buckets, (uint32_t)L, bucket_sum);
-    group_sum_kernel<F, 1><<<(groups + 127) / 128, 128, 0, st>>>((const uint8_t*)bucket_sum, hist, off[L], D.half, groups, 1u << L, 0, D.group, group_out);
+    group_sum_kernel<F, 1><<<(groups + 127) / 128, 128, 0, st>>>((const uint8_t*)bucket_sum, hist, off[L], D.half, groups, 1u << L, 0, D.group, group_out, 0);
     ZKE_COUNT_LAUNCH(2);
 }
 template <>
@@ -684,7 +717,7 @@
 
 template <class F>
 void MsmPlan<F>::run(const uint8_t* points, const uint8_t* scalars, uint32_t n, const MsmConfig& cfg, uint8_t* ws,
-                     uint8_t* result, cudaStream_t st, cudaEvent_t* ev, const Heavy* heavy) {
+                     uint8_t* result, cudaStream_t st, cudaEvent_t* ev, const Heavy* heavy, const MsmGroup& group) {
     Digits D;
     D.c = cfg.c;
     D.n_windows = (255 + cfg.c - 1) / cfg.c;
@@ -732,17 +765,25 @@
     if (two_level) sort.place(take);
     else cursor = (uint32_t*)take(4 * ((size_t)n_buckets + 1));
 
+    const uint32_t M = group.members;
+    if (M == 0) return;
+    if (M > 1 && (two_level || use_ba || cfg.precomputed)) throw std::runtime_error("grouped MSMs take the witness configuration only");
+    const size_t wss = workspace_bytes(n, cfg);
+    const size_t sstride = group.scalar_stride, rstride = group.result_stride;
+    auto per_member = [M](uint32_t blocks) { return dim3(std::max(1u, (blocks + M - 1) / M), M); };
+    auto zero = [&](void* dst, size_t pitch, size_t bytes) { cudaMemset2DAsync(dst, M > 1 ? pitch : bytes, 0, bytes, M, st); };
+
     uint8_t* res_ones = result;
     uint8_t* res_windows = result + sizeof(XYZZ<F>) * MSM_ONES_SLOTS;
-    cudaMemsetAsync(result, 0, sizeof(XYZZ<F>) * MSM_RESULT_SLOTS, st);
+    zero(result, rstride, sizeof(XYZZ<F>) * MSM_RESULT_SLOTS);
 
     const uint32_t* gen_count = nullptr;
     const uint32_t* gen_idx = nullptr;
     if (cfg.classify) {
-        cudaMemsetAsync(counters, 0, 8, st);
-        classify_kernel<F><<<(n + 255) / 256, 256, 0, st>>>(points, scalars, n, ones_list, gen_list, counters);
+        zero(counters, wss, 8);
+        classify_kernel<F><<<dim3((n + 255) / 256, M), 256, 0, st>>>(points, scalars, n, ones_list, gen_list, counters, wss, sstride);
         uint32_t upper = (n + LIST_FANIN - 1) / LIST_FANIN;
-        sum_affine_list_kernel<F><<<(upper + 127) / 128, 128, 0, st>>>(points, ones_list, counters, 0, red_a);
+        sum_affine_list_kernel<F><<<dim3((upper + 127) / 128, M), 128, 0, st>>>(points, ones_list, counters, 0, red_a, wss);
         ZKE_COUNT_LAUNCH(2);
         uint8_t *src = red_a, *dst = red_b;
         uint32_t level = 0;
@@ -751,7 +792,8 @@
             const bool last = next <= MSM_ONES_SLOTS;
             uint8_t* out = last ? res_ones : dst;
             const uint32_t threads = last ? (uint32_t)MSM_ONES_SLOTS : next;
-            sum_xyzz_kernel<F><<<(threads + 63) / 64, 64, 0, st>>>(src, counters, 0, level, last ? MSM_ONES_SLOTS : 0, out);
+            sum_xyzz_kernel<F><<<dim3((threads + 63) / 64, M), 64, 0, st>>>(src, counters, 0, level, last ? MSM_ONES_SLOTS : 0, out,
+                                                                           wss, last ? rstride : wss);
             ZKE_COUNT_LAUNCH(1);
             if (last) break;
             uint8_t* t = src; src = dst; dst = t;
@@ -765,11 +807,11 @@
     if (two_level) {
         sort.run(scalars, gen_idx, gen_count, n, D, hist, offsets, entries, st);
     } else {
-        cudaMemsetAsync(hist, 0, 4 * ((size_t)n_buckets + 1), st);
-        cudaMemsetAsync(cursor, 0, 4 * ((size_t)n_buckets + 1), st);
-        digit_hist_kernel<<<sms * 8, 256, 0, st>>>(scalars, gen_idx, gen_count, n, D, hist);
-        exclusive_scan(hist, n_buckets, 0, 0, offsets, tiles, st);
-        digit_scatter_kernel<<<sms * 8, 256, 0, st>>>(scalars, gen_idx, gen_count, n, D, offsets, cursor, entries);
+        zero(hist, wss, 4 * ((size_t)n_buckets + 1));
+        zero(cursor, wss, 4 * ((size_t)n_buckets + 1));
+        digit_hist_kernel<<<per_member(sms * 8), 256, 0, st>>>(scalars, gen_idx, gen_count, n, D, hist, wss, sstride);
+        exclusive_scan(hist, n_buckets, 0, 0, offsets, tiles, st, M, wss);
+        digit_scatter_kernel<<<per_member(sms * 8), 256, 0, st>>>(scalars, gen_idx, gen_count, n, D, offsets, cursor, entries, wss, sstride);
         ZKE_COUNT_LAUNCH(2);
     }
     if (use_ba) {
@@ -777,13 +819,13 @@
         ZKE_COUNT_LAUNCH(1);
         run_ba<F>(cfg, hist, offsets, n_buckets, max_entries, tiles, ba_ws, D, groups, group_out, st, ev, heavy);
     } else {
-        exclusive_scan(hist, n_buckets, D.chunk, 0, chunk_off, tiles, st);
-        fill_work_kernel<<<(n_buckets + 255) / 256, 256, 0, st>>>(hist, chunk_off, n_buckets, D.chunk, 0, work_bucket);
+        exclusive_scan(hist, n_buckets, D.chunk, 0, chunk_off, tiles, st, M, wss);
+        fill_work_kernel<<<dim3((n_buckets + 255) / 256, M), 256, 0, st>>>(hist, chunk_off, n_buckets, D.chunk, 0, work_bucket, wss);
         {
             const uint32_t nblk = (uint32_t)((max_chunks + ORDER_BLOCK - 1) / ORDER_BLOCK);
-            chunk_key_hist_kernel<<<nblk, ORDER_BLOCK, 4 * D.chunk, st>>>(hist, chunk_off, work_bucket, n_buckets, D.chunk, order_mat);
-            exclusive_scan(order_mat, nblk * D.chunk, 0, 0, order_off, order_tiles, st);
-            chunk_order_kernel<<<nblk, ORDER_BLOCK, 0, st>>>(hist, chunk_off, work_bucket, n_buckets, D.chunk, order_off, order);
+            chunk_key_hist_kernel<<<dim3(nblk, M), ORDER_BLOCK, 4 * D.chunk, st>>>(hist, chunk_off, work_bucket, n_buckets, D.chunk, order_mat, wss);
+            exclusive_scan(order_mat, nblk * D.chunk, 0, 0, order_off, order_tiles, st, M, wss);
+            chunk_order_kernel<<<dim3(nblk, M), ORDER_BLOCK, 0, st>>>(hist, chunk_off, work_bucket, n_buckets, D.chunk, order_off, order, wss);
             ZKE_COUNT_LAUNCH(2);
         }
         cudaStream_t st_light = st;
@@ -814,9 +856,9 @@
             size_t pad = 0;
             if (const char* e = getenv("ZKE_CHUNK_PAD_SMEM")) pad = (size_t)std::max(0, std::min(48 * 1024, atoi(e)));
             if (done) {}
-            else if (minb >= 6) chunk_sum_kernel<F, 6><<<sms * 6 * waves, 128, pad, st>>>(points, entries, offsets, hist, chunk_off, work_bucket, order, n_buckets, D.chunk, partial);
-            else if (minb == 5) chunk_sum_kernel<F, 5><<<sms * 5 * waves, 128, pad, st>>>(points, entries, offsets, hist, chunk_off, work_bucket, order, n_buckets, D.chunk, partial);
-            else chunk_sum_kernel<F, 4><<<sms * 4 * waves, 128, pad, st>>>(points, entries, offsets, hist, chunk_off, work_bucket, order, n_buckets, D.chunk, partial);
+            else if (minb >= 6) chunk_sum_kernel<F, 6><<<per_member(sms * 6 * waves), 128, pad, st>>>(points, entries, offsets, hist, chunk_off, work_bucket, order, n_buckets, D.chunk, partial, wss);
+            else if (minb == 5) chunk_sum_kernel<F, 5><<<per_member(sms * 5 * waves), 128, pad, st>>>(points, entries, offsets, hist, chunk_off, work_bucket, order, n_buckets, D.chunk, partial, wss);
+            else chunk_sum_kernel<F, 4><<<per_member(sms * 4 * waves), 128, pad, st>>>(points, entries, offsets, hist, chunk_off, work_bucket, order, n_buckets, D.chunk, partial, wss);
         }
         if (ev) cudaEventRecord(ev[1], st);
         if (st != st_light) {
@@ -828,18 +870,18 @@
         uint32_t *off_cur = chunk_off, *off_next = off2;
         uint32_t levels = 0;
         for (uint32_t pass = 0; pass < cfg.extra_passes; ++pass) {
-            exclusive_scan(hist, n_buckets, D.chunk, levels + 1, off_next, tiles, st);
-            fill_work_kernel<<<(n_buckets + 255) / 256, 256, 0, st>>>(hist, off_next, n_buckets, D.chunk, levels + 1, work_bucket);
-            partial_pass_kernel<F><<<sms * 4, 128, 0, st>>>(items, hist, off_cur, off_next, work_bucket, n_buckets, D.chunk, levels, items_next);
+            exclusive_scan(hist, n_buckets, D.chunk, levels + 1, off_next, tiles, st, M, wss);
+            fill_work_kernel<<<dim3((n_buckets + 255) / 256, M), 256, 0, st>>>(hist, off_next, n_buckets, D.chunk, levels + 1, work_bucket, wss);
+            partial_pass_kernel<F><<<per_member(sms * 4), 128, 0, st>>>(items, hist, off_cur, off_next, work_bucket, n_buckets, D.chunk, levels, items_next, wss);
             ZKE_COUNT_LAUNCH(2);
             uint8_t* t = items; items = items_next; items_next = t;
             uint32_t* o = off_cur; off_cur = off_next; off_next = o;
             ++levels;
         }
-        group_sum_kernel<F, 0><<<(groups + 127) / 128, 128, 0, st>>>(items, hist, off_cur, D.half, groups, D.chunk, levels, D.group, group_out);
-    }
-    window_reduce_kernel<F><<<bucket_sets, 512, 0, st>>>(group_out, groups_per_window);
-    gather_windows_kernel<F><<<1, 64, 0, st>>>(group_out, groups_per_window, bucket_sets, res_windows);
+        group_sum_kernel<F, 0><<<dim3((groups + 127) / 128, M), 128, 0, st>>>(items, hist, off_cur, D.half, groups, D.chunk, levels, D.group, group_out, wss);
+    }
+    window_reduce_kernel<F><<<dim3(bucket_sets, M), 512, 0, st>>>(group_out, groups_per_window, wss);
+    gather_windows_kernel<F><<<dim3(1, M), 64, 0, st>>>(group_out, groups_per_window, bucket_sets, res_windows, wss, rstride);
     ZKE_COUNT_LAUNCH(5);
 }
 
diff --git a/zk-email-verify_b200/csrc/msm.cuh b/zk-email-verify_b200/csrc/msm.cuh
--- a/zk-email-verify_b200/csrc/msm.cuh
+++ b/zk-email-verify_b200/csrc/msm.cuh
@@ -21,12 +21,15 @@
 static const int MSM_MAX_WINDOWS = 32;
 static const int MSM_RESULT_SLOTS = MSM_ONES_SLOTS + MSM_MAX_WINDOWS;
 
+struct MsmGroup { uint32_t members; size_t scalar_stride, result_stride; };
+
 template <class F>
 struct MsmPlan {
     static size_t workspace_bytes(uint32_t n, const MsmConfig& cfg);
     struct Heavy { cudaStream_t st; cudaEvent_t before, after; };
     static void run(const uint8_t* points, const uint8_t* scalars, uint32_t n, const MsmConfig& cfg, uint8_t* workspace,
-                    uint8_t* result, cudaStream_t st, cudaEvent_t* ev = nullptr, const Heavy* heavy = nullptr);
+                    uint8_t* result, cudaStream_t st, cudaEvent_t* ev = nullptr, const Heavy* heavy = nullptr,
+                    const MsmGroup& group = MsmGroup{1, 0, 0});
 };
 
 }
diff --git a/zk-email-verify_b200/host/zkemail_b200/_lib.py b/zk-email-verify_b200/host/zkemail_b200/_lib.py
--- a/zk-email-verify_b200/host/zkemail_b200/_lib.py
+++ b/zk-email-verify_b200/host/zkemail_b200/_lib.py
@@ -114,6 +114,7 @@
                                                         ctypes.POINTER(c_size_t), c_char_p, c_size_t])
 zke_upload_inputs = _sig("zke_upload_inputs", c_int, [c_void_p, c_void_p, c_size_t, c_char_p, c_size_t])
 zke_ctx_set_lanes = _sig("zke_ctx_set_lanes", c_int, [c_void_p, c_int])
+zke_ctx_set_msm_group = _sig("zke_ctx_set_msm_group", c_int, [c_void_p, c_int])
 zke_ctx_profile = _sig("zke_ctx_profile", c_int, [c_void_p, c_int])
 zke_ctx_profile_get = _sig("zke_ctx_profile_get", c_int, [c_void_p, ctypes.POINTER(ctypes.c_double), ctypes.POINTER(c_u64)])
 STAGES = ("witness", "matvec", "ntt", "msm_a", "msm_b1", "msm_c", "msm_h", "msm_h_buckets", "msm_b2")
```

Result: no change. 48.19 (median of 6 runs) (+0.9%).
